# carefree0910/carefree-learn

Hardware: AMD Instinct MI355X
Metric: train samples/sec + step ms, ViT-B/16 bf16 DDP at 1/2/4/8 MI355X (higher is better)
Workload: dtype bf16

## Files before the change

carefree-learn_amd/csrc/common.h:

```cpp
#pragma once
#include <hip/hip_runtime.h>
#include <stdint.h>
#include <stdio.h>
#include <stdarg.h>

#include "../../include/cfhip.h"

typedef uint16_t bf16_t;
typedef __attribute__((ext_vector_type(8))) short bf16x8;
typedef __attribute__((ext_vector_type(4))) short s16x4;
typedef __attribute__((ext_vector_type(4))) float f32x4;
typedef __attribute__((ext_vector_type(2))) unsigned int u32x2;
typedef __attribute__((ext_vector_type(4))) unsigned int u32x4;

#define LDS_PTR(p) ((__attribute__((address_space(3))) void*)(p))

__device__ __forceinline__ void lds_dma16(__amdgpu_buffer_rsrc_t rsrc, const void* lds_dst, unsigned voff) {
#ifdef CFHIP_DMA_BUILTIN
  __builtin_amdgcn_raw_ptr_buffer_load_lds(rsrc, LDS_PTR(const_cast<void*>(lds_dst)), 16, voff, 0, 0, 0);
  return;
#endif
  const unsigned la = (unsigned)(uintptr_t)LDS_PTR(const_cast<void*>(lds_dst));
  asm volatile("s_nop 0\n\tbuffer_load_dwordx4 %1, %2, 0 offen lds" ::"{m0}"(la), "v"(voff), "s"(rsrc) : "memory");
}

__device__ __forceinline__ void lds_dma16_s(__amdgpu_buffer_rsrc_t rsrc, const void* lds_dst, unsigned voff, unsigned soff) {
  const unsigned la = (unsigned)(uintptr_t)LDS_PTR(const_cast<void*>(lds_dst));
  asm volatile("s_nop 0\n\tbuffer_load_dwordx4 %1, %2, %3 offen lds" ::"{m0}"(la), "v"(voff), "s"(rsrc), "s"(soff) : "memory");
}
__device__ __forceinline__ void lds_dma_wait_all() { asm volatile("s_waitcnt vmcnt(0)" ::: "memory"); }

void cfhip_set_error(const char* fmt, ...);

#define CFHIP_REQUIRE(cond, ...)          \
  do {                                    \
    if (!(cond)) {                        \
      cfhip_set_error(__VA_ARGS__);       \
      return CFHIP_ERR_INVALID;           \
    }                                     \
  } while (0)

#define CFHIP_CHECK_LAUNCH(name)                                                \
  do {                                                                          \
    hipError_t e__ = hipGetLastError();                                         \
    if (e__ != hipSuccess) {                                                    \
      cfhip_set_error("%s: launch failed: %s", name, hipGetErrorString(e__));   \
      return CFHIP_ERR_LAUNCH;                                                  \
    }                                                                           \
  } while (0)

__device__ __forceinline__ float bf16_to_f32(bf16_t v) {
  return __uint_as_float(((unsigned)v) << 16);
}
typedef __bf16 bf16x2_native __attribute__((ext_vector_type(2)));
__device__ __forceinline__ bf16_t f32_to_bf16(float f) {
  return __builtin_bit_cast(unsigned short, (__bf16)f);
}
__device__ __forceinline__ unsigned pack_bf16x2(float lo, float hi) {
  const bf16x2_native v = {(__bf16)lo, (__bf16)hi};
  return __builtin_bit_cast(unsigned, v);
}
__device__ __forceinline__ float bf16lo(unsigned w) { return __uint_as_float(w << 16); }
__device__ __forceinline__ float bf16hi(unsigned w) { return __uint_as_float(w & 0xffff0000u); }

__device__ __forceinline__ void gelu_parts(float x, float& cdf, float& e) {
#ifdef CFHIP_GELU_PROBE
  cdf = 0.5f;
  e = 1.0f;
  return;
#endif
  const float t = __builtin_amdgcn_rcpf(fmaf(0.3275911f * 0.70710678118654752440f, fabsf(x), 1.0f));
  e = __builtin_amdgcn_exp2f(x * x * (-0.5f * 1.4426950408889634f));
  float poly = fmaf(t, 1.061405429f, -1.453152027f);
  poly = fmaf(t, poly, 1.421413741f);
  poly = fmaf(t, poly, -0.284496736f);
  poly = fmaf(t, poly, 0.254829592f);
  const float erf_abs = fmaf(-(poly * t), e, 1.0f);
  cdf = fmaf(copysignf(0.5f, x), erf_abs, 0.5f);
}
__device__ __forceinline__ float gelu_erf_f(float x) {
  float cdf, e;
  gelu_parts(x, cdf, e);
  return x * cdf;
}
__device__ __forceinline__ float gelu_erf_grad_f(float x) {
  float cdf, e;
  gelu_parts(x, cdf, e);
  return fmaf(x * 0.39894228040143267794f, e, cdf);
}

__device__ __forceinline__ float sigmoid_1702(float x) {
  return __builtin_amdgcn_rcpf(1.0f + __builtin_amdgcn_exp2f(x * (-1.702f * 1.4426950408889634f)));
}
__device__ __forceinline__ float quick_gelu_f(float x) { return x * sigmoid_1702(x); }
__device__ __forceinline__ float quick_gelu_grad_f(float x) {
  const float s = sigmoid_1702(x);
  return s * fmaf(1.702f * x, 1.0f - s, 1.0f);
}

struct Philox {
  unsigned c[4];
};

__device__ __forceinline__ Philox philox4x32_10(unsigned long long ctr, unsigned long long seed) {
  constexpr unsigned M0 = 0xD2511F53u, M1 = 0xCD9E8D57u, W0 = 0x9E3779B9u, W1 = 0xBB67AE85u;
  unsigned c0 = (unsigned)ctr, c1 = (unsigned)(ctr >> 32), c2 = 0u, c3 = 0u;
  unsigned k0 = (unsigned)seed, k1 = (unsigned)(seed >> 32);
#pragma unroll
  for (int r = 0; r < 10; ++r) {
    const unsigned hi0 = __umulhi(M0, c0), lo0 = M0 * c0;
    const unsigned hi1 = __umulhi(M1, c2), lo1 = M1 * c2;
    c0 = hi1 ^ c1 ^ k0;
    c1 = lo1;
    c2 = hi0 ^ c3 ^ k1;
    c3 = lo0;
    k0 += W0;
    k1 += W1;
  }
  return Philox{{c0, c1, c2, c3}};
}

__device__ __forceinline__ float wave_sum(float v) {
#pragma unroll
  for (int off = 32; off > 0; off >>= 1) v += __shfl_xor(v, off, 64);
  return v;
}
__device__ __forceinline__ float wave_max(float v) {
#pragma unroll
  for (int off = 32; off > 0; off >>= 1) v = fmaxf(v, __shfl_xor(v, off, 64));
  return v;
}
__device__ __forceinline__ float block_sum(float v, float* red) {
  v = wave_sum(v);
  const int lane = threadIdx.x & 63, wave = threadIdx.x >> 6;
  __syncthreads();
  if (lane == 0) red[wave] = v;
  __syncthreads();
  float s = 0.f;
  for (int w = 0; w < (int)(blockDim.x >> 6); ++w) s += red[w];
  return s;
}

__device__ __forceinline__ float ld_act(const void* p, long i, bool f32) {
  return f32 ? reinterpret_cast<const float*>(p)[i] : bf16_to_f32(reinterpret_cast<const bf16_t*>(p)[i]);
}
template <bool IN_F32>
__device__ __forceinline__ void ld_act8(const void* p, long off, float (&v)[8]) {
  if (IN_F32) {
    const f32x4 a = *reinterpret_cast<const f32x4*>(reinterpret_cast<const float*>(p) + off);
    const f32x4 b = *reinterpret_cast<const f32x4*>(reinterpret_cast<const float*>(p) + off + 4);
    v[0] = a[0]; v[1] = a[1]; v[2] = a[2]; v[3] = a[3]; v[4] = b[0]; v[5] = b[1]; v[6] = b[2]; v[7] = b[3];
  } else {
    const u32x4 w = *reinterpret_cast<const u32x4*>(reinterpret_cast<const bf16_t*>(p) + off);
#pragma unroll
    for (int e = 0; e < 4; ++e) {
      v[2 * e] = bf16lo(w[e]);
      v[2 * e + 1] = bf16hi(w[e]);
    }
  }
}
__device__ __forceinline__ void st_bf16x8(bf16_t* p, long off, const float (&v)[8]) {
  *reinterpret_cast<u32x4*>(p + off) = u32x4{pack_bf16x2(v[0], v[1]), pack_bf16x2(v[2], v[3]), pack_bf16x2(v[4], v[5]),
                                             pack_bf16x2(v[6], v[7])};
}
__device__ __forceinline__ float silu_f(float v) { return v * __builtin_amdgcn_rcpf(1.0f + __builtin_amdgcn_exp2f(-1.4426950408889634f * v)); }
__device__ __forceinline__ float silu_grad_f(float v) {
  const float s = __builtin_amdgcn_rcpf(1.0f + __builtin_amdgcn_exp2f(-1.4426950408889634f * v));
  return s * fmaf(v, 1.0f - s, 1.0f);
}
```

carefree-learn_amd/csrc/gemm.hip:

```cpp
#include "gemm_device.h"

namespace {

template <bool AT, bool BT, class C>
struct ItemCtx {
  int m0, n0, z, klen, nk, tile_n;
  __amdgpu_buffer_rsrc_t a_rsrc, b_rsrc;
  StagePlan<C::A_INSTR> pa;
  StagePlan<C::B_INSTR> pb;
  unsigned yx[C::A_INSTR];
  int bshift[C::B_INSTR];
  int btap[C::B_INSTR];
  int kb;
};

template <bool AT, bool BT, class C, int CONV = 0>
__device__ __forceinline__ ItemCtx<AT, BT, C> setup_item(const GemmParams& p, int item, int wave, int lane) {
  ItemCtx<AT, BT, C> c;
  const int ntiles = p.tiles_m * p.tiles_n;
  c.z = item / ntiles;
  const int tile = item - c.z * ntiles;
  int tile_m;
  if (p.group_n > 0) {
    const int per_group = p.group_n * p.tiles_m;
    const int grp = tile / per_group;
    const int first_n = grp * p.group_n;
    const int gw = min(p.group_n, p.tiles_n - first_n);
    const int r = tile - grp * per_group;
    tile_m = r / gw;
    c.tile_n = first_n + (r - tile_m * gw);
  } else if (p.group_n < 0) {
    const int gm = -p.group_n;
    const int per_group = gm * p.tiles_n;
    const int grp = tile / per_group;
    const int first_m = grp * gm;
    const int gh = min(gm, p.tiles_m - first_m);
    const int r = tile - grp * per_group;
    c.tile_n = r / gh;
    tile_m = first_m + (r - c.tile_n * gh);
  } else {
    tile_m = tile / p.tiles_n;
    c.tile_n = tile - tile_m * p.tiles_n;
  }
  c.m0 = tile_m * C::BM;
  c.n0 = c.tile_n * C::BN;
  const int kb = c.z * p.k_chunk;
  c.kb = kb;
  c.klen = min(p.K - kb, p.k_chunk);
  c.nk = (c.klen + C::BK - 1) / C::BK;
  const int rows_a = p.M - c.m0, rows_b = p.N - c.n0;
  const bf16_t* a_base = AT ? p.A + (long)kb * p.lda + c.m0 : p.A + (long)c.m0 * p.lda + kb;
  const bf16_t* b_base = BT ? p.B + (long)kb * p.ldb + c.n0 : p.B + (long)c.n0 * p.ldb + kb;
  const long a_bytes = AT ? ((long)(c.klen - 1) * p.lda + rows_a) * 2 : ((long)(rows_a - 1) * p.lda + c.klen) * 2;
  const long b_bytes = BT ? ((long)(c.klen - 1) * p.ldb + rows_b) * 2 : ((long)(rows_b - 1) * p.ldb + c.klen) * 2;
  if constexpr (CONV == 2) {
    static_assert(CONV != 2 || (AT && BT), "implicit weight gradient: layout (1,1), a K-step = BK pixels");
    const int back = min(kb, p.conv_w + 1);
    const long span = min((long)p.K - (kb - back), (long)back + c.klen + p.conv_w + 1);
    c.b_rsrc = make_rsrc(p.B + (long)(kb - back) * p.conv_c, span * p.conv_c * 2);
    constexpr int SLOTS = C::BN / 8;
#pragma unroll
    for (int j = 0; j < C::B_INSTR; ++j) {
      const int inst = wave * C::B_INSTR + j;
      const int krow = inst * (64 / SLOTS) + lane / SLOTS;
      const int sl = lane % SLOTS;
      const int col = (((sl >> 1) ^ mkey<C::BN>(krow)) << 4) + ((sl & 1) << 3);
      const int n = c.n0 + col;
      const int tap = n / p.conv_c;
      const int ch = n - tap * p.conv_c;
      const int ky = (tap * 11) >> 5;
      const int dy = ky - 1, dx = tap - 3 * ky - 1;
      c.pb.kpos[j] = krow;
      c.pb.voff[j] = (col < rows_b) ? 0u : OOB;
      c.bshift[j] = ((back + krow + dy * p.conv_w + dx) * p.conv_c + ch) * 2;
      c.btap[j] = (dy + 1) | ((dx + 1) << 2);
    }
  } else {
    c.b_rsrc = make_rsrc(b_base, b_bytes);
    c.pb = make_plan<BT, C::BN, C::B_INSTR, C::BK>(wave, lane, p.ldb, C::B_PADDED ? min(rows_b, C::BN) : rows_b);
  }
  if constexpr (CONV == 1) {
    static_assert(!AT, "implicit convolution: k-major A, a K-step = BK channels of one tap");
    const int back = min(c.m0, p.conv_w + 1);
    const long span = min((long)p.M - (c.m0 - back), (long)back + C::BM + p.conv_w + 1);
    c.a_rsrc = make_rsrc(p.A + (long)(c.m0 - back) * p.conv_c, span * p.conv_c * 2);
#pragma unroll
    for (int j = 0; j < C::A_INSTR; ++j) {
      const int inst = wave * C::A_INSTR + j;
      constexpr int SPR = C::BK / 8;
      const int row = inst * (64 / SPR) + lane / SPR;
      const int chunk = (lane % SPR) ^ kswz<C::BK>(row);
      c.pa.kpos[j] = chunk * 8;
      c.pa.voff[j] = (row < rows_a) ? (unsigned)(((back + row) * p.conv_c + chunk * 8) * 2) : OOB;
      const int m = c.m0 + row;
      const int q = m / p.conv_w;
      c.yx[j] = ((unsigned)(q % p.conv_h) << 16) | (unsigned)(m - q * p.conv_w);
    }
  } else {
    c.a_rsrc = make_rsrc(a_base, a_bytes);
    c.pa = make_plan<AT, C::BM, C::A_INSTR, C::BK>(wave, lane, p.lda, rows_a);
  }
  return c;
}

template <class C>
__device__ __forceinline__ void stage_tile_conv(const __amdgpu_buffer_rsrc_t rsrc, char* lds_tile, int wave,
                                                const StagePlan<C::A_INSTR>& pl, const unsigned (&yx)[C::A_INSTR],
                                                const GemmParams& p, int kstep) {
  const int tap = (int)(((float)kstep + 0.5f) * p.conv_inv_kpt);
  const int c0 = (kstep - tap * p.conv_kpt) * C::BK;
  const int ky = (tap * 11) >> 5;
  const int dy = ky - 1, dx = tap - 3 * ky - 1;
  const int shift = ((dy * p.conv_w + dx) * p.conv_c + c0) * 2;
#pragma unroll
  for (int j = 0; j < C::A_INSTR; ++j) {
    const int y = (int)(yx[j] >> 16) + dy, x = (int)(yx[j] & 0xffffu) + dx;
    const bool ok = pl.voff[j] != OOB && (unsigned)y < (unsigned)p.conv_h && (unsigned)x < (unsigned)p.conv_w;
    const unsigned off = ok ? pl.voff[j] + (unsigned)shift : OOB;
    lds_dma16(rsrc, lds_tile + (wave * C::A_INSTR + j) * 1024, off);
  }
}

template <class C, class Ctx>
__device__ __forceinline__ void stage_tile_wgrad(const Ctx& c, char* lds_tile, int wave, const GemmParams& p, int kstep) {
  const int k0 = kstep * C::BK;
#pragma unroll
  for (int j = 0; j < C::B_INSTR; ++j) {
    const int kl = k0 + (int)c.pb.kpos[j];
    const unsigned pix = (unsigned)(c.kb + kl);
    const unsigned q = __umulhi(pix, p.conv_magic_w);
    const int x = (int)(pix - q * (unsigned)p.conv_w) + ((c.btap[j] >> 2) - 1);
    const int y = (int)(q - __umulhi(q, p.conv_magic_h) * (unsigned)p.conv_h) + ((c.btap[j] & 3) - 1);
    const bool ok = c.pb.voff[j] != OOB && kl < c.klen && (unsigned)y < (unsigned)p.conv_h && (unsigned)x < (unsigned)p.conv_w;
    const unsigned off = ok ? (unsigned)(c.bshift[j] + k0 * p.conv_c * 2) : OOB;
    lds_dma16(c.b_rsrc, lds_tile + (wave * C::B_INSTR + j) * 1024, off);
  }
}

template <bool AT, bool BT, class C, int CONV = 0>
__device__ __forceinline__ void stage_step(const ItemCtx<AT, BT, C>& c, const GemmParams& p, char* smem,
                                           int slot, int wave, int kstep) {
  char* st = smem + slot * C::STAGE_BYTES;
  if constexpr (CONV == 1) stage_tile_conv<C>(c.a_rsrc, st, wave, c.pa, c.yx, p, kstep + c.kb / C::BK);
  else stage_tile<AT, C::A_INSTR, C::BK>(c.a_rsrc, st, wave, c.pa, p.lda, kstep * C::BK, c.klen);
  if constexpr (CONV == 2) {
    stage_tile_wgrad<C>(c, st + C::A_BYTES, wave, p, kstep);
    return;
  }
  stage_tile<BT, C::B_INSTR, C::BK>(c.b_rsrc, st + C::A_BYTES, wave, c.pb, p.ldb, kstep * C::BK, c.klen);
}

__device__ __forceinline__ int xcd_item() {
  const int G = gridDim.x;
  const int bid = blockIdx.x;
  const int q8 = G >> 3, r8 = G & 7;
  const int xcd = bid & 7, loc = bid >> 3;
  return (xcd < r8 ? xcd * (q8 + 1) : r8 * (q8 + 1) + (xcd - r8) * q8) + loc;
}

template <bool AT, bool BT, int EPI, class C, int CONV = 0, bool BG = false>
__device__ __forceinline__ void gemm_tile(const GemmParams& p, const int item, char* smem) {
  constexpr int D = C::NSTAGE - 1;
  static_assert(kFlatEpilogue<C> ? C::NW * 16 * (C::FN * 16 + 4) * 4 <= C::LDS_BYTES : C::NW * 16 * (C::FN * 16) * 4 <= C::STAGE_BYTES,
                "epilogue staging must fit in one ring slot (80-column wave tiles: in the ring)");

  const int tid = threadIdx.x;
  const int lane = tid & 63;
  const int wave = __builtin_amdgcn_readfirstlane(tid >> 6);
  const int wm = wave / C::WN, wn = wave % C::WN;

  const ItemCtx<AT, BT, C> cur = setup_item<AT, BT, C, CONV>(p, item, wave, lane);
  const int nk = cur.nk;
  int rd = 0;
#pragma unroll
  for (int st = 0; st < D; ++st)
    if (st < nk) stage_step<AT, BT, C, CONV>(cur, p, smem, st, wave, st);

  f32x4 acc[C::FM][C::FN];
#pragma unroll
  for (int mi = 0; mi < C::FM; ++mi)
#pragma unroll
    for (int ni = 0; ni < C::FN; ++ni) acc[mi][ni] = f32x4{0.f, 0.f, 0.f, 0.f};
  float accb[BG ? C::FM : 1];
  if constexpr (BG) {
#pragma unroll
    for (int mi = 0; mi < C::FM; ++mi) accb[mi] = 0.f;
  }
  const bool do_bg = BG && cur.tile_n == 0 && wn == 0 && (p.bgrad != nullptr || p.bgrad_slabs != nullptr);

  for (int t = 0; t < nk; ++t) {
    const int younger = min(D - 1, nk - 1 - t);
    if (D >= 3 && younger >= 2) CFHIP_WAIT_VMCNT(2 * C::LPS);
    else if (D >= 2 && younger == 1) CFHIP_WAIT_VMCNT(1 * C::LPS);
    else CFHIP_WAIT_VMCNT(0);
    __builtin_amdgcn_s_barrier();
    if (t + D < nk CFHIP_ABLATE_AND(!(p.ablate & 1))) {
      int wr = rd + D;
      if (wr >= C::NSTAGE) wr -= C::NSTAGE;
      stage_step<AT, BT, C, CONV>(cur, p, smem, wr, wave, t + D);
    }
    const char* tile = smem + rd * C::STAGE_BYTES;
    if (true CFHIP_ABLATE_AND(!(p.ablate & 2))) compute_tile<AT, BT, C>(tile, tile + C::A_BYTES, wm, wn, lane, acc);
    if constexpr (BG) {
      if (do_bg) bias_rows<C>(tile, wm, lane, accb);
    }
    rd = rd + 1 == C::NSTAGE ? 0 : rd + 1;
  }
#ifdef CFHIP_ABLATE
  if (p.ablate & 4) return;
#endif
  const int m0 = cur.m0, n0 = cur.n0, z = cur.z;
  if constexpr (BG) {
    if (do_bg) {
#pragma unroll
      for (int mi = 0; mi < C::FM; ++mi) {
        float v = accb[mi];
        v += __shfl_xor(v, 16, 64);
        v += __shfl_xor(v, 32, 64);
        const int m = m0 + wm * (C::FM * 16) + mi * 16 + (lane & 15);
        if ((lane >> 4) == 0 && m < p.M) {
          if (p.bgrad_slabs != nullptr) p.bgrad_slabs[(long)z * p.M + m] = v;
          else p.bgrad[m] = p.bgrad_acc ? p.bgrad[m] + v : v;
        }
      }
    }
  }
  __builtin_amdgcn_s_barrier();
  int eslot = rd - 1;
  if (eslot < 0) eslot += C::NSTAGE;
  epilogue<EPI, C>(p, acc, kFlatEpilogue<C> ? smem : smem + eslot * C::STAGE_BYTES, m0, n0, z, wm, wn, wave, lane);
}

template <bool AT, bool BT, int EPI, class C, int CONV = 0, bool BG = false>
__global__ __launch_bounds__(C::NT, C::WAVES_PER_SIMD)
void gemm_bf16_kernel(GemmParams p) {
  extern __shared__ __attribute__((aligned(16))) char smem[];
  gemm_tile<AT, BT, EPI, C, CONV, BG>(p, xcd_item(), smem);
}

template <bool AT, bool BT, int EPI, class C, int CONV = 0>
__global__ __launch_bounds__(C::NT, C::WAVES_PER_SIMD)
void gemm_bf16_phase_kernel(GemmParams p) {
  extern __shared__ __attribute__((aligned(16))) char smem[];
  static_assert(C::BK == 32 && C::NSTAGE >= 3 && C::NSTAGE <= 7 && C::WM == 2, "phase kernel: BK = 32, 3-7 ring slots, 2 wave rows");
  static_assert(5 * C::LPS < 64, "vmcnt is a 6-bit counter");
  constexpr int D = C::NSTAGE - 1;
  static_assert(C::NW * 16 * (C::FN * 16 + 4) * 4 <= C::LDS_BYTES, "epilogue staging must fit in the (free) ring");
  constexpr int PH = (C::FM / 2) * C::FN >= 16 ? 2 : 1;
  constexpr int HM = C::FM / PH;
  const int nwg = gridDim.x;
  const int bid = blockIdx.x;
  const int q8 = nwg >> 3, r8 = nwg & 7;
  const int xcd = bid & 7, loc = bid >> 3;
  const int item = (xcd < r8 ? xcd * (q8 + 1) : r8 * (q8 + 1) + (xcd - r8) * q8) + loc;
  const int tid = threadIdx.x;
  const int lane = tid & 63;
  const int wave = __builtin_amdgcn_readfirstlane(tid >> 6);
  const int wm = wave / C::WN, wn = wave % C::WN;
  const int i = lane & 15, g = lane >> 4;

  const ItemCtx<AT, BT, C> cur = setup_item<AT, BT, C, CONV>(p, item, wave, lane);
  const int nk = cur.nk;
  f32x4 acc[C::FM][C::FN];
#pragma unroll
  for (int mi = 0; mi < C::FM; ++mi)
#pragma unroll
    for (int ni = 0; ni < C::FN; ++ni) acc[mi][ni] = f32x4{0.f, 0.f, 0.f, 0.f};

#pragma unroll
  for (int st = 0; st < D; ++st)
    if (st < nk) stage_step<AT, BT, C, CONV>(cur, p, smem, st, wave, st);
  wait_stages<C::LPS>(min(min(nk, D) - 1, 5));
  __builtin_amdgcn_s_barrier();
  if (wm == 1) __builtin_amdgcn_s_barrier();

  int rd = 0, wr = D;
  for (int t = 0; t < nk; ++t) {
    const char* a_tile = smem + rd * C::STAGE_BYTES;
    const char* b_tile = a_tile + C::A_BYTES;
    bf16x8 bfr[C::FN], af[HM];
#pragma unroll
    for (int ph = 0; ph < PH; ++ph) {
      if (ph == 0) {
#pragma unroll
        for (int n = 0; n < C::FN; ++n)
          bfr[n] = BT ? frag_mmajor<C::BN>(b_tile, wn * (C::FN * 16) + n * 16, 0, lane)
                      : frag_kmajor<C::BK>(b_tile, wn * (C::FN * 16) + n * 16, 0, i, g);
      }
#pragma unroll
      for (int m = 0; m < HM; ++m)
        af[m] = AT ? frag_mmajor<C::BM>(a_tile, wm * (C::FM * 16) + (ph * HM + m) * 16, 0, lane)
                   : frag_kmajor<C::BK>(a_tile, wm * (C::FM * 16) + (ph * HM + m) * 16, 0, i, g);
      if (ph == PH - 1)
        wait_stages<C::LPS>(max(0, min(min(D - 2, nk - 2 - t), 5)));
      __builtin_amdgcn_sched_barrier(0);
      __builtin_amdgcn_s_barrier();
      __builtin_amdgcn_sched_barrier(0);
      if (ph == PH - 1 && t + D < nk) stage_step<AT, BT, C, CONV>(cur, p, smem, wr, wave, t + D);
      __builtin_amdgcn_s_setprio(1);
#pragma unroll
      for (int m = 0; m < HM; ++m)
#pragma unroll
        for (int n = 0; n < C::FN; ++n)
          acc[ph * HM + m][n] = __builtin_amdgcn_mfma_f32_16x16x32_bf16(bfr[n], af[m], acc[ph * HM + m][n], 0, 0, 0);
      __builtin_amdgcn_s_setprio(0);
      __builtin_amdgcn_sched_barrier(0);
      __builtin_amdgcn_s_barrier();
      __builtin_amdgcn_sched_barrier(0);
    }
    rd = rd + 1 == C::NSTAGE ? 0 : rd + 1;
    wr = wr + 1 == C::NSTAGE ? 0 : wr + 1;
  }
  if (wm == 0) __builtin_amdgcn_s_barrier();
#ifdef CFHIP_ABLATE
  if (p.ablate & 4) return;
#endif
  epilogue<EPI, C>(p, acc, smem, cur.m0, cur.n0, cur.z, wm, wn, wave, lane);
}

__global__ void splitk_reduce_kernel(const float* __restrict__ slabs, void* C, const float* bias,
                                     int M, int N, long ldc, int splits, int out_f32, int accumulate,
                                     const float* __restrict__ bgrad_slabs, float* bgrad, int bgrad_acc) {
  const long n4 = N >> 2;
  const long total = (long)M * n4;
  for (long idx = blockIdx.x * (long)blockDim.x + threadIdx.x; idx < total;
       idx += (long)gridDim.x * blockDim.x) {
    if (bgrad != nullptr && idx < M) {
      float b = 0.f;
      for (int z = 0; z < splits; ++z) b += bgrad_slabs[(long)z * M + idx];
      bgrad[idx] = bgrad_acc ? bgrad[idx] + b : b;
    }
    const int row = (int)(idx / n4);
    const int col = (int)(idx - (long)row * n4) * 4;
    f32x4 v = {0.f, 0.f, 0.f, 0.f};
    for (int z = 0; z < splits; ++z)
      v += *reinterpret_cast<const f32x4*>(slabs + ((long)z * M + row) * N + col);
    if (bias != nullptr) v += *reinterpret_cast<const f32x4*>(bias + col);
    const long off = (long)row * ldc + col;
    if (out_f32) {
      float* dst = reinterpret_cast<float*>(C) + off;
      if (accumulate) v += *reinterpret_cast<const f32x4*>(dst);
      *reinterpret_cast<f32x4*>(dst) = v;
    } else {
      bf16_t* dst = reinterpret_cast<bf16_t*>(C) + off;
      *reinterpret_cast<u32x2*>(dst) = u32x2{pack_bf16x2(v[0], v[1]), pack_bf16x2(v[2], v[3])};
    }
  }
}

__global__ void splitk_reduce_filter_kernel(const float* __restrict__ slabs, float* __restrict__ dW, int Cout, int Cin,
                                            int splits, int accumulate, const float* __restrict__ bgrad_slabs,
                                            float* bgrad, int bgrad_acc) {
  const long c4n = Cin >> 2;
  const long total = (long)Cout * c4n;
  const long N = 9L * Cin;
  for (long idx = blockIdx.x * (long)blockDim.x + threadIdx.x; idx < total; idx += (long)gridDim.x * blockDim.x) {
    if (bgrad != nullptr && idx < Cout) {
      float b = 0.f;
      for (int z = 0; z < splits; ++z) b += bgrad_slabs[(long)z * Cout + idx];
      bgrad[idx] = bgrad_acc ? bgrad[idx] + b : b;
    }
    const int co = (int)(idx / c4n);
    const int c = (int)(idx - (long)co * c4n) * 4;
    float o[36];
#pragma unroll
    for (int tap = 0; tap < 9; ++tap) {
      f32x4 v = {0.f, 0.f, 0.f, 0.f};
      for (int z = 0; z < splits; ++z)
        v += *reinterpret_cast<const f32x4*>(slabs + ((long)z * Cout + co) * N + (long)tap * Cin + c);
#pragma unroll
      for (int e = 0; e < 4; ++e) o[e * 9 + tap] = v[e];
    }
    float* dst = dW + ((long)co * Cin + c) * 9;
#pragma unroll
    for (int i = 0; i < 9; ++i) {
      f32x4 v = {o[4 * i], o[4 * i + 1], o[4 * i + 2], o[4 * i + 3]};
      if (accumulate) v += *reinterpret_cast<const f32x4*>(dst + 4 * i);
      *reinterpret_cast<f32x4*>(dst + 4 * i) = v;
    }
  }
}

__global__ void gemm_bf16_generic_kernel(GemmParams p, int a_trans, int b_trans) {
  const long total = (long)p.M * p.N;
  for (long idx = blockIdx.x * (long)blockDim.x + threadIdx.x; idx < total;
       idx += (long)gridDim.x * blockDim.x) {
    const int m = (int)(idx / p.N), n = (int)(idx - (long)m * p.N);
    float acc = 0.f, asum = 0.f;
    for (int k = 0; k < p.K; ++k) {
      const float a = bf16_to_f32(a_trans ? p.A[(long)k * p.lda + m] : p.A[(long)m * p.lda + k]);
      const float b = bf16_to_f32(b_trans ? p.B[(long)k * p.ldb + n] : p.B[(long)n * p.ldb + k]);
      acc = fmaf(a, b, acc);
      asum += a;
    }
    if (p.bgrad != nullptr && n == 0) p.bgrad[m] = p.bgrad_acc ? p.bgrad[m] + asum : asum;
    if (p.bias != nullptr) acc += p.bias[n];
    const long off = (long)m * p.ldc + n;
    if (p.epilogue == CFHIP_EPI_GELU) {
      const float pre = bf16_to_f32(f32_to_bf16(acc));
      if (p.aux_out != nullptr) p.aux_out[off] = f32_to_bf16(acc);
      acc = p.quick ? quick_gelu_f(pre) : gelu_erf_f(pre);
    } else if (p.epilogue == CFHIP_EPI_RESIDUAL) {
      acc += p.out_f32 ? reinterpret_cast<const float*>(p.aux_in)[off] : bf16_to_f32(p.aux_in[off]);
    } else if (p.epilogue == CFHIP_EPI_DGELU) {
      acc *= p.quick ? quick_gelu_grad_f(bf16_to_f32(p.aux_in[off])) : gelu_erf_grad_f(bf16_to_f32(p.aux_in[off]));
    }
    if (p.out_f32) {
      float* dst = reinterpret_cast<float*>(p.C) + off;
      *dst = p.accumulate ? *dst + acc : acc;
    } else {
      reinterpret_cast<bf16_t*>(p.C)[off] = f32_to_bf16(acc);
    }
  }
}

inline bool aligned16(const void* p) { return (reinterpret_cast<uintptr_t>(p) & 15u) == 0; }

using CfgA = Cfg<128, 128, 2, 2, 2, 64>;
using CfgB = Cfg<128, 128, 2, 2, 2, 32>;
using CfgC = Cfg<128, 128, 2, 2, 3, 32>;
using CfgD = Cfg<128, 64, 2, 2, 2, 64>;
using CfgE = Cfg<128, 128, 2, 2, 4, 32>;
using CfgF = Cfg<128, 64, 2, 2, 2, 32>;
using CfgG = Cfg<128, 64, 2, 2, 3, 32>;
using CfgP = Cfg<256, 256, 2, 4, 4, 32>;
using CfgQ = Cfg<256, 128, 2, 4, 3, 32>;
using CfgR = Cfg<256, 128, 2, 2, 3, 32>;
using CfgS = Cfg<128, 256, 2, 2, 3, 32>;
using CfgT = Cfg<256, 128, 2, 4, 6, 32>;
using CfgU = Cfg<256, 256, 2, 4, 5, 32>;
using CfgW = Cfg<256, 256, 2, 4, 2, 64>;
using CfgY = Cfg<192, 128, 2, 4, 2, 64>;
using CfgZ = Cfg<192, 128, 2, 2, 2, 64>;
using CfgV = Cfg<128, 256, 2, 4, 2, 64>;
using CfgH = Cfg<128, 160, 2, 2, 4, 32>;
using CfgI = Cfg<128, 160, 2, 2, 2, 64>;
constexpr int NUM_CFG = 17;
constexpr int BK_MAX = 64;

int g_gemm_config = -1;
#ifdef CFHIP_ABLATE
int g_gemm_ablate = 0;
#endif
int g_gemm_heuristic = 9;
int g_gemm_group_n = 8;
int g_conv_form = -1;
int g_conv_split = -1;

template <bool AT, bool BT, int EPI, class C, bool PIPE, int CONV = 0>
int launch_cfg(const GemmParams& p, dim3 grid, hipStream_t s) {
  void (*kern)(GemmParams) = nullptr;
  if (PIPE && p.bgrad != nullptr) {
    cfhip_set_error("gemm: the fused bias gradient is not provided by the big-tile kernel (gemm_config 7 / 8)");
    return CFHIP_ERR_INVALID;
  }
  if constexpr (PIPE) kern = gemm_bf16_phase_kernel<AT, BT, EPI, C, CONV>;
  else if constexpr (AT && BT && EPI == CFHIP_EPI_NONE) {
    if (p.bgrad != nullptr) {
      if constexpr (C::BM * C::BN <= 192 * 128) kern = gemm_bf16_kernel<AT, BT, EPI, C, CONV, true>;
      else {
        cfhip_set_error("gemm: the fused bias gradient is not provided by this tile configuration");
        return CFHIP_ERR_INVALID;
      }
    } else kern = gemm_bf16_kernel<AT, BT, EPI, C, CONV, false>;
  } else kern = gemm_bf16_kernel<AT, BT, EPI, C, CONV>;
  static bool attr_done_bg[2] = {false, false};
  bool& attr_done = attr_done_bg[p.bgrad != nullptr ? 1 : 0];
  if (!attr_done && C::LDS_BYTES > 64 * 1024) {
    hipError_t e = hipFuncSetAttribute(reinterpret_cast<const void*>(kern),
                                       hipFuncAttributeMaxDynamicSharedMemorySize, C::LDS_BYTES);
    if (e != hipSuccess) {
      cfhip_set_error("gemm: cannot reserve %d bytes of LDS: %s", C::LDS_BYTES, hipGetErrorString(e));
      return CFHIP_ERR_LAUNCH;
    }
    attr_done = true;
  }
  GemmParams q = p;
  const int gn = g_gemm_group_n;
  q.group_n = (gn > 0 && gn < p.tiles_n) || (gn < 0 && p.tiles_m > 1) ? gn : 0;
  hipLaunchKernelGGL(kern, grid, dim3(C::NT), C::LDS_BYTES, s, q);
  return CFHIP_OK;
}

template <class C, bool PIPE>
constexpr bool kHasEpilogues = !(C::BM == 128 && C::BN == 128 && C::BK == 32 && C::NSTAGE == 2);
template <class C, bool PIPE>
constexpr bool kHasTn = !(PIPE && C::BM == 256 && C::BN == 128 && C::WN == 4 && C::NSTAGE == 3);

template <class C, bool PIPE = false>
int launch_layout(GemmParams p, int a_trans, int b_trans, int epilogue, int split_k, hipStream_t s) {
  p.tiles_m = (p.M + C::BM - 1) / C::BM;
  p.tiles_n = (p.N + C::BN - 1) / C::BN;
  const long a_span = a_trans ? (long)p.k_chunk * p.lda * 2 : (long)C::BM * p.lda * 2;
  const long b_span = b_trans ? (long)p.k_chunk * p.ldb * 2 : (long)C::BN * p.ldb * 2;
  CFHIP_REQUIRE(a_span < 0x7fffffffL && b_span < 0x7fffffffL,
                "gemm: operand tile span exceeds 2 GiB (lda=%ld ldb=%ld K=%d)", p.lda, p.ldb, p.K);
  p.splits = split_k;
  dim3 grid(p.tiles_m * p.tiles_n * split_k);
  if (!a_trans && !b_trans) {
    switch (epilogue) {
      case CFHIP_EPI_NONE: return launch_cfg<false, false, CFHIP_EPI_NONE, C, PIPE>(p, grid, s);
      case CFHIP_EPI_GELU: return launch_cfg<false, false, CFHIP_EPI_GELU, C, PIPE>(p, grid, s);
      case CFHIP_EPI_RESIDUAL:
        if constexpr (kHasEpilogues<C, PIPE>) return launch_cfg<false, false, CFHIP_EPI_RESIDUAL, C, PIPE>(p, grid, s);
        break;
      default: break;
    }
  } else if (!a_trans && b_trans) {
    switch (epilogue) {
      case CFHIP_EPI_NONE: return launch_cfg<false, true, CFHIP_EPI_NONE, C, PIPE>(p, grid, s);
      case CFHIP_EPI_DGELU:
        if constexpr (kHasEpilogues<C, PIPE>) return launch_cfg<false, true, CFHIP_EPI_DGELU, C, PIPE>(p, grid, s);
        break;
      default: break;
    }
  } else if (epilogue == CFHIP_EPI_NONE) {
    if constexpr (kHasTn<C, PIPE>) return launch_cfg<true, true, CFHIP_EPI_NONE, C, PIPE>(p, grid, s);
  }
  cfhip_set_error("gemm: epilogue %d is not provided for layout (%d,%d)", epilogue, a_trans, b_trans);
  return CFHIP_ERR_INVALID;
}

int g_cfg_class[4] = {-1, -1, -1, -1};

int pick_config(int M, int N, int a_trans, int b_trans) {
  if (g_gemm_config >= 0 && g_gemm_config < NUM_CFG) return g_gemm_config;
  if (M >= 1024 || a_trans) {
    const int cls = a_trans ? 3 : b_trans ? 2 : (N >= 2560 ? 0 : 1);
    if (g_cfg_class[cls] >= 0 && g_cfg_class[cls] < NUM_CFG) return g_cfg_class[cls];
  }
  if (g_gemm_heuristic >= 7) {
    if (a_trans) return 1;
    if (M >= 512) {
      const long t14 = (long)((M + 191) / 192) * ((N + 127) / 128);
      if (t14 < 160 || (N < 512 && N % 128 != 0 && N % 64 == 0)) return 3;
    }
    if (M >= 1024) return (g_gemm_heuristic >= 9 || (g_gemm_heuristic >= 8 && N <= 1024)) ? 15 : 14;
    if (b_trans) return 1;
    return N <= 1024 ? 3 : 0;
  }
  if (g_gemm_heuristic >= 6) {
    if (a_trans) return 1;
    if (M >= 1024) {
      if (b_trans) return 8;
      return N >= 2560 ? 14 : 0;
    }
    if (b_trans) return 1;
    return N <= 1024 ? 3 : 0;
  }
  if (g_gemm_heuristic == 1) {
    if (a_trans && (long)M * N <= 768L * 768L) return 0;
    if (a_trans || b_trans) return 1;
    return N <= 1024 ? 1 : 0;
  }
  if (g_gemm_heuristic >= 2) {
    if (a_trans) return 1;
    if (N >= 2560 && M >= 1024) return 8;
    if (g_gemm_heuristic >= 4 && b_trans && M >= 1024) return 8;
    if (g_gemm_heuristic >= 5 && M >= 1024) return 8;
    if (g_gemm_heuristic >= 3) {
      const long tiles128 = (long)((M + 127) / 128) * ((N + 127) / 128);
      if (tiles128 >= 1024) return 0;
    }
  }
  if (a_trans || b_trans) return 1;
  if (N <= 1024) return 3;
  return 0;
}

}

#ifdef CFHIP_ABLATE
int cfhip_internal_set_attn_ablate(int v);
#endif
int cfhip_internal_set_ln_fused(int v);
int cfhip_internal_set_attn_persistent(int v);
int cfhip_internal_set_attn_one_pass(int v);
int cfhip_internal_set_attn_pers_ctas(int v);
int cfhip_internal_set_grouped_variant(int v);
int cfhip_internal_set_attn_two_tiles(int v);
int cfhip_internal_set_attn_short_max(int v);

extern "C" int cfhip_set_option(const char* name, int value) {
  if (name != nullptr && strcmp(name, "gemm_config") == 0) {
    g_gemm_config = value;
    return CFHIP_OK;
  }
  if (name != nullptr && strcmp(name, "gemm_heuristic") == 0) {
    g_gemm_heuristic = value;
    return CFHIP_OK;
  }
  static const char* const cls_names[4] = {"gemm_cfg_nt_wide", "gemm_cfg_nt", "gemm_cfg_nn", "gemm_cfg_tn"};
  for (int i = 0; i < 4; ++i)
    if (name != nullptr && strcmp(name, cls_names[i]) == 0) {
      g_cfg_class[i] = value;
      return CFHIP_OK;
    }
  if (name != nullptr && strcmp(name, "gemm_group_n") == 0) {
    g_gemm_group_n = value;
    return CFHIP_OK;
  }
  if (name != nullptr && strcmp(name, "conv_form") == 0) {
    g_conv_form = value;
    return CFHIP_OK;
  }
  if (name != nullptr && strcmp(name, "conv_split") == 0) {
    g_conv_split = value;
    return CFHIP_OK;
  }
  if (name != nullptr && strcmp(name, "ln_bwd_fused") == 0) return cfhip_internal_set_ln_fused(value);
  if (name != nullptr && strcmp(name, "attn_persistent") == 0) return cfhip_internal_set_attn_persistent(value);
  if (name != nullptr && strcmp(name, "attn_one_pass") == 0) return cfhip_internal_set_attn_one_pass(value);
  if (name != nullptr && strcmp(name, "attn_pers_ctas") == 0) return cfhip_internal_set_attn_pers_ctas(value);
  if (name != nullptr && strcmp(name, "grouped_variant") == 0) return cfhip_internal_set_grouped_variant(value);
  if (name != nullptr && strcmp(name, "attn_two_tiles") == 0) return cfhip_internal_set_attn_two_tiles(value);
  if (name != nullptr && strcmp(name, "attn_short_max") == 0) return cfhip_internal_set_attn_short_max(value);
#ifdef CFHIP_ABLATE
  if (name != nullptr && strcmp(name, "gemm_ablate") == 0) {
    g_gemm_ablate = value;
    return CFHIP_OK;
  }
  if (name != nullptr && strcmp(name, "attn_ablate") == 0) return cfhip_internal_set_attn_ablate(value);
#endif
  cfhip_set_error("set_option: unknown option '%s'", name ? name : "(null)");
  return CFHIP_ERR_INVALID;
}

static int resolve_config(int cfg, int a_trans, int epilogue, bool bias_grad) {
  if (cfg == 8 && a_trans) cfg = 1;
  if (bias_grad && ((cfg >= 7 && cfg <= 13) || cfg == 16)) cfg = 1;
  if (cfg == 1 && (epilogue == CFHIP_EPI_RESIDUAL || epilogue == CFHIP_EPI_DGELU)) cfg = 3;
  return cfg;
}

extern "C" int cfhip_gemm_kernel_name(int M, int N, int K, int a_trans, int b_trans, int epilogue, char* out, size_t out_bytes) {
  CFHIP_REQUIRE(out != nullptr && out_bytes >= 96, "gemm_kernel_name: buffer of at least 96 bytes");
  static const char* const cfg_names[NUM_CFG] = {
      "Cfg<128, 128, 2, 2, 2, 64>", "Cfg<128, 128, 2, 2, 2, 32>", "Cfg<128, 128, 2, 2, 3, 32>", "Cfg<128, 64, 2, 2, 2, 64>",
      "Cfg<128, 128, 2, 2, 4, 32>", "Cfg<128, 64, 2, 2, 2, 32>", "Cfg<128, 64, 2, 2, 3, 32>", "Cfg<256, 256, 2, 4, 4, 32>",
      "Cfg<256, 128, 2, 4, 3, 32>", "Cfg<256, 128, 2, 2, 3, 32>", "Cfg<128, 256, 2, 2, 3, 32>", "Cfg<256, 128, 2, 4, 6, 32>",
      "Cfg<256, 256, 2, 4, 5, 32>", "Cfg<256, 256, 2, 4, 2, 64>", "Cfg<192, 128, 2, 4, 2, 64>", "Cfg<192, 128, 2, 2, 2, 64>",
      "Cfg<128, 256, 2, 4, 2, 64>"};
  int epi = epilogue == CFHIP_EPI_QGELU ? CFHIP_EPI_GELU : epilogue == CFHIP_EPI_DQGELU ? CFHIP_EPI_DGELU : epilogue;
  int cfg = pick_config(M, N, a_trans, b_trans);
  cfg = resolve_config(cfg, a_trans, epi, false);
  const bool phase = cfg >= 7 && cfg <= 12;
  snprintf(out, out_bytes, "%s<%s, %s, %d, %s>", phase ? "gemm_bf16_phase_kernel" : "gemm_bf16_kernel",
           a_trans ? "true" : "false", b_trans ? "true" : "false", epi, cfg_names[cfg]);
  return CFHIP_OK;
}

static thread_local int g_last_config = -2;
extern "C" int cfhip_gemm_last_config(void) { return g_last_config; }

static int gemm_bf16_impl(const void* A, const void* B, void* C, const float* bias,
                          const void* aux_in, void* aux_out, int M, int N, int K, int64_t lda,
                          int64_t ldb, int64_t ldc, int a_trans, int b_trans, int epilogue,
                          int out_dtype, int accumulate, int split_k, void* workspace,
                          size_t workspace_bytes, float* bias_grad, int bias_grad_accumulate,
                          void* stream, int config_rows) {
  CFHIP_REQUIRE(A && B && C, "gemm: null operand");
  CFHIP_REQUIRE(bias_grad == nullptr || (a_trans && b_trans),
                "gemm: the fused bias gradient exists for layout (1,1) only");
  CFHIP_REQUIRE(M > 0 && N > 0 && K > 0, "gemm: empty problem M=%d N=%d K=%d", M, N, K);
  CFHIP_REQUIRE(epilogue >= 0 && epilogue <= 5, "gemm: bad epilogue %d", epilogue);
  const int quick = epilogue == CFHIP_EPI_QGELU || epilogue == CFHIP_EPI_DQGELU;
  if (epilogue == CFHIP_EPI_QGELU) epilogue = CFHIP_EPI_GELU;
  if (epilogue == CFHIP_EPI_DQGELU) epilogue = CFHIP_EPI_DGELU;
  CFHIP_REQUIRE(!(epilogue == CFHIP_EPI_RESIDUAL || epilogue == CFHIP_EPI_DGELU) || aux_in,
                "gemm: epilogue %d needs aux_in", epilogue);
  CFHIP_REQUIRE(!accumulate || (out_dtype == 1 && epilogue == CFHIP_EPI_NONE), "gemm: accumulate needs f32 output and epilogue NONE");
  CFHIP_REQUIRE(!(epilogue == CFHIP_EPI_GELU || epilogue == CFHIP_EPI_DGELU) || out_dtype == 0,
                "gemm: the GELU / GELU' epilogues write bf16");
  CFHIP_REQUIRE(!(a_trans && !b_trans), "gemm: layout (a_trans=1, b_trans=0) is not provided");
  if (split_k < 1) split_k = 1;
  hipStream_t s = reinterpret_cast<hipStream_t>(stream);

  GemmParams p;
  p.A = reinterpret_cast<const bf16_t*>(A);
  p.B = reinterpret_cast<const bf16_t*>(B);
  p.C = C;
  p.bias = bias;
  p.aux_in = reinterpret_cast<const bf16_t*>(aux_in);
  p.aux_out = reinterpret_cast<bf16_t*>(aux_out);
  p.M = M; p.N = N; p.K = K;
  p.lda = lda; p.ldb = ldb; p.ldc = ldc;
  p.epilogue = epilogue; p.out_f32 = out_dtype; p.accumulate = accumulate;
  p.slabs = nullptr;
  p.tiles_m = p.tiles_n = 0;
  p.quick = quick;
#ifdef CFHIP_ABLATE
  p.ablate = g_gemm_ablate;
#endif
  p.bgrad = bias_grad;
  p.bgrad_acc = bias_grad_accumulate;
  p.bgrad_slabs = nullptr;
  p.conv_h = p.conv_w = p.conv_c = p.conv_kpt = 0;
  p.conv_inv_kpt = 0.f;
  p.conv_magic_w = p.conv_magic_h = 0u;
  p.k_chunk = ((K + BK_MAX - 1) / BK_MAX) * BK_MAX;

  const bool k_ok = (a_trans && b_trans) || (K % 8 == 0);
  const bool fast = k_ok && (lda % 8 == 0) && (ldb % 8 == 0) && (N % 4 == 0) &&
                    (ldc % 4 == 0) && (!a_trans || M % 8 == 0) && (!b_trans || N % 8 == 0) &&
                    aligned16(A) && aligned16(B) && aligned16(C) &&
                    (bias == nullptr || aligned16(bias)) && (aux_in == nullptr || aligned16(aux_in)) &&
                    (aux_out == nullptr || aligned16(aux_out));
  if (!fast) {
    CFHIP_REQUIRE(split_k == 1, "gemm: split_k needs the aligned fast path");
    const long total = (long)M * N;
    const int blocks = (int)((total + 255) / 256 > 65535 ? 65535 : (total + 255) / 256);
    g_last_config = -1;
    hipLaunchKernelGGL(gemm_bf16_generic_kernel, dim3(blocks), dim3(256), 0, s, p, a_trans, b_trans);
    CFHIP_CHECK_LAUNCH("gemm_generic");
    return CFHIP_OK;
  }

  if (split_k > 1) {
    CFHIP_REQUIRE(epilogue == CFHIP_EPI_NONE, "gemm: split_k supports epilogue NONE only");
    const int steps = (K + BK_MAX - 1) / BK_MAX;
    if (split_k > steps) split_k = steps;
    const int per = (steps + split_k - 1) / split_k;
    split_k = (steps + per - 1) / per;
    p.k_chunk = per * BK_MAX;
  }
  if (split_k > 1) {
    const size_t need = (size_t)split_k * M * N * sizeof(float) + (bias_grad ? (size_t)split_k * M * sizeof(float) : 0);
    if (workspace == nullptr || workspace_bytes < need) {
      cfhip_set_error("gemm: split_k=%d needs %zu workspace bytes, got %zu", split_k, need, workspace_bytes);
      return CFHIP_ERR_WORKSPACE;
    }
    p.slabs = reinterpret_cast<float*>(workspace);
    if (bias_grad) p.bgrad_slabs = p.slabs + (size_t)split_k * M * N;
  }

  int rc;
  int cfg = pick_config(config_rows > M ? config_rows : M, N, a_trans, b_trans);
  cfg = resolve_config(cfg, a_trans, epilogue, bias_grad != nullptr);
  g_last_config = cfg;
  switch (cfg) {
    case 1: rc = launch_layout<CfgB>(p, a_trans, b_trans, epilogue, split_k, s); break;
    case 2: rc = launch_layout<CfgC>(p, a_trans, b_trans, epilogue, split_k, s); break;
    case 3: rc = launch_layout<CfgD>(p, a_trans, b_trans, epilogue, split_k, s); break;
    case 4: rc = launch_layout<CfgE>(p, a_trans, b_trans, epilogue, split_k, s); break;
    case 5: rc = launch_layout<CfgF>(p, a_trans, b_trans, epilogue, split_k, s); break;
    case 6: rc = launch_layout<CfgG>(p, a_trans, b_trans, epilogue, split_k, s); break;
    case 7: rc = launch_layout<CfgP, true>(p, a_trans, b_trans, epilogue, split_k, s); break;
    case 8: rc = launch_layout<CfgQ, true>(p, a_trans, b_trans, epilogue, split_k, s); break;
    case 9: rc = launch_layout<CfgR, true>(p, a_trans, b_trans, epilogue, split_k, s); break;
    case 10: rc = launch_layout<CfgS, true>(p, a_trans, b_trans, epilogue, split_k, s); break;
    case 11: rc = launch_layout<CfgT, true>(p, a_trans, b_trans, epilogue, split_k, s); break;
    case 12: rc = launch_layout<CfgU, true>(p, a_trans, b_trans, epilogue, split_k, s); break;
    case 13: rc = launch_layout<CfgW>(p, a_trans, b_trans, epilogue, split_k, s); break;
    case 14: rc = launch_layout<CfgY>(p, a_trans, b_trans, epilogue, split_k, s); break;
    case 15: rc = launch_layout<CfgZ>(p, a_trans, b_trans, epilogue, split_k, s); break;
    case 16: rc = launch_layout<CfgV>(p, a_trans, b_trans, epilogue, split_k, s); break;
    default: rc = launch_layout<CfgA>(p, a_trans, b_trans, epilogue, split_k, s); break;
  }
  if (rc != CFHIP_OK) return rc;
  CFHIP_CHECK_LAUNCH("gemm_bf16");

  if (split_k > 1) {
    const long total = (long)M * (N / 4);
    int blocks = (int)((total + 255) / 256);
    if (blocks > 2048) blocks = 2048;
    hipLaunchKernelGGL(splitk_reduce_kernel, dim3(blocks), dim3(256), 0, s, p.slabs, C, bias, M, N,
                       (long)ldc, split_k, out_dtype, accumulate, p.bgrad_slabs, p.bgrad, p.bgrad_acc);
    CFHIP_CHECK_LAUNCH("splitk_reduce");
  }
  return CFHIP_OK;
}

extern "C" int cfhip_gemm_bf16(const void* A, const void* B, void* C, const float* bias,
                               const void* aux_in, void* aux_out, int M, int N, int K, int64_t lda,
                               int64_t ldb, int64_t ldc, int a_trans, int b_trans, int epilogue,
                               int out_dtype, int accumulate, int split_k, void* workspace,
                               size_t workspace_bytes, float* bias_grad, int bias_grad_accumulate,
                               void* stream) {
  return gemm_bf16_impl(A, B, C, bias, aux_in, aux_out, M, N, K, lda, ldb, ldc, a_trans, b_trans, epilogue, out_dtype, accumulate,
                        split_k, workspace, workspace_bytes, bias_grad, bias_grad_accumulate, stream, 0);
}

extern "C" int cfhip_gemm_bf16_rows(const void* A, const void* B, void* C, const float* bias, const void* aux_in, void* aux_out,
                                    int M, int N, int K, int64_t lda, int64_t ldb, int64_t ldc, int b_trans, int epilogue,
                                    int out_dtype, int config_rows, void* stream) {
  CFHIP_REQUIRE(config_rows >= M, "gemm_rows: config_rows = %d is less than M = %d", config_rows, M);
  return gemm_bf16_impl(A, B, C, bias, aux_in, aux_out, M, N, K, lda, ldb, ldc, 0, b_trans, epilogue, out_dtype, 0, 1, nullptr, 0,
                        nullptr, 0, stream, config_rows);
}

template <class C, bool PIPE>
static int launch_conv(GemmParams p, int split_k, hipStream_t s) {
  p.tiles_m = (p.M + C::BM - 1) / C::BM;
  p.tiles_n = (p.N + C::BN - 1) / C::BN;
  p.splits = split_k;
  return launch_cfg<false, false, CFHIP_EPI_NONE, C, PIPE, 1>(p, dim3(p.tiles_m * p.tiles_n * split_k), s);
}

struct ConvPlan { int form, split; };

static int conv_split_for(long tiles, long slots, int Cin) {
  const int steps = (9 * Cin + BK_MAX - 1) / BK_MAX;
  if (tiles * 2 > slots || steps < 16) return 1;
  long split = (slots + tiles - 1) / tiles;
  if (split > steps / 8) split = steps / 8;
  if (split < 1) split = 1;
  const int per = (int)((steps + split - 1) / split);
  return (steps + per - 1) / per;
}

static ConvPlan conv_plan(long pixels, int Cin, int Cout) {
  ConvPlan pl;
  pl.form = pixels >= 1024 ? 0 : 1;
  if (g_conv_form != -2 && (long)((Cout + 159) / 160) * 160 * 8 <= 9L * Cout) pl.form = 3;
  if (g_conv_form >= 0 && g_conv_form <= 3) pl.form = g_conv_form;
  static const int bm[4] = {256, 128, 128, 128}, bn[4] = {128, 128, 160, 160}, slots[4] = {512, 1024, 512, 512};
  if (pl.form == 3 && Cin % 64 != 0) pl.form = 2;
  const long tiles = ((pixels + bm[pl.form] - 1) / bm[pl.form]) * ((Cout + bn[pl.form] - 1) / bn[pl.form]);
  pl.split = conv_split_for(tiles, slots[pl.form], Cin);
  if (g_conv_split >= 1) {
    const int steps = (9 * Cin + BK_MAX - 1) / BK_MAX;
    int split = g_conv_split > steps ? steps : g_conv_split;
    const int per = (steps + split - 1) / split;
    pl.split = (steps + per - 1) / per;
  }
  return pl;
}

extern "C" size_t cfhip_conv3x3_workspace(int B, int H, int W, int Cin, int Cout) {
  const long pixels = (long)B * H * W;
  const int split = conv_plan(pixels, Cin, Cout).split;
  return split > 1 ? (size_t)split * pixels * Cout * sizeof(float) : 0;
}

extern "C" int cfhip_conv3x3_nhwc_bf16(const void* X, const void* Wk, const float* bias, void* Y, int B, int H, int W,
                                       int Cin, int Cout, void* workspace, size_t workspace_bytes, void* stream) {
  CFHIP_REQUIRE(X && Wk && Y, "conv3x3: null operand");
  CFHIP_REQUIRE(B > 0 && H > 0 && W > 0 && H < 65536 && W < 65536, "conv3x3: bad image shape %d x %d x %d", B, H, W);
  CFHIP_REQUIRE(Cin > 0 && Cin % 32 == 0, "conv3x3: Cin = %d must be a multiple of 32 (one K-step = 32 channels of a tap)", Cin);
  CFHIP_REQUIRE(Cout > 0 && Cout % 8 == 0, "conv3x3: Cout = %d must be a multiple of 8", Cout);
  const long pixels = (long)B * H * W;
  CFHIP_REQUIRE(pixels < (1L << 30) && 9L * Cin < (1L << 20), "conv3x3: problem too large (%ld pixels, Cin %d)", pixels, Cin);
  CFHIP_REQUIRE(aligned16(X) && aligned16(Wk) && aligned16(Y) && (bias == nullptr || aligned16(bias)),
                "conv3x3: operands must be 16-byte aligned");
  GemmParams p;
  p.A = reinterpret_cast<const bf16_t*>(X);
  p.B = reinterpret_cast<const bf16_t*>(Wk);
  p.C = Y;
  p.bias = bias;
  p.aux_in = nullptr;
  p.aux_out = nullptr;
  p.M = (int)pixels; p.N = Cout; p.K = 9 * Cin;
  p.lda = Cin; p.ldb = 9L * Cin; p.ldc = Cout;
  p.epilogue = CFHIP_EPI_NONE; p.out_f32 = 0; p.accumulate = 0;
  p.k_chunk = ((p.K + BK_MAX - 1) / BK_MAX) * BK_MAX;
  p.slabs = nullptr;
  p.tiles_m = p.tiles_n = 0; p.splits = 1;
  p.bgrad = nullptr; p.bgrad_slabs = nullptr; p.bgrad_acc = 0;
  p.quick = 0;
#ifdef CFHIP_ABLATE
  p.ablate = 0;
#endif
  p.conv_h = H; p.conv_w = W; p.conv_c = Cin; p.conv_kpt = Cin / 32;
  p.conv_inv_kpt = 1.0f / (float)p.conv_kpt;
  p.conv_magic_w = p.conv_magic_h = 0u;
  const ConvPlan plan = conv_plan(pixels, Cin, Cout);
  const int split = plan.split;
  if (split > 1) {
    const size_t need = (size_t)split * pixels * Cout * sizeof(float);
    if (workspace == nullptr || workspace_bytes < need) {
      cfhip_set_error("conv3x3: split_k=%d needs %zu workspace bytes (cfhip_conv3x3_workspace), got %zu", split, need, workspace_bytes);
      return CFHIP_ERR_WORKSPACE;
    }
    const int steps = (p.K + BK_MAX - 1) / BK_MAX;
    p.k_chunk = ((steps + split - 1) / split) * BK_MAX;
    p.slabs = reinterpret_cast<float*>(workspace);
  }
  hipStream_t s = (hipStream_t)stream;
  int rc;
  switch (plan.form) {
    case 0: rc = launch_conv<CfgQ, true>(p, split, s); break;
    case 2: rc = launch_conv<CfgH, false>(p, split, s); break;
    case 3:
      p.conv_kpt = Cin / 64;
      p.conv_inv_kpt = 1.0f / (float)p.conv_kpt;
      rc = launch_conv<CfgI, false>(p, split, s);
      break;
    default: rc = launch_conv<CfgB, false>(p, split, s); break;
  }
  if (rc != CFHIP_OK) return rc;
  CFHIP_CHECK_LAUNCH("conv3x3_nhwc");
  if (split > 1) {
    const long total = (long)p.M * (p.N / 4);
    int blocks = (int)((total + 255) / 256);
    if (blocks > 2048) blocks = 2048;
    hipLaunchKernelGGL(splitk_reduce_kernel, dim3(blocks), dim3(256), 0, s, p.slabs, Y, bias, p.M, p.N, (long)p.ldc, split,
                       0, 0, (const float*)nullptr, (float*)nullptr, 0);
    CFHIP_CHECK_LAUNCH("splitk_reduce");
  }
  return CFHIP_OK;
}

extern "C" size_t cfhip_conv3x3_wgrad_workspace(int Cin, int Cout, int split_k) {
  if (split_k < 1) split_k = 1;
  return (size_t)split_k * Cout * (9 * (size_t)Cin + 1) * sizeof(float);
}

extern "C" int cfhip_conv3x3_wgrad_nhwc_bf16(const void* dY, const void* X, float* dW, int accumulate, float* bias_grad,
                                             int bias_grad_accumulate, int B, int H, int W, int Cin, int Cout,
                                             int split_k, void* workspace, size_t workspace_bytes, void* stream) {
  CFHIP_REQUIRE(dY && X && dW, "conv3x3_wgrad: null operand");
  CFHIP_REQUIRE(B > 0 && H >= 2 && W >= 2 && H < 65536 && W < 65536, "conv3x3_wgrad: bad image shape %d x %d x %d", B, H, W);
  CFHIP_REQUIRE(Cin > 0 && Cin % 8 == 0 && Cout > 0 && Cout % 8 == 0, "conv3x3_wgrad: Cin = %d and Cout = %d must be multiples of 8", Cin, Cout);
  const long pixels = (long)B * H * W;
  CFHIP_REQUIRE(pixels * (W > H ? W : H) < (1L << 32) && 9L * Cin < (1L << 20),
                "conv3x3_wgrad: problem too large (%ld pixels of %d x %d, Cin %d)", pixels, H, W, Cin);
  CFHIP_REQUIRE(aligned16(dY) && aligned16(X) && aligned16(dW), "conv3x3_wgrad: operands must be 16-byte aligned");
  if (split_k < 1) split_k = 1;
  GemmParams p;
  p.A = reinterpret_cast<const bf16_t*>(dY);
  p.B = reinterpret_cast<const bf16_t*>(X);
  p.C = nullptr;
  p.bias = nullptr; p.aux_in = nullptr; p.aux_out = nullptr;
  p.M = Cout; p.N = 9 * Cin; p.K = (int)pixels;
  p.lda = Cout; p.ldb = Cin; p.ldc = 9L * Cin;
  p.epilogue = CFHIP_EPI_NONE; p.out_f32 = 1; p.accumulate = 0;
  p.bgrad = bias_grad; p.bgrad_acc = bias_grad_accumulate; p.bgrad_slabs = nullptr;
  p.quick = 0;
#ifdef CFHIP_ABLATE
  p.ablate = 0;
#endif
  p.conv_h = H; p.conv_w = W; p.conv_c = Cin; p.conv_kpt = 0; p.conv_inv_kpt = 0.f;
  p.conv_magic_w = (unsigned)((1ULL << 32) / (unsigned)W + 1ULL);
  p.conv_magic_h = (unsigned)((1ULL << 32) / (unsigned)H + 1ULL);
  const int steps = (p.K + BK_MAX - 1) / BK_MAX;
  if (split_k > steps) split_k = steps;
  const int per = (steps + split_k - 1) / split_k;
  split_k = (steps + per - 1) / per;
  p.k_chunk = per * BK_MAX;
  CFHIP_REQUIRE(((long)p.k_chunk + 2L * W + 2) * Cin * 2 < 0x7fffffffL && (long)p.k_chunk * Cout * 2 < 0x7fffffffL,
                "conv3x3_wgrad: a K slice of %d pixels exceeds the 2 GiB descriptor range (raise split_k)", p.k_chunk);
  const size_t need = (size_t)split_k * p.M * p.N * sizeof(float) + (bias_grad ? (size_t)split_k * p.M * sizeof(float) : 0);
  if (workspace == nullptr || workspace_bytes < need) {
    cfhip_set_error("conv3x3_wgrad: split_k=%d needs %zu workspace bytes, got %zu", split_k, need, workspace_bytes);
    return CFHIP_ERR_WORKSPACE;
  }
  p.slabs = reinterpret_cast<float*>(workspace);
  if (bias_grad) p.bgrad_slabs = p.slabs + (size_t)split_k * p.M * p.N;
  p.splits = split_k;
  hipStream_t s = (hipStream_t)stream;
  p.tiles_m = (p.M + CfgC::BM - 1) / CfgC::BM;
  p.tiles_n = (p.N + CfgC::BN - 1) / CfgC::BN;
  const int rc = launch_cfg<true, true, CFHIP_EPI_NONE, CfgC, false, 2>(p, dim3(p.tiles_m * p.tiles_n * split_k), s);
  if (rc != CFHIP_OK) return rc;
  CFHIP_CHECK_LAUNCH("conv3x3_wgrad");
  const long total = (long)Cout * (Cin / 4);
  int blocks = (int)((total + 255) / 256);
  if (blocks > 2048) blocks = 2048;
  hipLaunchKernelGGL(splitk_reduce_filter_kernel, dim3(blocks), dim3(256), 0, s, p.slabs, dW, Cout, Cin, split_k, accumulate,
                     p.bgrad_slabs, p.bgrad, p.bgrad_acc);
  CFHIP_CHECK_LAUNCH("splitk_reduce_filter");
  return CFHIP_OK;
}
```

carefree-learn_amd/csrc/gemm_device.h:

```cpp
#pragma once
#include "common.h"
#include <string.h>

namespace {

constexpr unsigned OOB = 0x80000000u;

struct GemmParams {
  const bf16_t* A;
  const bf16_t* B;
  void* C;
  const float* bias;
  const bf16_t* aux_in;
  bf16_t* aux_out;
  int M, N, K;
  long lda, ldb, ldc;
  int epilogue, out_f32, accumulate;
  int k_chunk;
  float* slabs;
  int tiles_m, tiles_n, splits;
  float* bgrad;
  float* bgrad_slabs;
  int bgrad_acc;
  int quick;
  int conv_h, conv_w, conv_c, conv_kpt;
  float conv_inv_kpt;
  unsigned conv_magic_w, conv_magic_h;
  int group_n;
#ifdef CFHIP_ABLATE
  int ablate;
#endif
};

template <int BM_, int BN_, int WM_, int WN_, int NSTAGE_, int BK_>
struct Cfg {
  static constexpr int BM = BM_, BN = BN_, WM = WM_, WN = WN_, NSTAGE = NSTAGE_, BK = BK_;
  static constexpr int NW = WM * WN, NT = NW * 64;
  static constexpr int FM = BM / WM / 16, FN = BN / WN / 16;
  static constexpr int A_BYTES = BM * BK * 2, B_RAW = BN * BK * 2;
  static constexpr int B_BYTES = (B_RAW + 1024 * WM_ * WN_ - 1) / (1024 * WM_ * WN_) * (1024 * WM_ * WN_), STAGE_BYTES = A_BYTES + B_BYTES;
  static constexpr bool B_PADDED = B_BYTES != B_RAW;
  static constexpr int LDS_BYTES = STAGE_BYTES * NSTAGE;
  static constexpr int A_INSTR = A_BYTES / 1024 / NW, B_INSTR = B_BYTES / 1024 / NW;
  static constexpr int LPS = A_INSTR + B_INSTR;
  static constexpr int WGS_PER_CU = (160 * 1024 / LDS_BYTES) > (16 / NW) ? (16 / NW) : (160 * 1024 / LDS_BYTES);
  static constexpr int WAVES_PER_SIMD = WGS_PER_CU * NW / 4 < 1 ? 1 : WGS_PER_CU * NW / 4;
  static_assert(BK == 32 || BK == 64, "K-step must be 32 or 64");
  static_assert(A_BYTES % (1024 * NW) == 0 && B_BYTES % (1024 * NW) == 0, "tiles must split evenly over the waves");
};

__device__ __forceinline__ __amdgpu_buffer_rsrc_t make_rsrc(const void* base, long bytes) {
  if (bytes > 0x7fffffffL) bytes = 0x7fffffffL;
  if (bytes < 0) bytes = 0;
  return __builtin_amdgcn_make_buffer_rsrc(const_cast<void*>(base), 0, (int)bytes, 0x00020000);
}

template <int NI>
struct StagePlan {
  unsigned voff[NI];
  unsigned kpos[NI];
};

template <int BK>
__device__ __forceinline__ int kswz(int row) { return BK == 64 ? ((row >> 1) & 7) : ((row >> 2) & 3); }

template <int R>
__device__ __forceinline__ int mkey(int krow) {
  return R % 128 == 0 ? ((krow & 3) | (((krow >> 3) & 1) << 2)) : (((krow >> 1) & 1) | (((krow >> 3) & 1) << 1));
}

template <int R>
__device__ __forceinline__ int mkey32(int krow) {
  return R % 128 == 0 ? ((krow & 3) << 1) : (krow & 2);
}

template <bool TRANS, int R, int NI, int BK, bool KEY32 = false>
__device__ __forceinline__ StagePlan<NI> make_plan(int wave, int lane, long ld, int extent_valid) {
  StagePlan<NI> p;
#pragma unroll
  for (int j = 0; j < NI; ++j) {
    const int inst = wave * NI + j;
    if constexpr (!TRANS) {
      constexpr int SPR = BK / 8;
      const int row = inst * (64 / SPR) + lane / SPR;
      const int chunk = (lane % SPR) ^ kswz<BK>(row);
      p.kpos[j] = chunk * 8;
      p.voff[j] = (row < extent_valid) ? (unsigned)(row * ld * 2 + chunk * 16) : OOB;
    } else {
      static_assert(R % 64 == 0, "m-major tiles: whole 128-byte lines per k-row (mkey / mkey32)");
      constexpr int SLOTS = R / 8;
      const int slot = inst * 64 + lane;
      const int krow = slot / SLOTS;
      const int s = slot - krow * SLOTS;
      const int col = (((s >> 1) ^ (KEY32 ? mkey32<R>(krow) : mkey<R>(krow))) << 4) + ((s & 1) << 3);
      p.kpos[j] = krow;
      p.voff[j] = (col < extent_valid) ? (unsigned)(krow * ld * 2 + col * 2) : OOB;
    }
  }
  return p;
}

template <bool TRANS, int NI, int BKS = 0>
__device__ __forceinline__ void stage_tile(__amdgpu_buffer_rsrc_t rsrc, char* lds_tile, int wave,
                                           const StagePlan<NI>& p, long ld, int k0, int klen) {
  if (BKS > 0 && k0 + BKS <= klen) {
    const unsigned soff = TRANS ? (unsigned)((long)k0 * ld * 2) : (unsigned)(k0 * 2);
#pragma unroll
    for (int j = 0; j < NI; ++j) lds_dma16_s(rsrc, lds_tile + (wave * NI + j) * 1024, p.voff[j], soff);
    return;
  }
#pragma unroll
  for (int j = 0; j < NI; ++j) {
    unsigned off = TRANS ? p.voff[j] + (unsigned)((long)k0 * ld * 2) : p.voff[j] + (unsigned)(k0 * 2);
    off = ((int)(k0 + p.kpos[j]) < klen && p.voff[j] != OOB) ? off : OOB;
    lds_dma16(rsrc, lds_tile + (wave * NI + j) * 1024, off);
  }
}

template <int BK>
__device__ __forceinline__ bf16x8 frag_kmajor(const char* tile, int r0, int ks, int i, int g) {
  const int row = r0 + i;
  const int slot = (ks * 4 + g) ^ kswz<BK>(row);
  return *reinterpret_cast<const bf16x8*>(tile + row * (BK * 2) + slot * 16);
}

template <int R>
__device__ __forceinline__ bf16x8 frag_mmajor(const char* tile, int c0, int ks, int lane) {
  const int g = lane >> 4;
  const int j = (lane & 15) >> 2;
  const int q = lane & 3;
  const int krow = ks * 32 + g * 8 + j;
  const char* p = tile + krow * (R * 2) + (((c0 >> 4) ^ mkey<R>(krow)) << 5) + q * 8;
  s16x4 lo = __builtin_amdgcn_ds_read_tr16_b64_v4i16(
      (__attribute__((address_space(3))) s16x4*)LDS_PTR(p));
  s16x4 hi = __builtin_amdgcn_ds_read_tr16_b64_v4i16(
      (__attribute__((address_space(3))) s16x4*)LDS_PTR(p + 4 * (R * 2)));
  bf16x8 r;
  r[0] = lo[0]; r[1] = lo[1]; r[2] = lo[2]; r[3] = lo[3];
  r[4] = hi[0]; r[5] = hi[1]; r[6] = hi[2]; r[7] = hi[3];
  return r;
}

template <bool AT, bool BT, class C>
__device__ __forceinline__ void compute_tile(const char* a_tile, const char* b_tile, int wm, int wn,
                                             int lane, f32x4 (&acc)[C::FM][C::FN]) {
  const int i = lane & 15, g = lane >> 4;
  constexpr int KS = C::BK / 32;
  constexpr bool PRELOAD = KS == 2 && C::WAVES_PER_SIMD <= 3;
  bf16x8 af[KS][C::FM], bfr[KS][C::FN];
#pragma unroll
  for (int ks = 0; ks < KS; ++ks) {
#pragma unroll
    for (int t = 0; t < C::FM; ++t)
      af[ks][t] = AT ? frag_mmajor<C::BM>(a_tile, wm * (C::FM * 16) + t * 16, ks, lane)
                     : frag_kmajor<C::BK>(a_tile, wm * (C::FM * 16) + t * 16, ks, i, g);
#pragma unroll
    for (int t = 0; t < C::FN; ++t)
      bfr[ks][t] = BT ? frag_mmajor<C::BN>(b_tile, wn * (C::FN * 16) + t * 16, ks, lane)
                      : frag_kmajor<C::BK>(b_tile, wn * (C::FN * 16) + t * 16, ks, i, g);
    if (!PRELOAD) {
#pragma unroll
      for (int mi = 0; mi < C::FM; ++mi)
#pragma unroll
        for (int ni = 0; ni < C::FN; ++ni)
          acc[mi][ni] = __builtin_amdgcn_mfma_f32_16x16x32_bf16(bfr[ks][ni], af[ks][mi], acc[mi][ni], 0, 0, 0);
    }
  }
  if (PRELOAD) {
    __builtin_amdgcn_sched_barrier(0);
#pragma unroll
    for (int ks = 0; ks < KS; ++ks)
#pragma unroll
      for (int mi = 0; mi < C::FM; ++mi)
#pragma unroll
        for (int ni = 0; ni < C::FN; ++ni)
          acc[mi][ni] = __builtin_amdgcn_mfma_f32_16x16x32_bf16(bfr[ks][ni], af[ks][mi], acc[mi][ni], 0, 0, 0);
  }
}

template <class C>
__device__ __forceinline__ void bias_rows(const char* a_tile, int wm, int lane, float (&accb)[C::FM]) {
#pragma unroll
  for (int ks = 0; ks < C::BK / 32; ++ks)
#pragma unroll
    for (int mi = 0; mi < C::FM; ++mi) {
      union { bf16x8 v; unsigned w[4]; } u;
      u.v = frag_mmajor<C::BM>(a_tile, wm * (C::FM * 16) + mi * 16, ks, lane);
      accb[mi] += ((bf16lo(u.w[0]) + bf16hi(u.w[0])) + (bf16lo(u.w[1]) + bf16hi(u.w[1]))) +
                  ((bf16lo(u.w[2]) + bf16hi(u.w[2])) + (bf16lo(u.w[3]) + bf16hi(u.w[3])));
    }
}

#define CFHIP_WAIT_VMCNT(N) asm volatile("s_waitcnt vmcnt(%0)" ::"n"(N) : "memory")

template <int LPS>
__device__ __forceinline__ void wait_stages(int n) {
  switch (n) {
    case 0: CFHIP_WAIT_VMCNT(0); break;
    case 1: CFHIP_WAIT_VMCNT(1 * LPS); break;
    case 2: CFHIP_WAIT_VMCNT(2 * LPS); break;
    case 3: CFHIP_WAIT_VMCNT(3 * LPS); break;
    case 4: CFHIP_WAIT_VMCNT(4 * LPS); break;
    default: CFHIP_WAIT_VMCNT(5 * LPS); break;
  }
}

#ifdef CFHIP_ABLATE
#define CFHIP_ABLATE_AND(cond) && (cond)
#else
#define CFHIP_ABLATE_AND(cond)
#endif


struct AuxRegs { u32x4 a, b; };
#ifndef CFHIP_PF_F32
#define CFHIP_PF_F32 2
#endif
#ifndef CFHIP_PF_BF16
#define CFHIP_PF_BF16 4
#endif

#ifndef CFHIP_ST_AUX
#define CFHIP_ST_AUX 0
#endif
#ifndef CFHIP_LD_AUX
#define CFHIP_LD_AUX 0
#endif
__device__ __forceinline__ u32x4 bload16(__amdgpu_buffer_rsrc_t r, unsigned off) {
  return __builtin_bit_cast(u32x4, __builtin_amdgcn_raw_buffer_load_b128(r, (int)off, 0, CFHIP_LD_AUX));
}
__device__ __forceinline__ u32x2 bload8(__amdgpu_buffer_rsrc_t r, unsigned off) {
  return __builtin_bit_cast(u32x2, __builtin_amdgcn_raw_buffer_load_b64(r, (int)off, 0, CFHIP_LD_AUX));
}
__device__ __forceinline__ void bstore16(__amdgpu_buffer_rsrc_t r, unsigned off, u32x4 v) {
  __builtin_amdgcn_raw_buffer_store_b128(__builtin_bit_cast(__attribute__((ext_vector_type(4))) unsigned int, v), r, (int)off, 0, CFHIP_ST_AUX);
}
__device__ __forceinline__ void bstore8(__amdgpu_buffer_rsrc_t r, unsigned off, u32x2 v) {
  __builtin_amdgcn_raw_buffer_store_b64(__builtin_bit_cast(__attribute__((ext_vector_type(2))) unsigned int, v), r, (int)off, 0, CFHIP_ST_AUX);
}
#ifdef CFHIP_EPI_AUX_TEMPORAL
#define CFHIP_PRE_AUX 0
#else
#define CFHIP_PRE_AUX 2
#endif
__device__ __forceinline__ u32x4 bload16_pre(__amdgpu_buffer_rsrc_t r, unsigned off) {
  return __builtin_bit_cast(u32x4, __builtin_amdgcn_raw_buffer_load_b128(r, (int)off, 0, CFHIP_PRE_AUX));
}
__device__ __forceinline__ u32x2 bload8_pre(__amdgpu_buffer_rsrc_t r, unsigned off) {
  return __builtin_bit_cast(u32x2, __builtin_amdgcn_raw_buffer_load_b64(r, (int)off, 0, CFHIP_PRE_AUX));
}
__device__ __forceinline__ void bstore16_pre(__amdgpu_buffer_rsrc_t r, unsigned off, u32x4 v) {
  __builtin_amdgcn_raw_buffer_store_b128(__builtin_bit_cast(__attribute__((ext_vector_type(4))) unsigned int, v), r, (int)off, 0, CFHIP_PRE_AUX);
}
__device__ __forceinline__ void bstore8_pre(__amdgpu_buffer_rsrc_t r, unsigned off, u32x2 v) {
  __builtin_amdgcn_raw_buffer_store_b64(__builtin_bit_cast(__attribute__((ext_vector_type(2))) unsigned int, v), r, (int)off, 0, CFHIP_PRE_AUX);
}
__device__ __forceinline__ __amdgpu_buffer_rsrc_t tile_rsrc(const void* base, long ld, int es, int m0, int n0, int M, int N) {
  const char* origin = reinterpret_cast<const char*>(base) + ((long)m0 * ld + n0) * es;
  return make_rsrc(origin, ((long)(M - 1 - m0) * ld + (N - n0)) * es);
}

template <int EPI, class C, bool F32, bool N8, bool QUICK>
__device__ __forceinline__ void epilogue_impl(const GemmParams& p, f32x4 (&acc)[C::FM][C::FN], char* stage,
                                              int m0, int n0, int wm, int wn, int wave, int lane) {
  constexpr int WCOLS = C::FN * 16;
  constexpr int LPR = WCOLS / 8;
  constexpr int RPP = 64 / LPR;
  constexpr int PPM = 16 / RPP;
  constexpr int NIT = C::FM * PPM;
  constexpr bool HAS_AUX = EPI == CFHIP_EPI_RESIDUAL || EPI == CFHIP_EPI_DGELU;
  constexpr bool AUX_F32 = EPI == CFHIP_EPI_RESIDUAL && F32;
  constexpr int PFW = AUX_F32 ? CFHIP_PF_F32 : CFHIP_PF_BF16;
  constexpr int PF = HAS_AUX ? (PFW < NIT ? PFW : NIT) : 1;
  constexpr int ES = F32 ? 4 : 2, AES = AUX_F32 ? 4 : 2;
  float* stg = reinterpret_cast<float*>(stage) + wave * (16 * WCOLS);
  const int i = lane & 15, g = lane >> 4;
  const int rr = lane / LPR, c8 = lane % LPR;
  const int lcol = wn * WCOLS + c8 * 8;
  const bool c_lo = n0 + lcol < p.N, c_hi = n0 + lcol + 4 < p.N;
  const int lrow0 = wm * (C::FM * 16) + rr;
  f32x4 b_lo = {0.f, 0.f, 0.f, 0.f}, b_hi = {0.f, 0.f, 0.f, 0.f};
  if (p.bias != nullptr) {
    if (c_lo) b_lo = *reinterpret_cast<const f32x4*>(p.bias + n0 + lcol);
    if (c_hi) b_hi = *reinterpret_cast<const f32x4*>(p.bias + n0 + lcol + 4);
  }
  const __amdgpu_buffer_rsrc_t c_rsrc = tile_rsrc(p.C, p.ldc, ES, m0, n0, p.M, p.N);
  __amdgpu_buffer_rsrc_t x_rsrc = c_rsrc, o_rsrc = c_rsrc;
  if constexpr (HAS_AUX) x_rsrc = tile_rsrc(p.aux_in, p.ldc, AES, m0, n0, p.M, p.N);
  if constexpr (EPI == CFHIP_EPI_GELU) o_rsrc = tile_rsrc(p.aux_out, p.ldc, 2, m0, n0, p.M, p.N);
  const bool has_pre = EPI == CFHIP_EPI_GELU && p.aux_out != nullptr;
  auto eoff = [&](int it) -> unsigned { return (unsigned)((lrow0 + (it / PPM) * 16 + (it % PPM) * RPP) * (int)p.ldc + lcol); };
  auto load_aux = [&](int it) -> AuxRegs {
    AuxRegs r;
    r.b = u32x4{0u, 0u, 0u, 0u};
    const unsigned e = eoff(it);
    if constexpr (AUX_F32) {
      r.a = bload16(x_rsrc, c_lo ? e * 4u : OOB);
      r.b = bload16(x_rsrc, c_hi ? e * 4u + 16u : OOB);
    } else if constexpr (EPI == CFHIP_EPI_DGELU) {
      if constexpr (N8) {
        r.a = bload16_pre(x_rsrc, c_lo ? e * 2u : OOB);
      } else {
        const u32x2 h0 = bload8_pre(x_rsrc, c_lo ? e * 2u : OOB), h1 = bload8_pre(x_rsrc, c_hi ? e * 2u + 8u : OOB);
        r.a = u32x4{h0[0], h0[1], h1[0], h1[1]};
      }
    } else if constexpr (N8) {
      r.a = bload16(x_rsrc, c_lo ? e * 2u : OOB);
    } else {
      const u32x2 h0 = bload8(x_rsrc, c_lo ? e * 2u : OOB), h1 = bload8(x_rsrc, c_hi ? e * 2u + 8u : OOB);
      r.a = u32x4{h0[0], h0[1], h1[0], h1[1]};
    }
    return r;
  };
  AuxRegs ring[PF];
  if constexpr (HAS_AUX) {
#pragma unroll
    for (int it = 0; it < PF; ++it) ring[it] = load_aux(it);
  }
#pragma unroll
  for (int it = 0; it < NIT; ++it) {
    const int mi = it / PPM, ps = it % PPM;
    if (ps == 0) {
#pragma unroll
      for (int ni = 0; ni < C::FN; ++ni)
        *reinterpret_cast<f32x4*>(stg + i * WCOLS + (((ni * 4 + g) ^ (i & 7)) << 2)) = acc[mi][ni];
    }
    const int r = ps * RPP + rr;
    f32x4 lo = *reinterpret_cast<const f32x4*>(stg + r * WCOLS + (((2 * c8) ^ (r & 7)) << 2));
    f32x4 hi = *reinterpret_cast<const f32x4*>(stg + r * WCOLS + (((2 * c8 + 1) ^ (r & 7)) << 2));
    AuxRegs aux;
    if constexpr (HAS_AUX) {
      aux = ring[it % PF];
      if (it + PF < NIT) ring[it % PF] = load_aux(it + PF);
    }
    const unsigned e = eoff(it);
    lo += b_lo;
    hi += b_hi;
    if constexpr (EPI == CFHIP_EPI_GELU) {
      const u32x4 w = {pack_bf16x2(lo[0], lo[1]), pack_bf16x2(lo[2], lo[3]), pack_bf16x2(hi[0], hi[1]),
                       pack_bf16x2(hi[2], hi[3])};
      if constexpr (N8) {
        bstore16_pre(o_rsrc, (has_pre && c_lo) ? e * 2u : OOB, w);
      } else {
        bstore8_pre(o_rsrc, (has_pre && c_lo) ? e * 2u : OOB, u32x2{w[0], w[1]});
        bstore8_pre(o_rsrc, (has_pre && c_hi) ? e * 2u + 8u : OOB, u32x2{w[2], w[3]});
      }
      if constexpr (QUICK) {
        lo = f32x4{quick_gelu_f(bf16lo(w[0])), quick_gelu_f(bf16hi(w[0])), quick_gelu_f(bf16lo(w[1])), quick_gelu_f(bf16hi(w[1]))};
        hi = f32x4{quick_gelu_f(bf16lo(w[2])), quick_gelu_f(bf16hi(w[2])), quick_gelu_f(bf16lo(w[3])), quick_gelu_f(bf16hi(w[3]))};
      } else {
        lo = f32x4{gelu_erf_f(bf16lo(w[0])), gelu_erf_f(bf16hi(w[0])), gelu_erf_f(bf16lo(w[1])), gelu_erf_f(bf16hi(w[1]))};
        hi = f32x4{gelu_erf_f(bf16lo(w[2])), gelu_erf_f(bf16hi(w[2])), gelu_erf_f(bf16lo(w[3])), gelu_erf_f(bf16hi(w[3]))};
      }
    } else if constexpr (AUX_F32) {
      lo += __builtin_bit_cast(f32x4, aux.a);
      hi += __builtin_bit_cast(f32x4, aux.b);
    } else if constexpr (HAS_AUX) {
      const u32x4 w = aux.a;
      if constexpr (EPI == CFHIP_EPI_RESIDUAL) {
        lo += f32x4{bf16lo(w[0]), bf16hi(w[0]), bf16lo(w[1]), bf16hi(w[1])};
        hi += f32x4{bf16lo(w[2]), bf16hi(w[2]), bf16lo(w[3]), bf16hi(w[3])};
      } else if constexpr (QUICK) {
        lo *= f32x4{quick_gelu_grad_f(bf16lo(w[0])), quick_gelu_grad_f(bf16hi(w[0])), quick_gelu_grad_f(bf16lo(w[1])), quick_gelu_grad_f(bf16hi(w[1]))};
        hi *= f32x4{quick_gelu_grad_f(bf16lo(w[2])), quick_gelu_grad_f(bf16hi(w[2])), quick_gelu_grad_f(bf16lo(w[3])), quick_gelu_grad_f(bf16hi(w[3]))};
      } else {
        lo *= f32x4{gelu_erf_grad_f(bf16lo(w[0])), gelu_erf_grad_f(bf16hi(w[0])), gelu_erf_grad_f(bf16lo(w[1])), gelu_erf_grad_f(bf16hi(w[1]))};
        hi *= f32x4{gelu_erf_grad_f(bf16lo(w[2])), gelu_erf_grad_f(bf16hi(w[2])), gelu_erf_grad_f(bf16lo(w[3])), gelu_erf_grad_f(bf16hi(w[3]))};
      }
    }
    if constexpr (F32) {
      if constexpr (EPI == CFHIP_EPI_NONE) {
        if (p.accumulate) {
          lo += __builtin_bit_cast(f32x4, bload16(c_rsrc, c_lo ? e * 4u : OOB));
          hi += __builtin_bit_cast(f32x4, bload16(c_rsrc, c_hi ? e * 4u + 16u : OOB));
        }
      }
#ifdef CFHIP_ABLATE
      if ((p.ablate & 8) && lo[0] != 12345.678f) continue;
#endif
      bstore16(c_rsrc, c_lo ? e * 4u : OOB, __builtin_bit_cast(u32x4, lo));
      bstore16(c_rsrc, c_hi ? e * 4u + 16u : OOB, __builtin_bit_cast(u32x4, hi));
    } else {
      const u32x4 w = {pack_bf16x2(lo[0], lo[1]), pack_bf16x2(lo[2], lo[3]), pack_bf16x2(hi[0], hi[1]),
                       pack_bf16x2(hi[2], hi[3])};
#ifdef CFHIP_ABLATE
      if ((p.ablate & 8) && w[0] != 0x12345678u) continue;
#endif
      if constexpr (N8) {
        bstore16(c_rsrc, c_lo ? e * 2u : OOB, w);
      } else {
        bstore8(c_rsrc, c_lo ? e * 2u : OOB, u32x2{w[0], w[1]});
        bstore8(c_rsrc, c_hi ? e * 2u + 8u : OOB, u32x2{w[2], w[3]});
      }
    }
  }
}

template <int EPI, class C>
__device__ __forceinline__ void epilogue_f32(const GemmParams& p, f32x4 (&acc)[C::FM][C::FN], char* stage,
                                             int m0, int n0, int wm, int wn, int wave, int lane) {
  static_assert(EPI == CFHIP_EPI_NONE || EPI == CFHIP_EPI_RESIDUAL, "f32 output: bias / residual / accumulate only");
  constexpr int WCOLS = C::FN * 16;
  constexpr int LPR = WCOLS / 4;
  constexpr int RPP = 64 / LPR;
  constexpr int PPM = 16 / RPP;
  constexpr int NIT = C::FM * PPM;
  constexpr bool HAS_AUX = EPI == CFHIP_EPI_RESIDUAL;
  constexpr int PF = HAS_AUX ? (CFHIP_PF_BF16 < NIT ? CFHIP_PF_BF16 : NIT) : 1;
  float* stg = reinterpret_cast<float*>(stage) + wave * (16 * WCOLS);
  const int i = lane & 15, g = lane >> 4;
  const int rr = lane / LPR, c4 = lane % LPR;
  const int lcol = wn * WCOLS + c4 * 4;
  const bool c_ok = n0 + lcol < p.N;
  const int lrow0 = wm * (C::FM * 16) + rr;
  f32x4 bias = {0.f, 0.f, 0.f, 0.f};
  if (p.bias != nullptr && c_ok) bias = *reinterpret_cast<const f32x4*>(p.bias + n0 + lcol);
  const __amdgpu_buffer_rsrc_t c_rsrc = tile_rsrc(p.C, p.ldc, 4, m0, n0, p.M, p.N);
  __amdgpu_buffer_rsrc_t x_rsrc = c_rsrc;
  if constexpr (HAS_AUX) x_rsrc = tile_rsrc(p.aux_in, p.ldc, 4, m0, n0, p.M, p.N);
  auto boff = [&](int it) -> unsigned {
    return c_ok ? (unsigned)((lrow0 + (it / PPM) * 16 + (it % PPM) * RPP) * (int)p.ldc + lcol) * 4u : OOB;
  };
  u32x4 ring[PF];
  if constexpr (HAS_AUX) {
#pragma unroll
    for (int it = 0; it < PF; ++it) ring[it] = bload16(x_rsrc, boff(it));
  }
#pragma unroll
  for (int it = 0; it < NIT; ++it) {
    const int mi = it / PPM, ps = it % PPM;
    if (ps == 0) {
#pragma unroll
      for (int ni = 0; ni < C::FN; ++ni)
        *reinterpret_cast<f32x4*>(stg + i * WCOLS + (((ni * 4 + g) ^ (i & 7)) << 2)) = acc[mi][ni];
    }
    const int r = ps * RPP + rr;
    f32x4 v = *reinterpret_cast<const f32x4*>(stg + r * WCOLS + ((c4 ^ (r & 7)) << 2));
    v += bias;
    if constexpr (HAS_AUX) {
      v += __builtin_bit_cast(f32x4, ring[it % PF]);
      if (it + PF < NIT) ring[it % PF] = bload16(x_rsrc, boff(it + PF));
    }
    const unsigned off = boff(it);
    if constexpr (EPI == CFHIP_EPI_NONE) {
      if (p.accumulate) v += __builtin_bit_cast(f32x4, bload16(c_rsrc, off));
    }
#ifdef CFHIP_ABLATE
    if ((p.ablate & 8) && v[0] != 12345.678f) continue;
#endif
    bstore16(c_rsrc, off, __builtin_bit_cast(u32x4, v));
  }
}

template <class C>
__device__ __forceinline__ void epilogue_slab(const GemmParams& p, f32x4 (&acc)[C::FM][C::FN], char* stage,
                                              int m0, int n0, int z, int wm, int wn, int wave, int lane) {
  constexpr int WCOLS = C::FN * 16, LPR = WCOLS / 4, RPP = 64 / LPR;
  float* stg = reinterpret_cast<float*>(stage) + wave * (16 * WCOLS);
  const int i = lane & 15, g = lane >> 4;
  const int rr = lane / LPR, c4 = lane % LPR;
  const int lcol = wn * WCOLS + c4 * 4;
  const bool c_ok = n0 + lcol < p.N;
  const __amdgpu_buffer_rsrc_t s_rsrc = tile_rsrc(p.slabs + (long)z * p.M * p.N, p.N, 4, m0, n0, p.M, p.N);
#pragma unroll
  for (int mi = 0; mi < C::FM; ++mi) {
#pragma unroll
    for (int ni = 0; ni < C::FN; ++ni)
      *reinterpret_cast<f32x4*>(stg + i * WCOLS + (((ni * 4 + g) ^ (i & 7)) << 2)) = acc[mi][ni];
#pragma unroll
    for (int ps = 0; ps < 16 / RPP; ++ps) {
      const int r = ps * RPP + rr;
      const f32x4 v = *reinterpret_cast<const f32x4*>(stg + r * WCOLS + ((c4 ^ (r & 7)) << 2));
      const unsigned e = (unsigned)((wm * (C::FM * 16) + mi * 16 + r) * p.N + lcol);
      bstore16(s_rsrc, c_ok ? e * 4u : OOB, __builtin_bit_cast(u32x4, v));
    }
  }
}

template <class C>
__device__ __forceinline__ void epilogue_flat(const GemmParams& p, f32x4 (&acc)[C::FM][C::FN], char* stage,
                                              int m0, int n0, int z, int wm, int wn, int wave, int lane) {
  constexpr int WCOLS = C::FN * 16, PITCH = WCOLS + 4;
  float* stg = reinterpret_cast<float*>(stage) + wave * (16 * PITCH);
  const int i = lane & 15, g = lane >> 4;
  if (p.slabs != nullptr) {
    constexpr int CPR = WCOLS / 4, NCH = 16 * CPR, NP = (NCH + 63) / 64;
    const __amdgpu_buffer_rsrc_t s_rsrc = tile_rsrc(p.slabs + (long)z * p.M * p.N, p.N, 4, m0, n0, p.M, p.N);
    int srow[NP], scol[NP];
    bool sok[NP];
#pragma unroll
    for (int ps = 0; ps < NP; ++ps) {
      const int c = ps * 64 + lane;
      srow[ps] = c / CPR;
      scol[ps] = (c - srow[ps] * CPR) * 4;
      sok[ps] = c < NCH && n0 + wn * WCOLS + scol[ps] < p.N;
    }
#pragma unroll
    for (int mi = 0; mi < C::FM; ++mi) {
#pragma unroll
      for (int ni = 0; ni < C::FN; ++ni) *reinterpret_cast<f32x4*>(stg + i * PITCH + ni * 16 + g * 4) = acc[mi][ni];
#pragma unroll
      for (int ps = 0; ps < NP; ++ps) {
        const int r = sok[ps] ? srow[ps] : 0;
        const f32x4 v = *reinterpret_cast<const f32x4*>(stg + r * PITCH + (sok[ps] ? scol[ps] : 0));
        const unsigned e = (unsigned)((wm * (C::FM * 16) + mi * 16 + srow[ps]) * p.N + wn * WCOLS + scol[ps]);
        bstore16(s_rsrc, sok[ps] ? e * 4u : OOB, __builtin_bit_cast(u32x4, v));
      }
    }
    return;
  }
  constexpr int CPR = WCOLS / 8, NCH = 16 * CPR, NP = (NCH + 63) / 64;
  const __amdgpu_buffer_rsrc_t c_rsrc = tile_rsrc(p.C, p.ldc, 2, m0, n0, p.M, p.N);
  int srow[NP], scol[NP];
  bool sok[NP];
  f32x4 b_lo[NP], b_hi[NP];
#pragma unroll
  for (int ps = 0; ps < NP; ++ps) {
    const int c = ps * 64 + lane;
    srow[ps] = c / CPR;
    scol[ps] = (c - srow[ps] * CPR) * 8;
    const int col = n0 + wn * WCOLS + scol[ps];
    sok[ps] = c < NCH && col < p.N;
    b_lo[ps] = b_hi[ps] = f32x4{0.f, 0.f, 0.f, 0.f};
    if (p.bias != nullptr && sok[ps]) {
      b_lo[ps] = *reinterpret_cast<const f32x4*>(p.bias + col);
      b_hi[ps] = *reinterpret_cast<const f32x4*>(p.bias + col + 4);
    }
  }
#pragma unroll
  for (int mi = 0; mi < C::FM; ++mi) {
#pragma unroll
    for (int ni = 0; ni < C::FN; ++ni) *reinterpret_cast<f32x4*>(stg + i * PITCH + ni * 16 + g * 4) = acc[mi][ni];
#pragma unroll
    for (int ps = 0; ps < NP; ++ps) {
      const int r = sok[ps] ? srow[ps] : 0, cc = sok[ps] ? scol[ps] : 0;
      const f32x4 lo = *reinterpret_cast<const f32x4*>(stg + r * PITCH + cc) + b_lo[ps];
      const f32x4 hi = *reinterpret_cast<const f32x4*>(stg + r * PITCH + cc + 4) + b_hi[ps];
      const u32x4 w = {pack_bf16x2(lo[0], lo[1]), pack_bf16x2(lo[2], lo[3]), pack_bf16x2(hi[0], hi[1]), pack_bf16x2(hi[2], hi[3])};
      const unsigned e = (unsigned)((wm * (C::FM * 16) + mi * 16 + srow[ps]) * (int)p.ldc + wn * WCOLS + scol[ps]);
      bstore16(c_rsrc, sok[ps] ? e * 2u : OOB, w);
    }
  }
}

template <class C>
constexpr bool kFlatEpilogue = 64 % (C::FN * 2) != 0;

template <int EPI, class C>
__device__ __forceinline__ void epilogue_std(const GemmParams& p, f32x4 (&acc)[C::FM][C::FN], char* stage,
                                             int m0, int n0, int z, int wm, int wn, int wave, int lane) {
  if constexpr (EPI == CFHIP_EPI_NONE) {
    if (p.slabs != nullptr) {
      epilogue_slab<C>(p, acc, stage, m0, n0, z, wm, wn, wave, lane);
      return;
    }
  }
  if constexpr (EPI == CFHIP_EPI_GELU || EPI == CFHIP_EPI_DGELU) {
    if (p.quick) {
      if ((p.N & 7) == 0) epilogue_impl<EPI, C, false, true, true>(p, acc, stage, m0, n0, wm, wn, wave, lane);
      else epilogue_impl<EPI, C, false, false, true>(p, acc, stage, m0, n0, wm, wn, wave, lane);
    } else {
      if ((p.N & 7) == 0) epilogue_impl<EPI, C, false, true, false>(p, acc, stage, m0, n0, wm, wn, wave, lane);
      else epilogue_impl<EPI, C, false, false, false>(p, acc, stage, m0, n0, wm, wn, wave, lane);
    }
  } else {
    if (p.out_f32) epilogue_f32<EPI, C>(p, acc, stage, m0, n0, wm, wn, wave, lane);
    else if ((p.N & 7) == 0) epilogue_impl<EPI, C, false, true, false>(p, acc, stage, m0, n0, wm, wn, wave, lane);
    else epilogue_impl<EPI, C, false, false, false>(p, acc, stage, m0, n0, wm, wn, wave, lane);
  }
}

template <int EPI, class C>
__device__ __forceinline__ void epilogue(const GemmParams& p, f32x4 (&acc)[C::FM][C::FN], char* stage,
                                         int m0, int n0, int z, int wm, int wn, int wave, int lane) {
  if constexpr (kFlatEpilogue<C>) {
    static_assert(!kFlatEpilogue<C> || EPI == CFHIP_EPI_NONE, "80-column wave tiles: bias / bf16 output / split-K slabs only");
    epilogue_flat<C>(p, acc, stage, m0, n0, z, wm, wn, wave, lane);
  } else {
    epilogue_std<EPI, C>(p, acc, stage, m0, n0, z, wm, wn, wave, lane);
  }
}

}
```

carefree-learn_amd/fused.py:

```python
import os
from typing import Any, Optional

import torch
from torch import Tensor
from torch.autograd import Function

from . import functional as _functional
from . import ops
from .functional import SideStream, bf16, f32, claim_grads, claim_grads_one_flag, commit_grads, shadow_bf16


FUSE_BIAS_GRAD = True
_SKIP_BIAS_GRAD = False


def _dw_db(w: Tensor, b: Optional[Tensor], dy2: Tensor, x2: Tensor) -> None:
    n, k = w.shape[0], x2.shape[1]
    split = ops.pick_split_k(n, k, x2.shape[0])
    prms = [w] + ([b] if (b is not None and b.requires_grad) else [])
    (gw, acc_w), *bias_claim = claim_grads(prms)
    kw = {}
    if bias_claim:
        gb, acc_b = bias_claim[0]
        if _SKIP_BIAS_GRAD:
            pass
        elif FUSE_BIAS_GRAD:
            kw = dict(bias_grad=gb.view(-1), bias_grad_accumulate=acc_b)
        else:
            SideStream.run(lambda: ops.colsum(dy2, out=gb.view(-1), accumulate=acc_b), (dy2,), lane=1)
    ops.gemm(dy2, x2, a_trans=True, b_trans=True, out=gw.view(n, k), accumulate=acc_w, split_k=split, **kw)
    commit_grads(prms)


DW_GROUP_BLOCKS = 2
DW_GROUP_TILES = 256
DW_TAIL_BLOCKS = 0
DW_GROUP_ON_MAIN = False
_pending_dw: list = []
_slice_streams: list = []


LINEAR_DW_TILES = 256
LINEAR_DW_MIN_ROWS = 49152
DW_MIN_TILES = 48
GROUP_MAX = 24
_end_flush_queued = False


def _groupable(w: Tensor, dy2: Tensor, x2: Tensor) -> bool:
    n, k = dy2.shape[1], x2.shape[1]
    g = w.grad
    if g is not None and (not g.is_contiguous() or g.data_ptr() % 16 != 0 or g.dtype != f32):
        return False
    return (dy2.is_cuda and w.numel() == n * k and w.is_contiguous() and n % 8 == 0 and k % 8 == 0 and dy2.stride(0) % 8 == 0
            and x2.stride(0) % 8 == 0 and x2.shape[0] * max(dy2.stride(0), x2.stride(0)) * 2 < 2 ** 31
            and dy2.data_ptr() % 16 == 0 and x2.data_ptr() % 16 == 0)


DW_PEROP_TAIL = 0
_perop_now = False


def _queue_dw(w: Tensor, b: Optional[Tensor], dy2: Tensor, x2: Tensor) -> None:
    if not w.requires_grad:
        if b is not None and b.requires_grad:
            SideStream.run(lambda: _functional.write_param_grad(b, lambda out, acc: ops.colsum(dy2, out=out.view(-1), accumulate=acc)),
                           (dy2,), wait=tuple(_slice_streams))
        return
    if DW_GROUP_BLOCKS <= 0 or _perop_now or not _groupable(w, dy2, x2):
        SideStream.run(lambda: _dw_db(w, b, dy2, x2), (dy2, x2), wait=tuple(_slice_streams))
        return
    _pending_dw.append((w, b, dy2, x2))


def queue_linear_dw(w: Tensor, b: Optional[Tensor], dy2: Tensor, x2: Tensor) -> bool:
    global _end_flush_queued
    if LINEAR_DW_TILES <= 0 or DW_GROUP_BLOCKS <= 0 or not w.requires_grad or x2.shape[0] < LINEAR_DW_MIN_ROWS or not _groupable(w, dy2, x2):
        return False
    if any(not getattr(getattr(cb, "__self__", None), "accepts_deferred_gradients", False) for cb in _functional.grad_ready_callbacks):
        return False
    if not _end_flush_queued:
        try:
            torch.autograd.Variable._execution_engine.queue_callback(_end_of_backward_flush)
        except RuntimeError:
            return False
        _end_flush_queued = True
    _pending_dw.append((w, b, dy2, x2))
    if _pending_tiles() >= LINEAR_DW_TILES:
        _flush_dw(tuple(_slice_streams))
    return True


def _end_of_backward_flush() -> None:
    global _end_flush_queued
    _end_flush_queued = False
    if _pending_dw:
        _flush_dw(tuple(_slice_streams))
        SideStream.join()


def _flush_deferred() -> None:
    if _pending_dw:
        _flush_dw(tuple(_slice_streams))


_functional.deferred_grad_flushes.append(_flush_deferred)


def _tiles_of(items: list) -> int:
    return sum(((dy2.shape[1] + 255) // 256) * ((x2.shape[1] + 255) // 256) for _, _, dy2, x2 in items)


def _pending_tiles() -> int:
    return _tiles_of(_pending_dw)


def _flush_dw(wait: tuple = ()) -> None:
    if not _pending_dw:
        return
    items = list(_pending_dw)
    _pending_dw.clear()
    few = _tiles_of(items) < DW_MIN_TILES
    if few:
        for w, b, dy2, x2 in items:
            SideStream.run(lambda w=w, b=b, dy2=dy2, x2=x2: _dw_db(w, b, dy2, x2), (dy2, x2), wait=wait)
        return
    launches: list = [[]]
    seen: set = set()
    for it in items:
        if id(it[0]) in seen or len(launches[-1]) == GROUP_MAX:
            launches.append([])
            seen = set()
        seen.add(id(it[0]))
        launches[-1].append(it)

    def launch() -> None:
        for group in launches:
            probs, done = [], []
            for w, b, dy2, x2 in group:
                prms = [w] + ([b] if (b is not None and b.requires_grad) else [])
                (gw, acc_w), *bias_claim = claim_grads(prms)
                bg, acc_b = None, False
                if bias_claim and not _SKIP_BIAS_GRAD:
                    bg, acc_b = bias_claim[0][0].view(-1), bias_claim[0][1]
                probs.append((dy2, x2, gw.view(dy2.shape[1], x2.shape[1]), acc_w, bg, acc_b))
                done.extend(prms)
            ops.gemm_grouped_tn(probs)
            commit_grads(done)

    if DW_GROUP_ON_MAIN:
        for st in wait:
            _functional.cur_stream().wait_stream(st)
        launch()
    else:
        SideStream.run(launch, tuple(t for it in items for t in (it[2], it[3])), wait=wait)


LN_REDUCE_ASIDE = True
SPLIT_LN_BWD = False


def _ln_defers(w: Tensor, b: Tensor, dy2: Tensor) -> bool:
    return (LN_REDUCE_ASIDE and not SPLIT_LN_BWD and dy2.is_cuda and SideStream.enabled and _functional.cuda_ok()
            and w.shape[0] % 256 == 0 and w.shape[0] <= 1280 and w.grad is not None and b.grad is not None
            and b.grad.dtype == f32 and b.grad.data_ptr() == w.grad.data_ptr() + 4 * w.numel() and dy2.stride(0) % 8 == 0)


def _ln_bwd(dy2: Tensor, x2: Tensor, w: Tensor, b: Tensor, mean: Tensor, rstd: Tensor,
            dx_add: Optional[Tensor], dx_out: Optional[Tensor] = None, notify: bool = True,
            dx_add_lo: Optional[Tensor] = None, dx_lo_out: Optional[Tensor] = None) -> Tensor:
    gamma = w.detach()
    if not (w.requires_grad and b.requires_grad):
        dx, dg, db = ops.layernorm_bwd(dy2, x2, gamma, mean, rstd, dx_add=dx_add, dx_out=dx_out, dx_add_lo=dx_add_lo, dx_lo_out=dx_lo_out)
        for prm, g in ((w, dg), (b, db)):
            if prm.requires_grad:
                ((buf, acc),) = claim_grads((prm,))
                buf.add_(g.view(buf.shape)) if acc else buf.copy_(g.view(buf.shape))
                commit_grads((prm,), notify)
        return dx
    if _ln_defers(w, b, dy2):
        dx, ws, rows = ops.layernorm_bwd_partials(dy2, x2, gamma, mean, rstd, dx_add=dx_add, dx_out=dx_out, dx_add_lo=dx_add_lo,
                                                  dx_lo_out=dx_lo_out)
        (gw, gb), acc = claim_grads_one_flag((w, b))
        d = w.shape[0]

        def reduce() -> None:
            ops.layernorm_bwd_reduce(ws, rows, d, gw.view(-1), gb.view(-1), acc)
            commit_grads((w, b), notify)

        SideStream.run(reduce, (ws,))
        return dx

    def param_grads(with_dx: bool = False) -> Optional[Tensor]:
        (gw, gb), acc = claim_grads_one_flag((w, b))
        dx, _, _ = ops.layernorm_bwd(dy2, x2, gamma, mean, rstd, dgamma=gw.view(-1), dbeta=gb.view(-1),
                                     accumulate=acc, want_dx=with_dx, dx_add=dx_add if with_dx else None,
                                     dx_out=dx_out if with_dx else None, dx_add_lo=dx_add_lo if with_dx else None,
                                     dx_lo_out=dx_lo_out if with_dx else None)
        commit_grads((w, b), notify)
        return dx

    if not SPLIT_LN_BWD:
        return param_grads(True)
    SideStream.run(param_grads, (dy2, x2, mean, rstd), lane=1)
    dx, _, _ = ops.layernorm_bwd(dy2, x2, gamma, mean, rstd, dx_add=dx_add, want_param_grads=False, dx_out=dx_out,
                                 dx_add_lo=dx_add_lo, dx_lo_out=dx_lo_out)
    return dx


FWD_HALVES = int(os.environ.get("CFHIP_FWD_HALVES", "2"))


def _block_fwd(x2: Tensor, prm: tuple, num_heads: int, eps1: float, eps2: float, bsz: int, t: int,
               keep_mask: Optional[Tensor], causal: bool, quick: bool = False, streams: Optional[list] = None,
               head_only: bool = False):
    ln1_w, ln1_b, in_w, qkv_b, out_w, out_b, ln2_w, ln2_b, w1, b1, w2, b2 = prm
    d = x2.shape[1]
    fb = lambda p: None if p is None else p.detach().reshape(-1)
    in_w16, out_w16 = shadow_bf16(in_w), shadow_bf16(out_w)
    w1_16, w2_16 = shadow_bf16(w1), shadow_bf16(w2)
    m, dev = bsz * t, x2.device
    ff = w1.shape[0]
    E = lambda *shape, dt=bf16: torch.empty(shape, dtype=dt, device=dev)
    ln1, mean1, rstd1 = E(m, d), E(m, dt=f32), E(m, dt=f32)
    qkv, o2, lse = E(m, 3 * d), E(m, d), E(bsz, num_heads, t, dt=f32)
    x1 = E(m, d, dt=x2.dtype)
    ln2, mean2, rstd2 = E(m, d), E(m, dt=f32), E(m, dt=f32)
    pre, h, y = E(m, ff), E(m, ff), E(m, d, dt=x2.dtype)
    act = ops.EPI_QGELU if quick else ops.EPI_GELU
    g1, bt1, g2, bt2 = ln1_w.detach(), ln1_b.detach(), ln2_w.detach(), ln2_b.detach()

    def run(b0: int, b1_: int) -> None:
        r = slice(b0 * t, b1_ * t)
        nb = b1_ - b0
        km = None if keep_mask is None else keep_mask[b0:b1_] if keep_mask.shape[0] == bsz else keep_mask
        ops.layernorm_fwd(x2[r], g1, bt1, eps1, out=ln1[r], mean=mean1[r], rstd=rstd1[r])
        ops.gemm(ln1[r], in_w16, bias=fb(qkv_b), out=qkv[r])
        q3 = qkv[r].view(nb, t, 3 * d)
        ops.attn_fwd(q3[..., :d], q3[..., d:2 * d], q3[..., 2 * d:], num_heads, mask=km, causal=causal,
                     out=o2[r].view(nb, t, d), lse=lse[b0:b1_])
        if head_only:
            rows = nb * t
            hv = lambda u: u[r].view(nb, -1)[:, :u.shape[1]]
            with _Unrecorded():
                ops.head_rows_zero(x1[r], d)
                ops.head_rows_zero(h[r], ff)
            ops.gemm(hv(o2), out_w16, bias=fb(out_b), epilogue=ops.EPI_RESIDUAL, aux_in=hv(x2), out=hv(x1), config_rows=rows)
            ops.layernorm_fwd(x1[r], g2, bt2, eps2, out=ln2[r], mean=mean2[r], rstd=rstd2[r])
            ops.gemm(hv(ln2), w1_16, bias=fb(b1), epilogue=act, aux_out=hv(pre), out=hv(h), config_rows=rows)
            ops.gemm(hv(h), w2_16, bias=fb(b2), epilogue=ops.EPI_RESIDUAL, aux_in=hv(x1), out=hv(y), config_rows=rows)
            return
        ops.gemm(o2[r], out_w16, bias=fb(out_b), epilogue=ops.EPI_RESIDUAL, aux_in=x2[r], out=x1[r])
        ops.layernorm_fwd(x1[r], g2, bt2, eps2, out=ln2[r], mean=mean2[r], rstd=rstd2[r])
        ops.gemm(ln2[r], w1_16, bias=fb(b1), epilogue=act, aux_out=pre[r], out=h[r])
        ops.gemm(h[r], w2_16, bias=fb(b2), epilogue=ops.EPI_RESIDUAL, aux_in=x1[r], out=y[r])

    if not streams or len(streams) == 1 or bsz < 2 * len(streams):
        run(0, bsz)
    else:
        n = len(streams)
        cuts = _slice_cuts(bsz, n)
        for i, st in enumerate(streams):
            with _functional.on_stream(st):
                run(cuts[i], cuts[i + 1])
    saved = (x2, mean1, rstd1, ln1, qkv, o2, lse, x1, mean2, rstd2, ln2, pre, h, in_w16, out_w16, w1_16, w2_16)
    return y, saved


N_SAVED = 17

FIRST_SLICE_SHARE = 0.5


def _slice_cuts(bsz: int, n: int) -> list:
    if n == 2 and FIRST_SLICE_SHARE != 0.5:
        first = min(bsz - 1, max(1, int(round(bsz * FIRST_SLICE_SHARE))))
        return [0, first, bsz]
    return [bsz * i // n for i in range(n + 1)]


BWD_HALVES = int(os.environ.get("CFHIP_BWD_HALVES", "2"))
SideStream.lanes = min(4, max(SideStream.lanes, BWD_HALVES, FWD_HALVES - 1))


class _Unrecorded:

    def __enter__(self) -> None:
        from . import _lib

        self.rec, _lib.RECORDER = _lib.RECORDER, None

    def __exit__(self, *exc: Any) -> None:
        from . import _lib

        _lib.RECORDER = self.rec


def _block_bwd(saved: tuple, prm: tuple, num_heads: int, bsz: int, t: int, keep_mask: Optional[Tensor],
               causal: bool, d2: Tensor, quick: bool = False, streams: Optional[list] = None, head_only: bool = False) -> Tensor:
    x2, mean1, rstd1, ln1, qkv, o2, lse, x1, mean2, rstd2, ln2, pre, h, in_w16, out_w16, w1_16, w2_16 = saved
    ln1_w, ln1_b, in_w, qkv_b, out_w, out_b, ln2_w, ln2_b, w1, b1, w2, b2 = prm
    two = d2.dim() == 3
    d2_full = d2
    d2, d2_lo = (d2[0], d2[1]) if two else (d2, None)
    d = d2.shape[1]
    m = bsz * t
    E = lambda cols: torch.empty((m, cols), dtype=bf16, device=d2.device)
    dpre, dqkv = E(pre.shape[1]), E(3 * d)
    if two:
        dx1_full, dx_full = (torch.empty((2, m, d), dtype=bf16, device=d2.device) for _ in range(2))
        (dx1, dx1_lo), (dx, dx_lo) = (dx1_full[0], dx1_full[1]), (dx_full[0], dx_full[1])
    else:
        dx1, dx = E(d), E(d)
        dx1_lo = dx_lo = None
        dx_full = dx
    qkv3, dqkv3, o3 = qkv.view(bsz, t, 3 * d), dqkv.view(bsz, t, 3 * d), o2.view(bsz, t, d)
    dact = ops.EPI_DQGELU if quick else ops.EPI_DGELU
    nsl = len(streams) if streams else 1
    if bsz < 2 * nsl:
        nsl, streams = 1, None
    cuts = _slice_cuts(bsz, nsl)
    ln_done: list = [None, None]

    def run(i: int) -> None:
        b0, b1_ = cuts[i], cuts[i + 1]
        r = slice(b0 * t, b1_ * t)
        nb = b1_ - b0
        last = i == nsl - 1
        km = None if keep_mask is None else keep_mask[b0:b1_] if keep_mask.shape[0] == bsz else keep_mask
        cur = _functional.cur_stream() if d2.is_cuda else None

        def ln(which: int, dy_, x_, w_, b_, mean_, rstd_, add_, out_, add_lo_=None, out_lo_=None) -> None:
            if _ln_defers(w_, b_, dy_):
                _ln_bwd(dy_, x_, w_, b_, mean_, rstd_, dx_add=add_, dx_out=out_, notify=last, dx_add_lo=add_lo_, dx_lo_out=out_lo_)
                return
            if ln_done[which] is not None:
                _functional.rec_wait_event(cur, ln_done[which])
            _ln_bwd(dy_, x_, w_, b_, mean_, rstd_, dx_add=add_, dx_out=out_, notify=last, dx_add_lo=add_lo_, dx_lo_out=out_lo_)
            if nsl > 1 and not last:
                ev = torch.cuda.Event()
                _functional.rec_record_event(ev, cur)
                ln_done[which] = ev

        if head_only:
            rows = nb * t
            hv = lambda u: u[r].view(nb, -1)[:, :u.shape[1]]
            dln2, d_o = (torch.empty((rows, d), dtype=bf16, device=d2.device) for _ in range(2))
            hv0 = lambda u: u.view(nb, -1)[:, :d]
            with _Unrecorded():
                ops.head_rows_zero(dpre[r], dpre.shape[1])
                ops.head_rows_zero(dln2, d)
                ops.head_rows_zero(d_o, d)
            ops.gemm(hv(d2), w2_16, b_trans=True, epilogue=dact, aux_in=hv(pre), out=hv(dpre), config_rows=rows)
            ops.gemm(hv(dpre), w1_16, b_trans=True, out=hv0(dln2), config_rows=rows)
        else:
            ops.gemm(d2[r], w2_16, b_trans=True, epilogue=dact, aux_in=pre[r], out=dpre[r])
            dln2 = ops.gemm(dpre[r], w1_16, b_trans=True)
        ln(0, dln2, x1[r], ln2_w, ln2_b, mean2[r], rstd2[r], d2[r], dx1[r], None if d2_lo is None else d2_lo[r],
           None if dx1_lo is None else dx1_lo[r])
        if head_only:
            ops.gemm(hv(dx1), out_w16, b_trans=True, out=hv0(d_o), config_rows=rows)
        else:
            d_o = ops.gemm(dx1[r], out_w16, b_trans=True)
        q3, dq3 = qkv3[b0:b1_], dqkv3[b0:b1_]
        ops.attn_bwd(q3[..., :d], q3[..., d:2 * d], q3[..., 2 * d:], o3[b0:b1_], d_o.view(nb, t, d), lse[b0:b1_], num_heads,
                     dq=dq3[..., :d], dk=dq3[..., d:2 * d], dv=dq3[..., 2 * d:], mask=km, causal=causal)
        dln1 = ops.gemm(dqkv[r], in_w16, b_trans=True)
        ln(1, dln1, x2[r], ln1_w, ln1_b, mean1[r], rstd1[r], dx1[r], dx[r], None if dx1_lo is None else dx1_lo[r],
           None if dx_lo is None else dx_lo[r])

    if nsl == 1:
        run(0)
    else:
        for i, st in enumerate(streams):
            with _functional.on_stream(st):
                run(i)
    _queue_dw(w2, b2, d2, h)
    _queue_dw(w1, b1, dpre, ln2)
    _queue_dw(out_w, out_b, dx1, o2)
    _queue_dw(in_w, qkv_b, dqkv, ln1)
    if two:
        SideStream.keep.append(d2_full)
    return dx_full


GRAD_STREAM_WORDS = int(os.environ.get("CFHIP_GRAD_STREAM_WORDS", "2"))

HEAD_ONLY = os.environ.get("CFHIP_HEAD_ONLY", "1") != "0"
HEAD_ONLY_MIN_ROWS = 1024


def _as_bf16_rows(dy: Tensor, rows: int, d: int, words: int = 1) -> Tensor:
    if words == 2:
        out = torch.empty((2, rows, d), dtype=bf16, device=dy.device)
        if dy.dtype == bf16:
            out[0].copy_(dy.contiguous().view(rows, d))
            out[1].zero_()
        else:
            ops.split_f32(dy.float().contiguous().view(rows, d), out[0], out[1])
        return out
    if dy.dtype != bf16:
        dy = ops.to_bf16(dy.float().contiguous())
    return dy.contiguous().view(rows, d)


class MixingBlockFn(Function):
    @staticmethod
    def forward(ctx: Any, x: Tensor, ln1_w: Tensor, ln1_b: Tensor, in_w: Tensor, qkv_b: Optional[Tensor],
                out_w: Tensor, out_b: Optional[Tensor], ln2_w: Tensor, ln2_b: Tensor, w1: Tensor,
                b1: Optional[Tensor], w2: Tensor, b2: Optional[Tensor], num_heads: int, eps1: float,
                eps2: float, keep_mask: Optional[Tensor], causal: bool, quick: bool = False) -> Tensor:
        bsz, t, d = x.shape
        if x.dtype not in (bf16, f32):
            x = x.float()
        x2 = x.contiguous().view(bsz * t, d)
        prm = (ln1_w, ln1_b, in_w, qkv_b, out_w, out_b, ln2_w, ln2_b, w1, b1, w2, b2)
        y, saved = _block_fwd(x2, prm, num_heads, eps1, eps2, bsz, t, keep_mask, causal, quick)
        ctx.save_for_backward(*saved, keep_mask)
        ctx.params = prm
        ctx.meta = (bsz, t, d, num_heads, causal, quick)
        return y.view(bsz, t, d)

    @staticmethod
    def backward(ctx: Any, dy: Tensor):
        *saved, keep_mask = ctx.saved_tensors
        bsz, t, d, num_heads, causal, quick = ctx.meta
        d2 = _as_bf16_rows(dy, bsz * t, d)
        dx = _block_bwd(tuple(saved), ctx.params, num_heads, bsz, t, keep_mask, causal, d2, quick)
        _flush_dw()
        return (dx.view(bsz, t, d),) + (None,) * 18


STACK_PLANS = os.environ.get("CFHIP_STACK_PLANS", "1") != "0"
_plans: dict = {}
_plan_conflicts: dict = {}
_PLAN_CACHE = 8


class StackPlan:
    def __init__(self, key: tuple, params: tuple) -> None:
        self.key = key
        self.calls = 0
        self.fwd: list = []
        self.bwd: list = []
        self.fwd_alt: Optional[list] = None
        self.bwd_alt: Optional[list] = None
        self.keep: list = []
        self.x_in: Optional[Tensor] = None
        self.y_out: Optional[Tensor] = None
        self.dy_in: Optional[Tensor] = None
        self.dx_out: Optional[Tensor] = None
        self.all_saved: Optional[list] = None
        self.w_ptr = 0
        self.w_alt = 0
        self.in_flight = False
        self.ready_fwd = False
        self.ready_bwd = False
        self.x_live: Optional[Tensor] = None
        self.x_sites: list = []
        self.dy_sites: list = []
        self.x_now = self.dy_now = 0
        self.disabled = False
        self.mask_tensor: Optional[Tensor] = None
        self.state = key[-1]
        self.params_ref = [__import__("weakref").ref(p) for p in params if p is not None][:1]

    @staticmethod
    def _subst(ops_: list, mp: dict) -> list:
        out = []
        for kind, f, a in ops_:
            if kind == 0:
                a = tuple(mp.get(v, v) if type(v) is int else v for v in a)
            out.append((kind, f, a))
        return out

    def _patch_sites(self, base: int, nbytes: int) -> list:
        sites = []
        for li, ops_ in enumerate((self.fwd, self.bwd)):
            for ei, (kind, _f, a) in enumerate(ops_):
                if kind == 3:
                    for pi in range(a):
                        for field in ("A", "B"):
                            v = getattr(_f[pi], field) or 0
                            if base <= v < base + nbytes:
                                sites.append((li, ei, (pi, field), v - base))
                    continue
                if kind != 0:
                    continue
                for ai, v in enumerate(a):
                    if type(v) is int and base <= v < base + nbytes:
                        sites.append((li, ei, ai, v - base))
        return sites

    def repoint(self, sites: list, new_base: int) -> None:
        for li, ei, ai, off in sites:
            if type(ai) is tuple:
                setattr((self.fwd if li == 0 else self.bwd)[ei][1][ai[0]], ai[1], new_base + off)
                continue
            for ops_ in ((self.fwd, self.fwd_alt) if li == 0 else (self.bwd, self.bwd_alt)):
                if ops_ is None:
                    continue
                kind, f, a = ops_[ei]
                ops_[ei] = (kind, f, a[:ai] + (new_base + off,) + a[ai + 1:])

    def finish_recording(self, params: tuple) -> None:
        self.x_sites = self._patch_sites(self.x_in.data_ptr(), self.x_in.numel() * self.x_in.element_size())
        self.dy_sites = self._patch_sites(self.dy_in.data_ptr(), self.dy_in.numel() * self.dy_in.element_size())
        self.x_now, self.dy_now = self.x_in.data_ptr(), self.dy_in.data_ptr()
        mp = {}
        for p in params:
            ar = getattr(p, "_cfhip_arena", None) if p is not None else None
            views = getattr(ar, "_shadow_views", None) if ar is not None else None
            if views is None:
                continue
            i = ar._index(p)
            a0, a1 = views[0][i].data_ptr(), views[1][i].data_ptr()
            mp[a0], mp[a1] = a1, a0
        if mp:
            self.fwd_alt, self.bwd_alt = self._subst(self.fwd, mp), self._subst(self.bwd, mp)
            self.w_alt = mp.get(self.w_ptr, 0)


def _replay(ops_: list) -> None:
    from . import _lib

    for kind, f, a in ops_:
        if kind == 0:
            rc = f(*a)
            if rc:
                _lib.check(rc, "launch plan")
        elif kind == 1:
            f(*a)
        elif kind == 3:
            continue
        else:
            with _functional.on_stream(a):
                commit_grads((f,))


class _KeepAllocations:

    def __init__(self, keep: list) -> None:
        self.keep = keep

    def __enter__(self) -> None:
        import threading

        self.empty, self.empty_like = torch.empty, torch.empty_like
        keep, e0, e1 = self.keep, self.empty, self.empty_like
        me, ident = threading.get_ident(), threading.get_ident

        def empty(*a, **k):
            t = e0(*a, **k)
            if ident() == me:
                keep.append(t)
            return t

        def empty_like(*a, **k):
            t = e1(*a, **k)
            if ident() == me:
                keep.append(t)
            return t

        torch.empty, torch.empty_like = empty, empty_like

    def __exit__(self, *exc) -> None:
        torch.empty, torch.empty_like = self.empty, self.empty_like


def _grad_state(params: tuple) -> Optional[tuple]:
    n_fresh = n = 0
    fp = 0
    for p in params:
        if p is None:
            continue
        g = p.grad
        if g is None or not p.requires_grad:
            return None
        n += 1
        n_fresh += 1 if getattr(p, "_cfhip_fresh", False) else 0
        fp = (fp * 1000003 + p.data_ptr() + 31 * g.data_ptr()) & 0xFFFFFFFFFFFFFFFF
    state = 1 if n_fresh == n else 0 if n_fresh == 0 else None
    return None if state is None else (state, fp)


def _plan_key(x: Tensor, metas: tuple, keep_mask: Optional[Tensor], causal: bool, state: tuple) -> tuple:
    return (tuple(x.shape), x.dtype, metas, causal, None if keep_mask is None else keep_mask.data_ptr(), FWD_HALVES, BWD_HALVES,
            DW_GROUP_BLOCKS, DW_GROUP_TILES, DW_TAIL_BLOCKS, DW_PEROP_TAIL, LN_REDUCE_ASIDE, DW_GROUP_ON_MAIN, FIRST_SLICE_SHARE, FUSE_BIAS_GRAD,
            ops.FORCE_SPLIT_K, tuple(id(cb) for cb in _functional.grad_ready_callbacks), x.requires_grad, GRAD_STREAM_WORDS, HEAD_ONLY,
            HEAD_ONLY_MIN_ROWS, state)


def _plan_for(x: Tensor, metas: tuple, keep_mask: Optional[Tensor], causal: bool, params: tuple, training: bool) -> Optional[StackPlan]:
    from . import _lib

    if (not STACK_PLANS or not x.is_cuda or not training or ops.GEMM_TIMER is not None or ops.FLOP_COUNTER is not None
            or _lib.RECORDER is not None or torch.cuda.is_current_stream_capturing() or params[2] is None):
        return None
    state = _grad_state(params)
    if state is None:
        return None
    key = _plan_key(x, metas, keep_mask, causal, state)
    pid = id(params[0])
    plan = _plans.get(pid)
    if plan is None or plan.key != key or (plan.params_ref and plan.params_ref[0]() is not params[0]):
        if len(_plans) >= _PLAN_CACHE:
            _plan_conflicts.pop(next(iter(_plans)), None)
            _plans.pop(next(iter(_plans)))
        if plan is not None and plan.params_ref and plan.params_ref[0]() is not params[0]:
            _plan_conflicts.pop(pid, None)
        plan = _plans[pid] = StackPlan(key, params)
    return plan


class MixingStackFn(Function):

    @staticmethod
    def _slices(metas: tuple, default: int) -> int:
        m0 = metas[0]
        return int(m0[4]) if len(m0) > 4 and m0[4] else default

    @staticmethod
    def _slices_bwd(metas: tuple, default: int) -> int:
        m0 = metas[0]
        return int(m0[5]) if len(m0) > 5 and m0[5] else MixingStackFn._slices(metas, default)

    @staticmethod
    def _words(metas: tuple, x_is_f32: bool) -> int:
        m0 = metas[0]
        w = int(m0[6]) if len(m0) > 6 and m0[6] else GRAD_STREAM_WORDS
        return 2 if (w == 2 and x_is_f32) else 1

    @staticmethod
    def _head_only(metas: tuple, keep_mask: Optional[Tensor], causal: bool, training: bool, rows: int) -> bool:
        m = metas[-1]
        return bool(HEAD_ONLY and len(m) > 7 and m[7] and training and keep_mask is None and not causal and rows >= HEAD_ONLY_MIN_ROWS)

    @staticmethod
    def _forward_body(cur: Tensor, bsz: int, t: int, metas: tuple, keep_mask: Optional[Tensor], causal: bool, params: tuple,
                      head_only: bool = False):
        nblk = len(metas)
        all_saved = []
        streams = None
        FWD_HALVES = MixingStackFn._slices(metas, globals()["FWD_HALVES"])
        if FWD_HALVES > 1 and cur.is_cuda and bsz >= 2 * FWD_HALVES:
            for i in range(nblk):
                for j in (2, 4, 8, 10):
                    shadow_bf16(params[12 * i + j])
            main = _functional.cur_stream()
            streams = [main] + [SideStream.fork(lane) for lane in range(FWD_HALVES - 1)]
            if any(st is None for st in streams):
                streams = None
        for i, meta in enumerate(metas):
            num_heads, eps1, eps2 = meta[:3]
            quick = bool(meta[3]) if len(meta) > 3 else False
            cur, saved = _block_fwd(cur, params[12 * i:12 * i + 12], num_heads, eps1, eps2, bsz, t, keep_mask, causal,
                                    quick, streams, head_only and i == nblk - 1)
            all_saved.extend(saved)
        if streams is not None:
            for st in streams[1:]:
                _functional.rec_wait_stream(_functional.cur_stream(), st)
        return cur, all_saved

    @staticmethod
    def forward(ctx: Any, x: Tensor, metas: tuple, keep_mask: Optional[Tensor], causal: bool,
                *params: Optional[Tensor]) -> Tensor:
        from . import _lib

        bsz, t, d = x.shape
        if x.dtype not in (bf16, f32):
            x = x.float()
        cur = x.contiguous().view(bsz * t, d)
        assert len(params) == 12 * len(metas)
        ctx.params = params
        ctx.meta = (bsz, t, d, metas, causal)
        ctx.words = MixingStackFn._words(metas, x.dtype == f32)
        ctx.plan = None
        ho = ctx.head_only = MixingStackFn._head_only(metas, keep_mask, causal, any(ctx.needs_input_grad), bsz * t)
        plan = _plan_for(x, metas, keep_mask, causal, params, any(ctx.needs_input_grad))
        if plan is not None and plan.in_flight and not plan.disabled:
            pid = id(params[0])
            n = _plan_conflicts[pid] = _plan_conflicts.get(pid, 0) + 1
            plan = _plans[pid] = StackPlan(plan.key, params)
            if n > 2:
                plan.disabled = True
                if n == 3:
                    import warnings

                    warnings.warn("cfhip: a block stack is called again before the backward of its previous call, repeatedly: "
                                  "launch plans are off for this stack (normal launch path; results are the same)")
        if plan is not None and not plan.in_flight and not plan.disabled:
            plan.calls += 1
            plan.mask_tensor = keep_mask
            for j in range(2, len(params), 12):
                for q in (params[j], params[j + 2], params[j + 6], params[j + 8]):
                    shadow_bf16(q)
            w_now = shadow_bf16(params[2]).data_ptr()
            if plan.ready_fwd and plan.ready_bwd and w_now in (plan.w_ptr, plan.w_alt):
                if cur.data_ptr() != plan.x_now:
                    plan.repoint(plan.x_sites, cur.data_ptr())
                    plan.x_now = cur.data_ptr()
                plan.x_live = cur
                _replay(plan.fwd if w_now == plan.w_ptr else plan.fwd_alt)
                plan.in_flight = True
                ctx.plan = plan
                ctx.plan_alt = w_now != plan.w_ptr
                return plan.y_out.detach().view(bsz, t, d)
            if plan.calls >= 2 and not plan.ready_fwd:
                plan.keep, plan.fwd, plan.bwd = [], [], []
                plan.w_ptr = w_now
                _lib.RECORDER = plan.fwd
                try:
                    with _KeepAllocations(plan.keep):
                        plan.x_in = cur
                        y, all_saved = MixingStackFn._forward_body(cur, bsz, t, metas, keep_mask, causal, params, ho)
                finally:
                    _lib.RECORDER = None
                plan.y_out, plan.all_saved = y, all_saved
                plan.ready_fwd, plan.in_flight = True, True
                ctx.plan, ctx.plan_alt = plan, False
                return y.detach().view(bsz, t, d)
        y, all_saved = MixingStackFn._forward_body(cur, bsz, t, metas, keep_mask, causal, params, ho)
        ctx.save_for_backward(*all_saved, keep_mask)
        return y.view(bsz, t, d)

    @staticmethod
    def _backward_body(all_saved: list, keep_mask: Optional[Tensor], bsz: int, t: int, metas: tuple, causal: bool, d2: Tensor,
                       params: tuple, head_only: bool = False) -> Tensor:
        streams = None
        BWD_HALVES = MixingStackFn._slices_bwd(metas, globals()["BWD_HALVES"])
        if BWD_HALVES > 1 and d2.is_cuda and bsz >= 2 * BWD_HALVES:
            main = _functional.cur_stream()
            streams = [main] + [SideStream.fork(lane + 1) for lane in range(BWD_HALVES - 1)]
            if any(st is None for st in streams) or len({id(st) for st in streams}) != len(streams) or SideStream.get(0) in streams[1:]:
                streams = None
        _slice_streams[:] = streams[1:] if streams else []
        try:
            for i in range(len(metas) - 1, -1, -1):
                saved = tuple(all_saved[N_SAVED * i:N_SAVED * (i + 1)])
                quick = bool(metas[i][3]) if len(metas[i]) > 3 else False
                before = _pending_tiles()
                global _perop_now
                if i < DW_PEROP_TAIL and not _perop_now:
                    _flush_dw(tuple(_slice_streams))
                    _perop_now = True
                d2 = _block_bwd(saved, params[12 * i:12 * i + 12], metas[i][0], bsz, t, keep_mask, causal, d2, quick, streams,
                                head_only and i == len(metas) - 1)
                if DW_GROUP_BLOCKS > 0 and DW_GROUP_TILES > 0:
                    now = _pending_tiles()
                    if now + (now - before) > DW_GROUP_TILES or i <= DW_TAIL_BLOCKS:
                        _flush_dw(tuple(_slice_streams))
                elif DW_GROUP_BLOCKS > 0 and (len(metas) - i) % DW_GROUP_BLOCKS == 0:
                    _flush_dw(tuple(_slice_streams))
            _flush_dw(tuple(_slice_streams))
            if streams is not None:
                for st in streams[1:]:
                    _functional.rec_wait_stream(_functional.cur_stream(), st)
                SideStream.keep.append(d2)
            if d2.dim() == 3:
                d2 = ops.join_bf16x2(d2[0], d2[1])
        except BaseException:
            _pending_dw.clear()
            raise
        finally:
            _slice_streams[:] = []
            _perop_now = False
        return d2

    @staticmethod
    def backward(ctx: Any, dy: Tensor):
        from . import _lib

        bsz, t, d, metas, causal = ctx.meta
        params = ctx.params
        plan: Optional[StackPlan] = ctx.plan
        nret = (None, None, None) + (None,) * len(params)
        if plan is None:
            *all_saved, keep_mask = ctx.saved_tensors
            d2 = _as_bf16_rows(dy, bsz * t, d, ctx.words)
            d2 = MixingStackFn._backward_body(list(all_saved), keep_mask, bsz, t, metas, causal, d2, params, ctx.head_only)
            return (d2.view(bsz, t, d),) + nret
        plan.in_flight = False
        if _plan_conflicts:
            _plan_conflicts.pop(id(params[0]), None)
        km = plan.mask_tensor
        fresh = _grad_state(params) == plan.state
        if plan.ready_bwd and fresh and _lib.RECORDER is None and ops.GEMM_TIMER is None and ops.FLOP_COUNTER is None:
            d2 = _as_bf16_rows(dy, bsz * t, d, ctx.words)
            if d2.data_ptr() != plan.dy_now:
                plan.repoint(plan.dy_sites, d2.data_ptr())
                plan.dy_now = d2.data_ptr()
            SideStream.queue_join()
            _replay(plan.bwd_alt if ctx.plan_alt else plan.bwd)
            SideStream.keep.append(d2)
            plan.x_live = None
            return (plan.dx_out.detach().view(bsz, t, d),) + nret
        if not plan.ready_bwd and fresh and _lib.RECORDER is None:
            d2 = _as_bf16_rows(dy, bsz * t, d, ctx.words)
            plan.dy_in = d2
            _lib.RECORDER = plan.bwd
            try:
                with _KeepAllocations(plan.keep):
                    dx = MixingStackFn._backward_body(plan.all_saved, km, bsz, t, metas, causal, d2, params, ctx.head_only)
            finally:
                _lib.RECORDER = None
            plan.dx_out = dx
            plan.keep.append(dx)
            plan.finish_recording(params)
            plan.ready_bwd = True
            return (dx.detach().view(bsz, t, d),) + nret
        d2 = _as_bf16_rows(dy, bsz * t, d, ctx.words)
        saved = list(plan.all_saved)
        if plan.x_live is not None:
            saved[0] = plan.x_live
            plan.x_live = None
        d2 = MixingStackFn._backward_body(saved, km, bsz, t, metas, causal, d2, params, ctx.head_only)
        return (d2.view(bsz, t, d),) + nret


def mixing_block(x: Tensor, *args: Any) -> Tensor:
    return MixingBlockFn.apply(x, *args)


def mixing_stack(x: Tensor, metas: tuple, keep_mask: Optional[Tensor], causal: bool, params: list) -> Tensor:
    return MixingStackFn.apply(x, metas, keep_mask, causal, *params)
```

carefree-learn_amd/ops.py:

```python
import math
import os
from typing import Dict, List, Optional, Sequence, Tuple

import ctypes

import torch
from torch import Tensor

from . import _lib

_H = _lib.DEFINES
EPI_NONE, EPI_GELU, EPI_RESIDUAL, EPI_DGELU, EPI_QGELU, EPI_DQGELU = (_H["CFHIP_EPI_" + e] for e in ("NONE", "GELU", "RESIDUAL", "DGELU", "QGELU", "DQGELU"))

bf16 = torch.bfloat16
f32 = torch.float32


_raw_stream = getattr(torch._C, "_cuda_getCurrentRawStream", None)
_raw_device = getattr(torch._C, "_cuda_getDevice", None)


def _stream() -> int:
    if _raw_stream is not None and _raw_device is not None:
        return _raw_stream(_raw_device())
    return torch.cuda.current_stream().cuda_stream


def _p(t: Optional[Tensor]) -> Optional[int]:
    return None if t is None else t.data_ptr()


def _need(t: Tensor, dtype: torch.dtype, name: str) -> None:
    if not t.is_cuda:
        raise RuntimeError(f"cfhip: `{name}` must live on the HIP device (got {t.device})")
    if t.dtype != dtype:
        raise TypeError(f"cfhip: `{name}` must be {dtype}, got {t.dtype}")


def _mat(t: Tensor, name: str) -> Tuple[int, int, int]:
    if t.dim() != 2 or t.stride(1) != 1:
        raise ValueError(f"cfhip: `{name}` must be 2-D with a contiguous last dim, got {tuple(t.shape)} / {t.stride()}")
    return t.shape[0], t.shape[1], t.stride(0)


def set_option(name: str, value: int) -> None:
    _lib.check(_lib.load().cfhip_set_option(name.encode(), int(value)), "set_option")




FORCE_SPLIT_K = 0


def pick_split_k(m: int, n: int, k: int) -> int:
    if FORCE_SPLIT_K > 0:
        return FORCE_SPLIT_K
    tiles = ((m + 127) // 128) * ((n + 127) // 128)
    steps = (k + 63) // 64
    if tiles >= 256 or steps < 16:
        return 1
    split = min(steps // 4, (512 + tiles - 1) // tiles, 32)
    return max(1, split)


class GemmTimer:

    def __init__(self) -> None:
        self.records: list = []

    def durations(self) -> dict:
        per: dict = {}
        for key, e0, e1 in self.records:
            e1.synchronize()
            per.setdefault(key, []).append(e0.elapsed_time(e1) * 1.0e-3)
        out: dict = {}
        for key, ds in per.items():
            med = sorted(ds)[len(ds) // 2]
            out[key] = [len(ds), sum(d if d <= 8.0 * med else med for d in ds)]
        return out


GEMM_TIMER: Optional[GemmTimer] = None


class FlopCounter:

    def __init__(self) -> None:
        self.flops = {"gemm": 0.0, "conv3x3": 0.0, "attention": 0.0}

    def total(self) -> float:
        return sum(self.flops.values())


FLOP_COUNTER: Optional[FlopCounter] = None


def gemm(
    a: Tensor,
    b: Tensor,
    *,
    a_trans: bool = False,
    b_trans: bool = False,
    bias: Optional[Tensor] = None,
    epilogue: int = EPI_NONE,
    aux_in: Optional[Tensor] = None,
    aux_out: Optional[Tensor] = None,
    out: Optional[Tensor] = None,
    out_dtype: torch.dtype = bf16,
    accumulate: bool = False,
    split_k: int = 1,
    bias_grad: Optional[Tensor] = None,
    bias_grad_accumulate: bool = False,
    config_rows: int = 0,
) -> Tensor:
    if a.dtype is not bf16 or b.dtype is not bf16 or not a.is_cuda or not b.is_cuda:
        _need(a, bf16, "a")
        _need(b, bf16, "b")
    sha, shb, sta, stb = a.shape, b.shape, a.stride(), b.stride()
    if len(sha) != 2 or sta[1] != 1:
        _mat(a, "a")
    if len(shb) != 2 or stb[1] != 1:
        _mat(b, "b")
    lda, ldb = sta[0], stb[0]
    m, k = (sha[1], sha[0]) if a_trans else (sha[0], sha[1])
    n, kb = (shb[1], shb[0]) if b_trans else (shb[0], shb[1])
    if k != kb:
        raise ValueError(f"cfhip gemm: reduction dims differ ({k} vs {kb})")
    if out is None:
        out = torch.empty((m, n), dtype=out_dtype, device=a.device)
        ldc, odt = n, out_dtype
    else:
        odt, sho, sto = out.dtype, out.shape, out.stride()
        if not out.is_cuda or (odt is not bf16 and odt is not f32) or len(sho) != 2 or sho[0] != m or sho[1] != n or sto[1] != 1:
            raise ValueError("cfhip gemm: bad `out`")
        ldc = sto[0]
    if bias is not None and (bias.dtype is not f32 or not bias.is_cuda or bias.numel() != n or not bias.is_contiguous()):
        _need(bias, f32, "bias")
        raise ValueError("cfhip gemm: bias must be a contiguous f32 [N]")
    if aux_in is not None or aux_out is not None:
        for t, nm in ((aux_in, "aux_in"), (aux_out, "aux_out")):
            if t is not None:
                _need(t, f32 if (nm == "aux_in" and epilogue == EPI_RESIDUAL and odt is f32) else bf16, nm)
                stt = t.stride()
                if tuple(t.shape) != (m, n) or stt[1] != 1 or stt[0] != ldc:
                    raise ValueError(f"cfhip gemm: `{nm}` must match the output layout")
    if bias_grad is not None:
        _need(bias_grad, f32, "bias_grad")
        if bias_grad.numel() != m or not bias_grad.is_contiguous():
            raise ValueError("cfhip gemm: bias_grad must be a contiguous f32 [M]")
    ws, ws_bytes = None, 0
    if split_k > 1:
        ws = torch.empty((split_k * m * (n + (1 if bias_grad is not None else 0)),), dtype=f32, device=a.device)
        ws_bytes = ws.numel() * 4
    if FLOP_COUNTER is not None:
        FLOP_COUNTER.flops["gemm"] += 2.0 * m * n * k
    timer = GEMM_TIMER
    if timer is not None:
        e0, e1 = torch.cuda.Event(enable_timing=True), torch.cuda.Event(enable_timing=True)
        e0.record()
    if config_rows:
        if a_trans or split_k > 1 or accumulate or bias_grad is not None or config_rows < m:
            raise ValueError("cfhip gemm: config_rows takes a_trans = False, no split_k / accumulate / bias_grad, and at least m rows")
        rc = _lib.load().cfhip_gemm_bf16_rows(a.data_ptr(), b.data_ptr(), out.data_ptr(), _p(bias), _p(aux_in), _p(aux_out), m, n, k, lda,
                                              ldb, ldc, int(b_trans), epilogue, 1 if odt is f32 else 0, int(config_rows), _stream())
    else:
        rc = _lib.load().cfhip_gemm_bf16(
            a.data_ptr(), b.data_ptr(), out.data_ptr(), _p(bias), _p(aux_in), _p(aux_out), m, n, k, lda,
            ldb, ldc, int(a_trans), int(b_trans), epilogue, 1 if odt is f32 else 0,
            int(accumulate), split_k, _p(ws), ws_bytes, _p(bias_grad), int(bias_grad_accumulate), _stream(),
        )
    _lib.check(rc, "gemm")
    if timer is not None:
        e1.record()
        layout = "tn" if a_trans else ("nn" if b_trans else "nt")
        timer.records.append(((layout, m, n, k, int(epilogue)), e0, e1))
    return out


def gemm_grouped_tn(problems: list) -> None:
    if not problems:
        return
    arr = (_lib.GemmProblem * len(problems))()
    flops = 0.0
    for i, (dy, x, out, acc, bg, bg_acc) in enumerate(problems):
        _need(dy, bf16, "dy")
        _need(x, bf16, "x")
        _need(out, f32, "out")
        k, m, lda = _mat(dy, "dy")
        kb, n, ldb = _mat(x, "x")
        if k != kb or tuple(out.shape) != (m, n) or out.stride(1) != 1:
            raise ValueError(f"cfhip gemm_grouped_tn: problem {i}: dy {tuple(dy.shape)} x {tuple(x.shape)} out {tuple(out.shape)}")
        if bg is not None:
            _need(bg, f32, "bias_grad")
            if bg.numel() != m or not bg.is_contiguous():
                raise ValueError("cfhip gemm_grouped_tn: bias_grad must be a contiguous f32 [M]")
        pr = arr[i]
        pr.A, pr.B, pr.C, pr.bias_grad = dy.data_ptr(), x.data_ptr(), out.data_ptr(), _p(bg)
        pr.M, pr.N, pr.K = m, n, k
        pr.lda, pr.ldb, pr.ldc = lda, ldb, out.stride(0)
        pr.accumulate, pr.bias_grad_accumulate = int(bool(acc)), int(bool(bg_acc))
        flops += 2.0 * m * n * k
    if FLOP_COUNTER is not None:
        FLOP_COUNTER.flops["gemm"] += flops
    timer = GEMM_TIMER
    if timer is not None:
        e0, e1 = torch.cuda.Event(enable_timing=True), torch.cuda.Event(enable_timing=True)
        e0.record()
    if _lib.RECORDER is not None:
        _lib.RECORDER.append((3, arr, len(problems)))
    rc = _lib.load().cfhip_gemm_bf16_grouped_tn(ctypes.cast(arr, ctypes.c_void_p), len(problems), _stream())
    _lib.check(rc, "gemm_grouped_tn")
    if timer is not None:
        e1.record()
        timer.records.append((("tn-grouped", tuple((int(pr.M), int(pr.N), int(pr.K)) for pr in arr), 0, 0, 0), e0, e1))


def colsum(x: Tensor, out: Optional[Tensor] = None, accumulate: bool = False) -> Tensor:
    _need(x, bf16, "x")
    m, n, ldx = _mat(x, "x")
    if out is None:
        out = torch.empty((n,), dtype=f32, device=x.device)
        accumulate = False
    _need(out, f32, "out")
    lib = _lib.load()
    nbytes = lib.cfhip_colsum_workspace(m, n)
    ws = torch.empty((max(nbytes, 4) // 4,), dtype=f32, device=x.device)
    rc = lib.cfhip_colsum_bf16(x.data_ptr(), out.data_ptr(), m, n, ldx, int(accumulate), ws.data_ptr(),
                               ws.numel() * 4, _stream())
    _lib.check(rc, "colsum")
    return out




def layernorm_fwd(
    x: Tensor, gamma: Tensor, beta: Tensor, eps: float, out: Optional[Tensor] = None,
    mean: Optional[Tensor] = None, rstd: Optional[Tensor] = None, out_f32: bool = False,
) -> Tuple[Tensor, Tensor, Tensor]:
    _need(x, x.dtype if x.dtype in (bf16, f32) else bf16, "x")
    _need(gamma, f32, "gamma")
    _need(beta, f32, "beta")
    m, d, xs = _mat(x, "x")
    if out is not None:
        out_f32 = out.dtype == f32
    if out_f32 and x.dtype != f32:
        raise ValueError("cfhip layernorm_fwd: an f32 output is built for f32 rows only")
    y = torch.empty((m, d), dtype=f32 if out_f32 else bf16, device=x.device) if out is None else out
    mean = torch.empty((m,), dtype=f32, device=x.device) if mean is None else mean
    rstd = torch.empty((m,), dtype=f32, device=x.device) if rstd is None else rstd
    rc = _lib.load().cfhip_layernorm_fwd(
        x.data_ptr(), int(x.dtype == f32) | (2 if out_f32 else 0), gamma.data_ptr(), beta.data_ptr(), y.data_ptr(), mean.data_ptr(),
        rstd.data_ptr(), m, d, xs, y.stride(0), float(eps), _stream(),
    )
    _lib.check(rc, "layernorm_fwd")
    return y, mean, rstd


def layernorm4d_fwd(x: Tensor, weight: Optional[Tensor], bias: Optional[Tensor], eps: float) -> Tuple[Tensor, Tensor, Tensor]:
    _need(x, bf16, "x")
    if x.dim() != 4 or not x.is_contiguous():
        raise ValueError("cfhip layernorm4d_fwd: a contiguous [B, C, H, W] tensor is expected")
    if (weight is None) != (bias is None):
        raise ValueError("cfhip layernorm4d_fwd: weight and bias come together")
    b, c, h, w = x.shape
    lib = _lib.load()
    nbytes = lib.cfhip_layernorm4d_workspace(b, c, h * w)
    ws = torch.empty((nbytes,), dtype=torch.uint8, device=x.device)
    y = torch.empty_like(x)
    mean = torch.empty((b,), dtype=f32, device=x.device)
    std = torch.empty((b,), dtype=f32, device=x.device)
    _lib.check(lib.cfhip_layernorm4d_fwd(x.data_ptr(), _p(weight), _p(bias), y.data_ptr(), mean.data_ptr(), std.data_ptr(), b, c, h * w,
                                         float(eps), ws.data_ptr(), nbytes, _stream()), "layernorm4d_fwd")
    return y, mean, std


def layernorm4d_bwd(dy: Tensor, x: Tensor, weight: Optional[Tensor], mean: Tensor, std: Tensor, eps: float, *, want_dx: bool = True,
                    dweight: Optional[Tensor] = None, dbias: Optional[Tensor] = None, accumulate: bool = False) -> Optional[Tensor]:
    _need(dy, bf16, "dy")
    _need(x, bf16, "x")
    if dy.shape != x.shape or not dy.is_contiguous() or not x.is_contiguous():
        raise ValueError("cfhip layernorm4d_bwd: dy and x must be contiguous [B, C, H, W] of one shape")
    b, c, h, w = x.shape
    lib = _lib.load()
    nbytes = lib.cfhip_layernorm4d_workspace(b, c, h * w)
    ws = torch.empty((nbytes,), dtype=torch.uint8, device=x.device)
    dx = torch.empty_like(x) if want_dx else None
    _lib.check(lib.cfhip_layernorm4d_bwd(dy.data_ptr(), x.data_ptr(), _p(weight), mean.data_ptr(), std.data_ptr(), _p(dx), _p(dweight),
                                         _p(dbias), int(accumulate), b, c, h * w, float(eps), ws.data_ptr(), nbytes, _stream()),
               "layernorm4d_bwd")
    return dx


def layernorm_bwd(
    dy: Tensor,
    x: Tensor,
    gamma: Tensor,
    mean: Tensor,
    rstd: Tensor,
    *,
    dx_add: Optional[Tensor] = None,
    dgamma: Optional[Tensor] = None,
    dbeta: Optional[Tensor] = None,
    accumulate: bool = False,
    want_dx: bool = True,
    want_param_grads: bool = True,
    dx_out: Optional[Tensor] = None,
    dx_add_lo: Optional[Tensor] = None,
    dx_lo_out: Optional[Tensor] = None,
) -> Tuple[Optional[Tensor], Optional[Tensor], Optional[Tensor]]:
    _need(dy, bf16, "dy")
    _need(x, x.dtype if x.dtype in (bf16, f32) else bf16, "x")
    m, d, xs = _mat(x, "x")
    _, _, dys = _mat(dy, "dy")
    if dx_out is not None and want_dx:
        _need(dx_out, bf16, "dx_out")
# ... 2798 lines not shown
```

include/cfhip.h:

```cpp
#ifndef CFHIP_H
#define CFHIP_H

#include <stddef.h>
#include <stdint.h>

#ifdef __cplusplus
extern "C" {
#endif

#define CFHIP_VERSION 100

#define CFHIP_OK 0
#define CFHIP_ERR_INVALID (-1)
#define CFHIP_ERR_LAUNCH (-2)
#define CFHIP_ERR_WORKSPACE (-3)

int cfhip_version(void);
const char* cfhip_last_error(void);
int cfhip_set_option(const char* name, int value);

#define CFHIP_EPI_NONE 0
#define CFHIP_EPI_GELU 1
#define CFHIP_EPI_RESIDUAL 2
#define CFHIP_EPI_DGELU 3
#define CFHIP_EPI_QGELU 4
#define CFHIP_EPI_DQGELU 5

int cfhip_gemm_bf16(const void* A, const void* B, void* C, const float* bias, const void* aux_in,
                    void* aux_out, int M, int N, int K, int64_t lda, int64_t ldb, int64_t ldc,
                    int a_trans, int b_trans, int epilogue, int out_dtype, int accumulate,
                    int split_k, void* workspace, size_t workspace_bytes, float* bias_grad,
                    int bias_grad_accumulate, void* stream);

int cfhip_gemm_kernel_name(int M, int N, int K, int a_trans, int b_trans, int epilogue, char* out, size_t out_bytes);

int cfhip_gemm_last_config(void);

typedef struct cfhip_gemm_problem {
  const void* A;
  const void* B;
  void* C;
  float* bias_grad;
  int M, N, K;
  int64_t lda, ldb, ldc;
  int accumulate;
  int bias_grad_accumulate;
} cfhip_gemm_problem;
int cfhip_gemm_bf16_grouped_tn(const cfhip_gemm_problem* problems, int count, void* stream);

size_t cfhip_colsum_workspace(int M, int N);
int cfhip_colsum_bf16(const void* X, float* out, int M, int N, int64_t ldx, int accumulate,
                      void* workspace, size_t workspace_bytes, void* stream);

int cfhip_layernorm_fwd(const void* x, int dtype_flags, const float* gamma, const float* beta, void* y,
                        float* mean, float* rstd, int M, int D, int64_t x_row_stride,
                        int64_t y_row_stride, float eps, void* stream);
size_t cfhip_layernorm_bwd_workspace(int M, int D);
int cfhip_layernorm_bwd(const void* dy, const void* x, int x_is_f32, const float* gamma, const float* mean,
                        const float* rstd, const void* dx_add, void* dx, float* dgamma, float* dbeta,
                        int M, int D, int64_t dy_row_stride, int64_t x_row_stride,
                        int64_t dx_row_stride, int accumulate_param_grads, void* workspace,
                        size_t workspace_bytes, void* stream);
int cfhip_layernorm_bwd_partials(const void* dy, const void* x, int x_is_f32, const float* gamma, const float* mean,
                                 const float* rstd, const void* dx_add, void* dx, int M, int D, int64_t dy_row_stride,
                                 int64_t x_row_stride, int64_t dx_row_stride, void* workspace, size_t workspace_bytes,
                                 int* rows_out, void* stream);
int cfhip_layernorm_bwd_reduce(void* workspace, int rows, int D, float* dgamma, float* dbeta, int accumulate, void* stream);
int cfhip_layernorm_bwd2(const void* dy, const void* x, int x_is_f32, const float* gamma, const float* mean,
                         const float* rstd, const void* dx_add, const void* dx_add_lo, void* dx, void* dx_lo,
                         float* dgamma, float* dbeta, int M, int D, int64_t dy_row_stride, int64_t x_row_stride,
                         int64_t dx_row_stride, int accumulate_param_grads, void* workspace, size_t workspace_bytes,
                         int* rows_out, void* stream);
size_t cfhip_layernorm4d_workspace(int B, int C, int HW);
int cfhip_layernorm4d_fwd(const void* x, const float* weight, const float* bias, void* y, float* mean, float* std, int B, int C,
                          int HW, float eps, void* workspace, size_t workspace_bytes, void* stream);
int cfhip_layernorm4d_bwd(const void* dy, const void* x, const float* weight, const float* mean, const float* std, void* dx,
                          float* dweight, float* dbias, int accumulate_param_grads, int B, int C, int HW, float eps, void* workspace,
                          size_t workspace_bytes, void* stream);
int cfhip_split_f32_bf16x2(const float* src, void* hi, void* lo, int64_t n, void* stream);
int cfhip_join_bf16x2_f32(const void* hi, const void* lo, float* dst, int64_t n, void* stream);

#define CFHIP_ATTN_MAX_T 256
#define CFHIP_ATTN_HEAD_DIM 64

int cfhip_attn_fwd(const void* q, const void* k, const void* v, void* o, float* lse,
                   const uint8_t* mask, int B, int H, int Tq, int Tk, int64_t q_stride_b,
                   int64_t q_stride_t, int64_t kv_stride_b, int64_t kv_stride_t, int64_t o_stride_b,
                   int64_t o_stride_t, int64_t ms_b, int64_t ms_h, int64_t ms_q, float scale,
                   int causal, void* stream);

int cfhip_attn_bwd(const void* q, const void* k, const void* v, const void* o, const void* d_o,
                   const float* lse, float* delta, const uint8_t* mask, void* dq, void* dk, void* dv,
                   int B, int H, int Tq, int Tk, int64_t q_stride_b, int64_t q_stride_t,
                   int64_t kv_stride_b, int64_t kv_stride_t, int64_t o_stride_b, int64_t o_stride_t,
                   int64_t ms_b, int64_t ms_h, int64_t ms_q, float scale, int causal, int parts,
                   void* stream);
int cfhip_attn_probs(const void* q, const void* k, const float* lse, const uint8_t* mask, float* probs, int B, int H,
                     int Tq, int Tk, int head_dim, int64_t q_stride_b, int64_t q_stride_t, int64_t k_stride_b,
                     int64_t k_stride_t, int64_t ms_b, int64_t ms_h, int64_t ms_q, float scale, int causal, void* stream);
int cfhip_attn_probs_bwd(const void* q, const void* k, const float* lse, const uint8_t* mask, const float* d_probs,
                         float* ds_workspace, void* dq, void* dk, int B, int H, int Tq, int Tk, int head_dim,
                         int64_t q_stride_b, int64_t q_stride_t, int64_t k_stride_b, int64_t k_stride_t, int64_t ms_b,
                         int64_t ms_h, int64_t ms_q, float scale, int causal, void* stream);

int cfhip_attn_fwd_dh(const void* q, const void* k, const void* v, void* o, float* lse,
                      const uint8_t* mask, int B, int H, int Tq, int Tk, int head_dim, int64_t q_stride_b,
                      int64_t q_stride_t, int64_t kv_stride_b, int64_t kv_stride_t, int64_t o_stride_b,
                      int64_t o_stride_t, int64_t ms_b, int64_t ms_h, int64_t ms_q, float scale, int causal,
                      void* stream);
int cfhip_attn_bwd_dh(const void* q, const void* k, const void* v, const void* o, const void* d_o,
                      const float* lse, float* delta, const uint8_t* mask, void* dq, void* dk, void* dv,
                      int B, int H, int Tq, int Tk, int head_dim, int64_t q_stride_b, int64_t q_stride_t,
                      int64_t kv_stride_b, int64_t kv_stride_t, int64_t o_stride_b, int64_t o_stride_t,
                      int64_t ms_b, int64_t ms_h, int64_t ms_q, float scale, int causal, int parts,
                      void* stream);
int cfhip_attn_fwd_dropout(const void* q, const void* k, const void* v, void* o, float* lse, const uint8_t* mask,
                           int B, int H, int Tq, int Tk, int head_dim, int64_t q_stride_b, int64_t q_stride_t,
                           int64_t kv_stride_b, int64_t kv_stride_t, int64_t o_stride_b, int64_t o_stride_t,
                           int64_t ms_b, int64_t ms_h, int64_t ms_q, float scale, int causal, float dropout_p,
                           uint64_t seed, uint64_t offset, void* stream);
int cfhip_attn_bwd_dropout(const void* q, const void* k, const void* v, const void* o, const void* d_o,
                           const float* lse, float* delta, const uint8_t* mask, void* dq, void* dk, void* dv, int B,
                           int H, int Tq, int Tk, int head_dim, int64_t q_stride_b, int64_t q_stride_t,
                           int64_t kv_stride_b, int64_t kv_stride_t, int64_t o_stride_b, int64_t o_stride_t,
                           int64_t ms_b, int64_t ms_h, int64_t ms_q, float scale, int causal, int parts,
                           float dropout_p, uint64_t seed, uint64_t offset, void* stream);
int cfhip_attn_dropout_mask(void* mask_out, int B, int H, int Tq, int Tk, float dropout_p, uint64_t seed,
                            uint64_t offset, void* stream);
int cfhip_attn_plan(int backward, int head_dim, int Tq, int Tk, int has_mask, int causal, int dropout, int parts,
                    int has_lse, char* out, size_t out_bytes);

#define CFHIP_ATTN_WIDE_MAX_HEAD_DIM 512
#define CFHIP_ATTN_WIDE_CHUNK 64
int cfhip_attn_wide_fwd(const void* q, const void* k, const void* v, void* o, float* lse, int B, int H, int Tq, int Tk,
                        int head_dim, int64_t q_stride_b, int64_t q_stride_t, int64_t kv_stride_b, int64_t kv_stride_t,
                        int64_t o_stride_b, int64_t o_stride_t, float scale, void* stream);

int cfhip_im2row(const void* img, int img_is_bf16, void* rows, int B, int C, int Hh, int Ww, int P,
                 void* stream);
int cfhip_assemble_tokens_fwd(const void* patches, const float* head_token, const float* pos,
                              void* x0, int x0_is_f32, int B, int Np, int D, void* stream);
int cfhip_assemble_tokens_bwd(const void* dx0, void* dpatches, float* dhead_token, float* dpos,
                              int B, int Np, int D, int accumulate, void* stream);

int cfhip_cast_f32_to_bf16(const float* src, void* dst, int64_t n, void* stream);
int cfhip_cast_bf16_to_f32(const void* src, float* dst, int64_t n, void* stream);
int cfhip_gelu_fwd(const void* x, void* y, int64_t n, void* stream);
int cfhip_gelu_bwd(const void* dy, const void* x, void* dx, int64_t n, void* stream);
int cfhip_quick_gelu_fwd(const void* x, void* y, int64_t n, void* stream);
int cfhip_quick_gelu_bwd(const void* dy, const void* x, void* dx, int64_t n, void* stream);
int cfhip_q_sample(const float* x, const float* noise, const int64_t* t, const float* sqrt_ac,
                   const float* sqrt_1mac, void* out, int out_is_f32, int64_t B, int64_t inner, void* stream);
int cfhip_mse_loss(const void* pred, const float* target, float* loss_sum, void* dpred, int64_t B, int64_t inner,
                   float grad_scale, void* stream);
int cfhip_diffusion_loss(const void* pred, const float* target, const float* weight, float* per_sample, void* dpred,
                         int64_t B, int64_t inner, int loss_type, void* stream);
#define CFHIP_SAMPLE_ROW 8
#define CFHIP_SAMPLER_DDIM 0
#define CFHIP_SAMPLER_BASIC 1
#define CFHIP_PARAM_EPS 0
#define CFHIP_PARAM_X0 1
#define CFHIP_PARAM_V 2
int cfhip_randn_f32(float* out, int64_t n, uint64_t seed, uint64_t offset, void* stream);
int cfhip_gaussian_posterior(const void* moments, int channels_last, float* z, float* kl, const float* noise, int deterministic,
                             int64_t B, int E, int64_t hw, float scale_factor, uint64_t seed, uint64_t offset, void* stream);
int cfhip_diffusion_sample_step(float* x, void* xin, const void* out_c, const void* out_u, float scale, const float* table,
                                int steps, const int* k, const float* noise, int64_t B, int64_t n, int kind, int param,
                                float temperature, int clip_last, int dup, uint64_t seed, uint64_t offset, void* stream);
int cfhip_diffusion_sample_advance(int* k, const float* table, int steps, int64_t* timesteps, int gb, void* stream);
#define CFHIP_KSAMPLE_ROW 12
#define CFHIP_KSAMPLER_EULER_A 0
#define CFHIP_KSAMPLER_HEUN 1
#define CFHIP_KSAMPLER_DPMPP_2M 2
int cfhip_k_sample_step(float* x, float* aux, void* xin, const void* out_c, const void* out_u, float scale, const float* table,
                        int rows, const int* k, const float* noise, int64_t B, int64_t n, int kind, int param, int clip_last,
                        int dup, uint64_t seed, uint64_t offset, void* stream);
int cfhip_k_sample_advance(int* k, const float* table, int rows, void* timesteps, int timesteps_int64, int gb, void* stream);
#define CFHIP_MERGE_NOISE_PHILOX 0
#define CFHIP_MERGE_NOISE_UNIFIED 1
#define CFHIP_MERGE_NOISE_BANK 2
int cfhip_diffusion_sample_step_ref(float* x, void* xin, const void* out_c, const void* out_u, float scale, const float* table,
                                    int steps, const int* k, const float* noise, int64_t B, int64_t n, int kind, int param,
                                    float temperature, int clip_last, int dup, uint64_t seed, uint64_t offset, const float* ref,
                                    const float* mask, int64_t mask_bstride, int64_t mask_cstride, int64_t hw, const float* side,
                                    const float* merge_noise, int merge_noise_mode, int merge_row0, void* stream);
int cfhip_diffusion_sample_merge(float* x, void* xin, int steps, const int* k, int64_t B, int64_t n, int dup, uint64_t seed,
                                 uint64_t offset, const float* ref, const float* mask, int64_t mask_bstride, int64_t mask_cstride,
                                 int64_t hw, const float* side, const float* merge_noise, int merge_noise_mode, int merge_row0,
                                 void* stream);
int cfhip_k_sample_step_ref(float* x, float* aux, void* xin, const void* out_c, const void* out_u, float scale, const float* table,
                            int rows, const int* k, const float* noise, int64_t B, int64_t n, int kind, int param, int clip_last,
                            int dup, uint64_t seed, uint64_t offset, const float* ref, const float* mask, int64_t mask_bstride,
                            int64_t mask_cstride, int64_t hw, void* stream);
#define CFHIP_VQ_MAX_DIM 64
#define CFHIP_VQ_LDS_FLOATS 8192
#define CFHIP_VQ_TWO_ROWS_MIN_GROUPS 512
int cfhip_vq_chunk(int D);
int cfhip_vq_code_sqnorm(const float* codebook, float* out, int N, int D, void* stream);
int cfhip_vq_nearest(const void* z, int z_is_f32, int channels_last, const float* codebook, const float* code_sq, int64_t* indices,
                     float* z_q, int64_t B, int D, int64_t hw, int N, float scale_factor, void* stream);
#define CFHIP_TOME_MAX_CHANNELS 1280
#define CFHIP_TOME_MAX_TOKENS 65536
int cfhip_tome_match(const void* x, const int* src_idx, const int* dst_idx, float* rinv, float* node_max, int* node_idx, int64_t B,
                     int N, int C, int n_src, int n_dst, void* stream);
int cfhip_tome_select(const float* node_max, const int* node_idx, const int* src_idx, const int* dst_idx, int* row_of_token,
                      int* token_of_row, int* member_off, int* members, int* cursor, int64_t B, int N, int n_src, int n_dst, int r,
                      void* stream);
int cfhip_tome_merge(const void* x, const int* token_of_row, const int* member_off, const int* members, void* out, int64_t B, int N,
                     int C, int n_src, int n_dst, int r, void* stream);
int cfhip_tome_unmerge_add(const void* y, const int* row_of_token, const void* residual, void* out, int out_is_f32, int64_t B, int N,
                           int C, int r, void* stream);
int cfhip_copy_strided_bf16(const void* src, void* dst, int64_t batch, int64_t n, int64_t src_batch_stride,
                            int64_t dst_batch_stride, void* stream);
int cfhip_copy_strided2_bf16(const void* src_a, void* dst_a, int64_t n_a, int64_t src_a_batch_stride, int64_t dst_a_batch_stride,
                             const void* src_b, void* dst_b, int64_t n_b, int64_t src_b_batch_stride, int64_t dst_b_batch_stride,
                             int64_t batch, void* stream);
int cfhip_geglu_fwd(const void* vg, void* out, int64_t M, int L, void* stream);
int cfhip_geglu_bwd(const void* dy, const void* vg, void* dvg, int64_t M, int L, void* stream);
int cfhip_add_bf16(const void* a, const void* b, void* out, int64_t n, void* stream);
int cfhip_transpose_bf16(const void* src, void* dst, int R, int C, int64_t ld_src, int64_t ld_dst,
                         void* stream);

int cfhip_adam_step(float* p, const float* g, float* m, float* v, void* p_bf16, int64_t n, float lr,
                    double beta1, double beta2, float eps, float weight_decay, int decoupled, int step,
                    float grad_scale, void* stream);
int cfhip_adam_step_dev(float* p, const float* g, float* m, float* v, void* p_bf16, int64_t n,
                        const float* hyper, int decoupled, void* stream);
int cfhip_ema_update(float* ema, const float* p, int64_t n, float one_minus_decay, float decay, void* stream);
size_t cfhip_conv3x3_workspace(int B, int H, int W, int Cin, int Cout);
int cfhip_conv3x3_nhwc_bf16(const void* X, const void* Wk, const float* bias, void* Y, int B, int H, int W, int Cin,
                            int Cout, void* workspace, size_t workspace_bytes, void* stream);
size_t cfhip_conv3x3_wgrad_workspace(int Cin, int Cout, int split_k);
int cfhip_conv3x3_wgrad_nhwc_bf16(const void* dY, const void* X, float* dW, int accumulate, float* bias_grad,
                                  int bias_grad_accumulate, int B, int H, int W, int Cin, int Cout, int split_k,
                                  void* workspace, size_t workspace_bytes, void* stream);
int cfhip_conv3x3_pack_filters(const void* w, void* out, int Cout, int Cin, int rotate, void* stream);
#define CFHIP_PACK_GROUP_MAX 64
int cfhip_conv3x3_pack_filters_grouped(const int64_t* table, int count, void* stream);
int cfhip_conv3x3_direct_pack(const float* w, void* wp, int Cout, int Cin, int mode, void* stream);
int cfhip_conv3x3_direct_bf16(const void* x, const void* wp, const float* bias, void* y, int B, int H, int W, int Cp, int N,
                              int stride, int mode, void* stream);
int cfhip_silu_bf16_fwd(const void* x, void* y, int64_t n, void* stream);
int cfhip_silu_bf16_bwd(const void* dy, const void* x, void* dx, int64_t n, void* stream);
int cfhip_scale_bf16(const void* x, void* y, int64_t n, float scale, void* stream);
#define CFHIP_DENSE_TILE_H 8
#define CFHIP_DENSE_TILE_W 32
#define CFHIP_DENSE_EPI_NONE 0
#define CFHIP_DENSE_EPI_LRELU 1
#define CFHIP_DENSE_EPI_RES1 2
#define CFHIP_DENSE_EPI_RES2 3
int cfhip_conv3x3_dense_bf16(const void* x, const void* wp, const float* bias, void* y, const void* r1, const void* r2, int B, int H, int W,
                             int Cin, int N, int n_store, int64_t ld_in, int64_t ld_out, int64_t ld_r1, int64_t ld_r2, int epilogue,
                             float slope, float s1, float s2, int up2, int out_f32_nchw, void* stream);
int cfhip_pixel_unshuffle_nhwc(const void* x, int x_is_f32, void* y, int64_t B, int C, int H, int W, int s, void* stream);
int cfhip_spin(int microseconds, void* stream);
int cfhip_sumsq_f32(const float* g, float* out, int64_t n, void* stream);

int cfhip_softmax_xent(const float* logits, const int64_t* labels, float* loss_sum, float* dlogits,
                       int B, int C, float grad_scale, void* stream);
int cfhip_softmax_focal(const float* logits, const int64_t* labels, float* loss_sum, float* dlogits,
                        int B, int C, float gamma, float eps, float grad_scale, void* stream);

int cfhip_conv_im2row(const void* x, int x_is_f32, void* rows, int B, int C, int H, int W, int kh,
                      int kw, int stride, int pad, int dil, int Kp, void* stream);
int cfhip_conv_row2im(const void* drows, void* dx, int B, int C, int H, int W, int kh, int kw,
                      int stride, int pad, int dil, int Kp, void* stream);
int cfhip_conv_im2row_pad(const void* x, int x_is_f32, void* rows, int B, int C, int H, int W, int kh, int kw, int stride,
                          int pad_t, int pad_b, int pad_l, int pad_r, int dil, int Kp, void* stream);
int cfhip_conv_row2im_pad(const void* drows, void* dx, int B, int C, int H, int W, int kh, int kw, int stride, int pad_t,
                          int pad_b, int pad_l, int pad_r, int dil, int Kp, void* stream);
int cfhip_transpose_batched(const void* src, int src_is_f32, void* dst, int batch, int R, int C,
                            void* stream);
int cfhip_batchnorm_fwd(const void* x, int x_is_f32, const float* gamma, const float* beta, void* y,
                        float* mean, float* rstd, float* running_mean, float* running_var, int B, int C,
                        int inner, float eps, float momentum, int training, void* stream);
int cfhip_batchnorm_bwd(const void* dy, const void* x, int x_is_f32, const float* gamma,
                        const float* mean, const float* rstd, void* dx, float* dgamma, float* dbeta,
                        int B, int C, int inner, int accumulate, int training, void* stream);
int cfhip_leaky_relu_fwd(const void* x, void* y, int64_t n, float slope, void* stream);
int cfhip_leaky_relu_bwd(const void* dy, const void* x, void* dx, int64_t n, float slope, void* stream);
int cfhip_avgpool_fwd(const void* x, void* y, int64_t BC, int inner, void* stream);
int cfhip_avgpool_bwd(const void* dy, void* dx, int64_t BC, int inner, void* stream);

#define CFHIP_GN_MAX_CG 128
int cfhip_groupnorm_fwd(const void* x, int x_is_f32, const float* add, const float* gamma, const float* beta,
                        void* y, float* mean, float* rstd, int B, int C, int G, int inner, float eps, int silu,
                        int affine_batch_stride, int splits, float* workspace, void* stream);
int cfhip_groupnorm_bwd(const void* dy, const void* x, int x_is_f32, const float* add, const float* gamma,
                        const float* beta, const float* mean, const float* rstd, void* dx, float* dgamma_part,
                        float* dbeta_part, float* dadd, int B, int C, int G, int inner, int silu,
                        int affine_batch_stride, int splits, float* workspace, void* stream);
int cfhip_silu_f32_fwd(const float* x, float* y, int64_t n, void* stream);
int cfhip_silu_f32_bwd(const float* dy, const float* x, float* dx, int64_t n, void* stream);
#define CFHIP_TIME_PROJ_MAX 32
int cfhip_time_proj_fwd(const float* emb, int B, int K, const int64_t* table, int count, void* t_bf16, void* stream);
int cfhip_time_proj_bwd(const float* emb, int B, int K, const int64_t* table, int count, float* partial, float* d_emb, void* stream);
int cfhip_upsample2_fwd(const void* x, void* y, int64_t BC, int H, int W, void* stream);
int cfhip_upsample2_bwd(const void* dy, void* dx, int64_t BC, int H, int W, void* stream);
int cfhip_avgpool2_fwd(const void* x, void* y, int64_t BC, int Ho, int Wo, void* stream);
int cfhip_avgpool2_bwd(const void* dy, void* dx, int64_t BC, int Ho, int Wo, void* stream);
size_t cfhip_groupnorm_nhwc_workspace(int B, int C, int G, int splits, int backward, int with_add);
int cfhip_groupnorm_nhwc_fwd(const void* x, const float* add, const float* gamma, const float* beta, void* y, float* mean, float* rstd,
                             int B, int C, int G, int inner, float eps, int silu, int affine_batch_stride, int splits, float* workspace,
                             void* stream);
int cfhip_groupnorm_nhwc_bwd(const void* dy, const void* x, const float* add, const float* gamma, const float* beta, const float* mean,
                             const float* rstd, void* dx, float* dgamma_part, float* dbeta_part, float* dadd, int B, int C, int G, int inner,
                             int silu, int affine_batch_stride, int splits, float* workspace, void* stream);
int cfhip_upsample2_nhwc_fwd(const void* x, void* y, int64_t B, int H, int W, int C, void* stream);
int cfhip_upsample2_nhwc_bwd(const void* dy, void* dx, int64_t B, int H, int W, int C, void* stream);
int cfhip_reflect_pad2d_fwd(const void* x, int x_is_f32, void* y, int64_t BC, int H, int W, int pl, int pr, int pt, int pb,
                            void* stream);
int cfhip_reflect_pad2d_bwd(const void* dy, void* dx, int64_t BC, int H, int W, int pl, int pr, int pt, int pb, void* stream);
int cfhip_colreduce_f32(const float* x, float* out, int R, int D, int accumulate, void* stream);
int cfhip_colreduce2_f32(const float* x_a, float* out_a, const float* x_b, float* out_b, int R, int D, int accumulate, void* stream);
int cfhip_timestep_embedding(const int64_t* t, float* out, int B, int dim, float max_period, void* stream);
int cfhip_timestep_embedding_f32(const float* t, float* out, int B, int dim, float max_period, void* stream);


int cfhip_embedding_fwd(const float* table, const int64_t* indices, const float* pos, void* out,
                        int out_is_f32, int64_t N, int D, int T, int64_t V, void* stream);
int cfhip_embedding_bwd(const void* dy, int dy_is_f32, const int64_t* indices, float* dtable, int64_t N,
                        int D, int64_t V, int64_t padding_idx, void* stream);
int cfhip_l2norm_fwd(const float* x, float* y, float* inv_norm, int64_t N, int D, void* stream);
int cfhip_l2norm_bwd(const float* dy, const float* y, const float* inv_norm, float* dx, int64_t N, int D,
                     void* stream);
int cfhip_sgemm_f32(const float* A, const float* B, float* C, int M, int N, int K, int64_t lda, int64_t ldb,
                    int a_trans, int b_trans, const float* alpha_dev, float alpha, void* stream);
int cfhip_dot_f32(const float* a, const float* b, float* out, int64_t n, void* stream);

// ... 146 lines not shown
```

Measured before the change: 7509.

## Save encoded GELU derivative in forward epilogue, multiply it in backward

The FC1 forward GEMM epilogue now computes the GELU derivative alongside the activation and stores it as a 16-bit fixed-point code in place of the pre-activation. The backward FC2 dgrad GEMM then decodes that code and multiplies, so the erf/sigmoid evaluation in the backward epilogue is skipped. This moves transcendental work from backward into the forward epilogue, which now computes both values. The fixed-point encoding (scale 1/32768, offset) changes gradient precision relative to recomputing from the bf16 pre-activation.

New measurement: 7545, median of 6. About the same (+0.5%).

```diff
diff --git a/carefree-learn_amd/csrc/common.h b/carefree-learn_amd/csrc/common.h
--- a/carefree-learn_amd/csrc/common.h
+++ b/carefree-learn_amd/csrc/common.h
@@ -98,6 +98,34 @@
   return s * fmaf(1.702f * x, 1.0f - s, 1.0f);
 }
 
+__device__ __forceinline__ unsigned grad_code_enc(float d) {
+  return __float_as_uint(fmaf(d, 32768.0f, 8388608.0f + 16384.0f)) & 0xffffu;
+}
+__device__ __forceinline__ unsigned grad_code_enc2(float d_lo, float d_hi) {
+  return __builtin_amdgcn_perm(__float_as_uint(fmaf(d_hi, 32768.0f, 8388608.0f + 16384.0f)),
+                               __float_as_uint(fmaf(d_lo, 32768.0f, 8388608.0f + 16384.0f)), 0x05040100u);
+}
+__device__ __forceinline__ float grad_code_dec(unsigned code) {
+  return fmaf(__uint_as_float(0x4B000000u | code), 1.0f / 32768.0f, -256.5f);
+}
+__device__ __forceinline__ float grad_code_dec_lo(unsigned w) {
+  return fmaf(__uint_as_float((w & 0xffffu) | 0x4B000000u), 1.0f / 32768.0f, -256.5f);
+}
+__device__ __forceinline__ float grad_code_dec_hi(unsigned w) {
+  return fmaf(__uint_as_float(__builtin_amdgcn_perm(0x4B000000u, w, 0x07060302u)), 1.0f / 32768.0f, -256.5f);
+}
+__device__ __forceinline__ void gelu_erf_both(float x, float& h, float& d) {
+  float cdf, e;
+  gelu_parts(x, cdf, e);
+  h = x * cdf;
+  d = fmaf(x * 0.39894228040143267794f, e, cdf);
+}
+__device__ __forceinline__ void quick_gelu_both(float x, float& h, float& d) {
+  const float s = sigmoid_1702(x);
+  h = x * s;
+  d = s * fmaf(1.702f * x, 1.0f - s, 1.0f);
+}
+
 struct Philox {
   unsigned c[4];
 };
diff --git a/carefree-learn_amd/csrc/gemm.hip b/carefree-learn_amd/csrc/gemm.hip
--- a/carefree-learn_amd/csrc/gemm.hip
+++ b/carefree-learn_amd/csrc/gemm.hip
@@ -238,10 +238,16 @@
   gemm_tile<AT, BT, EPI, C, CONV, BG>(p, xcd_item(), smem);
 }
 
+template <bool AT, bool BT, int EPI, class C>
+__global__ __launch_bounds__(C::NT, C::WAVES_PER_SIMD)
+void gemm_bf16_sgrad_kernel(GemmParams p) {
+  static_assert(EPI == CFHIP_EPI_GELU_SAVE_GRAD || EPI == CFHIP_EPI_MUL_SAVED_GRAD, "the saved-derivative forms only");
+  extern __shared__ __attribute__((aligned(16))) char smem[];
+  gemm_tile<AT, BT, EPI, C, 0, false>(p, xcd_item(), smem);
+}
+
 template <bool AT, bool BT, int EPI, class C, int CONV = 0>
-__global__ __launch_bounds__(C::NT, C::WAVES_PER_SIMD)
-void gemm_bf16_phase_kernel(GemmParams p) {
-  extern __shared__ __attribute__((aligned(16))) char smem[];
+__device__ __forceinline__ void gemm_phase_tile(const GemmParams& p, char* smem) {
   static_assert(C::BK == 32 && C::NSTAGE >= 3 && C::NSTAGE <= 7 && C::WM == 2, "phase kernel: BK = 32, 3-7 ring slots, 2 wave rows");
   static_assert(5 * C::LPS < 64, "vmcnt is a 6-bit counter");
   constexpr int D = C::NSTAGE - 1;
@@ -318,6 +324,21 @@
   epilogue<EPI, C>(p, acc, smem, cur.m0, cur.n0, cur.z, wm, wn, wave, lane);
 }
 
+template <bool AT, bool BT, int EPI, class C, int CONV = 0>
+__global__ __launch_bounds__(C::NT, C::WAVES_PER_SIMD)
+void gemm_bf16_phase_kernel(GemmParams p) {
+  extern __shared__ __attribute__((aligned(16))) char smem[];
+  gemm_phase_tile<AT, BT, EPI, C, CONV>(p, smem);
+}
+
+template <bool AT, bool BT, int EPI, class C>
+__global__ __launch_bounds__(C::NT, C::WAVES_PER_SIMD)
+void gemm_bf16_sgrad_phase_kernel(GemmParams p) {
+  static_assert(EPI == CFHIP_EPI_GELU_SAVE_GRAD || EPI == CFHIP_EPI_MUL_SAVED_GRAD, "the saved-derivative forms only");
+  extern __shared__ __attribute__((aligned(16))) char smem[];
+  gemm_phase_tile<AT, BT, EPI, C, 0>(p, smem);
+}
+
 __global__ void splitk_reduce_kernel(const float* __restrict__ slabs, void* C, const float* bias,
                                      int M, int N, long ldc, int splits, int out_f32, int accumulate,
                                      const float* __restrict__ bgrad_slabs, float* bgrad, int bgrad_acc) {
@@ -404,6 +425,14 @@
       acc += p.out_f32 ? reinterpret_cast<const float*>(p.aux_in)[off] : bf16_to_f32(p.aux_in[off]);
     } else if (p.epilogue == CFHIP_EPI_DGELU) {
       acc *= p.quick ? quick_gelu_grad_f(bf16_to_f32(p.aux_in[off])) : gelu_erf_grad_f(bf16_to_f32(p.aux_in[off]));
+    } else if (p.epilogue == CFHIP_EPI_GELU_SAVE_GRAD) {
+      const float pre = bf16_to_f32(f32_to_bf16(acc));
+      float d;
+      if (p.quick) quick_gelu_both(pre, acc, d);
+      else gelu_erf_both(pre, acc, d);
+      if (p.aux_out != nullptr) p.aux_out[off] = (bf16_t)grad_code_enc(d);
+    } else if (p.epilogue == CFHIP_EPI_MUL_SAVED_GRAD) {
+      acc *= grad_code_dec(p.aux_in[off]);
     }
     if (p.out_f32) {
       float* dst = reinterpret_cast<float*>(p.C) + off;
@@ -454,7 +483,11 @@
     cfhip_set_error("gemm: the fused bias gradient is not provided by the big-tile kernel (gemm_config 7 / 8)");
     return CFHIP_ERR_INVALID;
   }
-  if constexpr (PIPE) kern = gemm_bf16_phase_kernel<AT, BT, EPI, C, CONV>;
+  if constexpr (EPI == CFHIP_EPI_GELU_SAVE_GRAD || EPI == CFHIP_EPI_MUL_SAVED_GRAD) {
+    static_assert(CONV == 0, "the saved-derivative forms are Linear epilogues");
+    if constexpr (PIPE) kern = gemm_bf16_sgrad_phase_kernel<AT, BT, EPI, C>;
+    else kern = gemm_bf16_sgrad_kernel<AT, BT, EPI, C>;
+  } else if constexpr (PIPE) kern = gemm_bf16_phase_kernel<AT, BT, EPI, C, CONV>;
   else if constexpr (AT && BT && EPI == CFHIP_EPI_NONE) {
     if (p.bgrad != nullptr) {
       if constexpr (C::BM * C::BN <= 192 * 128) kern = gemm_bf16_kernel<AT, BT, EPI, C, CONV, true>;
@@ -504,6 +537,9 @@
       case CFHIP_EPI_RESIDUAL:
         if constexpr (kHasEpilogues<C, PIPE>) return launch_cfg<false, false, CFHIP_EPI_RESIDUAL, C, PIPE>(p, grid, s);
         break;
+      case CFHIP_EPI_GELU_SAVE_GRAD:
+        if constexpr (kHasEpilogues<C, PIPE>) return launch_cfg<false, false, CFHIP_EPI_GELU_SAVE_GRAD, C, PIPE>(p, grid, s);
+        break;
       default: break;
     }
   } else if (!a_trans && b_trans) {
@@ -511,6 +547,9 @@
       case CFHIP_EPI_NONE: return launch_cfg<false, true, CFHIP_EPI_NONE, C, PIPE>(p, grid, s);
       case CFHIP_EPI_DGELU:
         if constexpr (kHasEpilogues<C, PIPE>) return launch_cfg<false, true, CFHIP_EPI_DGELU, C, PIPE>(p, grid, s);
+        break;
+      case CFHIP_EPI_MUL_SAVED_GRAD:
+        if constexpr (kHasEpilogues<C, PIPE>) return launch_cfg<false, true, CFHIP_EPI_MUL_SAVED_GRAD, C, PIPE>(p, grid, s);
         break;
       default: break;
     }
@@ -629,7 +668,9 @@
 static int resolve_config(int cfg, int a_trans, int epilogue, bool bias_grad) {
   if (cfg == 8 && a_trans) cfg = 1;
   if (bias_grad && ((cfg >= 7 && cfg <= 13) || cfg == 16)) cfg = 1;
-  if (cfg == 1 && (epilogue == CFHIP_EPI_RESIDUAL || epilogue == CFHIP_EPI_DGELU)) cfg = 3;
+  if (cfg == 1 && (epilogue == CFHIP_EPI_RESIDUAL || epilogue == CFHIP_EPI_DGELU || epilogue == CFHIP_EPI_GELU_SAVE_GRAD ||
+                   epilogue == CFHIP_EPI_MUL_SAVED_GRAD))
+    cfg = 3;
   return cfg;
 }
 
@@ -641,11 +682,14 @@
       "Cfg<256, 128, 2, 4, 3, 32>", "Cfg<256, 128, 2, 2, 3, 32>", "Cfg<128, 256, 2, 2, 3, 32>", "Cfg<256, 128, 2, 4, 6, 32>",
       "Cfg<256, 256, 2, 4, 5, 32>", "Cfg<256, 256, 2, 4, 2, 64>", "Cfg<192, 128, 2, 4, 2, 64>", "Cfg<192, 128, 2, 2, 2, 64>",
       "Cfg<128, 256, 2, 4, 2, 64>"};
-  int epi = epilogue == CFHIP_EPI_QGELU ? CFHIP_EPI_GELU : epilogue == CFHIP_EPI_DQGELU ? CFHIP_EPI_DGELU : epilogue;
+  int epi = epilogue == CFHIP_EPI_QGELU ? CFHIP_EPI_GELU : epilogue == CFHIP_EPI_DQGELU ? CFHIP_EPI_DGELU
+          : epilogue == CFHIP_EPI_QGELU_SAVE_GRAD ? CFHIP_EPI_GELU_SAVE_GRAD : epilogue;
   int cfg = pick_config(M, N, a_trans, b_trans);
   cfg = resolve_config(cfg, a_trans, epi, false);
   const bool phase = cfg >= 7 && cfg <= 12;
-  snprintf(out, out_bytes, "%s<%s, %s, %d, %s>", phase ? "gemm_bf16_phase_kernel" : "gemm_bf16_kernel",
+  const bool sgrad = epi == CFHIP_EPI_GELU_SAVE_GRAD || epi == CFHIP_EPI_MUL_SAVED_GRAD;
+  snprintf(out, out_bytes, "%s<%s, %s, %d, %s>",
+           sgrad ? (phase ? "gemm_bf16_sgrad_phase_kernel" : "gemm_bf16_sgrad_kernel") : (phase ? "gemm_bf16_phase_kernel" : "gemm_bf16_kernel"),
            a_trans ? "true" : "false", b_trans ? "true" : "false", epi, cfg_names[cfg]);
   return CFHIP_OK;
 }
@@ -663,14 +707,16 @@
   CFHIP_REQUIRE(bias_grad == nullptr || (a_trans && b_trans),
                 "gemm: the fused bias gradient exists for layout (1,1) only");
   CFHIP_REQUIRE(M > 0 && N > 0 && K > 0, "gemm: empty problem M=%d N=%d K=%d", M, N, K);
-  CFHIP_REQUIRE(epilogue >= 0 && epilogue <= 5, "gemm: bad epilogue %d", epilogue);
-  const int quick = epilogue == CFHIP_EPI_QGELU || epilogue == CFHIP_EPI_DQGELU;
+  CFHIP_REQUIRE(epilogue >= 0 && epilogue <= CFHIP_EPI_MUL_SAVED_GRAD, "gemm: bad epilogue %d", epilogue);
+  const int quick = epilogue == CFHIP_EPI_QGELU || epilogue == CFHIP_EPI_DQGELU || epilogue == CFHIP_EPI_QGELU_SAVE_GRAD;
   if (epilogue == CFHIP_EPI_QGELU) epilogue = CFHIP_EPI_GELU;
   if (epilogue == CFHIP_EPI_DQGELU) epilogue = CFHIP_EPI_DGELU;
-  CFHIP_REQUIRE(!(epilogue == CFHIP_EPI_RESIDUAL || epilogue == CFHIP_EPI_DGELU) || aux_in,
+  if (epilogue == CFHIP_EPI_QGELU_SAVE_GRAD) epilogue = CFHIP_EPI_GELU_SAVE_GRAD;
+  CFHIP_REQUIRE(!(epilogue == CFHIP_EPI_RESIDUAL || epilogue == CFHIP_EPI_DGELU || epilogue == CFHIP_EPI_MUL_SAVED_GRAD) || aux_in,
                 "gemm: epilogue %d needs aux_in", epilogue);
   CFHIP_REQUIRE(!accumulate || (out_dtype == 1 && epilogue == CFHIP_EPI_NONE), "gemm: accumulate needs f32 output and epilogue NONE");
-  CFHIP_REQUIRE(!(epilogue == CFHIP_EPI_GELU || epilogue == CFHIP_EPI_DGELU) || out_dtype == 0,
+  CFHIP_REQUIRE(!(epilogue == CFHIP_EPI_GELU || epilogue == CFHIP_EPI_DGELU || epilogue == CFHIP_EPI_GELU_SAVE_GRAD ||
+                  epilogue == CFHIP_EPI_MUL_SAVED_GRAD) || out_dtype == 0,
                 "gemm: the GELU / GELU' epilogues write bf16");
   CFHIP_REQUIRE(!(a_trans && !b_trans), "gemm: layout (a_trans=1, b_trans=0) is not provided");
   if (split_k < 1) split_k = 1;
diff --git a/carefree-learn_amd/csrc/gemm_device.h b/carefree-learn_amd/csrc/gemm_device.h
--- a/carefree-learn_amd/csrc/gemm_device.h
+++ b/carefree-learn_amd/csrc/gemm_device.h
@@ -268,7 +268,10 @@
   constexpr int RPP = 64 / LPR;
   constexpr int PPM = 16 / RPP;
   constexpr int NIT = C::FM * PPM;
-  constexpr bool HAS_AUX = EPI == CFHIP_EPI_RESIDUAL || EPI == CFHIP_EPI_DGELU;
+  constexpr bool SAVE_GRAD = EPI == CFHIP_EPI_GELU_SAVE_GRAD;
+  constexpr bool ACT = EPI == CFHIP_EPI_GELU || SAVE_GRAD;
+  constexpr bool SAVED = EPI == CFHIP_EPI_DGELU || EPI == CFHIP_EPI_MUL_SAVED_GRAD;
+  constexpr bool HAS_AUX = EPI == CFHIP_EPI_RESIDUAL || SAVED;
   constexpr bool AUX_F32 = EPI == CFHIP_EPI_RESIDUAL && F32;
   constexpr int PFW = AUX_F32 ? CFHIP_PF_F32 : CFHIP_PF_BF16;
   constexpr int PF = HAS_AUX ? (PFW < NIT ? PFW : NIT) : 1;
@@ -287,8 +290,8 @@
   const __amdgpu_buffer_rsrc_t c_rsrc = tile_rsrc(p.C, p.ldc, ES, m0, n0, p.M, p.N);
   __amdgpu_buffer_rsrc_t x_rsrc = c_rsrc, o_rsrc = c_rsrc;
   if constexpr (HAS_AUX) x_rsrc = tile_rsrc(p.aux_in, p.ldc, AES, m0, n0, p.M, p.N);
-  if constexpr (EPI == CFHIP_EPI_GELU) o_rsrc = tile_rsrc(p.aux_out, p.ldc, 2, m0, n0, p.M, p.N);
-  const bool has_pre = EPI == CFHIP_EPI_GELU && p.aux_out != nullptr;
+  if constexpr (ACT) o_rsrc = tile_rsrc(p.aux_out, p.ldc, 2, m0, n0, p.M, p.N);
+  const bool has_pre = ACT && p.aux_out != nullptr;
   auto eoff = [&](int it) -> unsigned { return (unsigned)((lrow0 + (it / PPM) * 16 + (it % PPM) * RPP) * (int)p.ldc + lcol); };
   auto load_aux = [&](int it) -> AuxRegs {
     AuxRegs r;
@@ -297,7 +300,7 @@
     if constexpr (AUX_F32) {
       r.a = bload16(x_rsrc, c_lo ? e * 4u : OOB);
       r.b = bload16(x_rsrc, c_hi ? e * 4u + 16u : OOB);
-    } else if constexpr (EPI == CFHIP_EPI_DGELU) {
+    } else if constexpr (SAVED) {
       if constexpr (N8) {
         r.a = bload16_pre(x_rsrc, c_lo ? e * 2u : OOB);
       } else {
@@ -336,7 +339,30 @@
     const unsigned e = eoff(it);
     lo += b_lo;
     hi += b_hi;
-    if constexpr (EPI == CFHIP_EPI_GELU) {
+    if constexpr (SAVE_GRAD) {
+      const u32x4 w = {pack_bf16x2(lo[0], lo[1]), pack_bf16x2(lo[2], lo[3]), pack_bf16x2(hi[0], hi[1]),
+                       pack_bf16x2(hi[2], hi[3])};
+      float h[8], d[8];
+#pragma unroll
+      for (int j = 0; j < 4; ++j) {
+        if constexpr (QUICK) {
+          quick_gelu_both(bf16lo(w[j]), h[2 * j], d[2 * j]);
+          quick_gelu_both(bf16hi(w[j]), h[2 * j + 1], d[2 * j + 1]);
+        } else {
+          gelu_erf_both(bf16lo(w[j]), h[2 * j], d[2 * j]);
+          gelu_erf_both(bf16hi(w[j]), h[2 * j + 1], d[2 * j + 1]);
+        }
+      }
+      const u32x4 cw = {grad_code_enc2(d[0], d[1]), grad_code_enc2(d[2], d[3]), grad_code_enc2(d[4], d[5]), grad_code_enc2(d[6], d[7])};
+      if constexpr (N8) {
+        bstore16_pre(o_rsrc, (has_pre && c_lo) ? e * 2u : OOB, cw);
+      } else {
+        bstore8_pre(o_rsrc, (has_pre && c_lo) ? e * 2u : OOB, u32x2{cw[0], cw[1]});
+        bstore8_pre(o_rsrc, (has_pre && c_hi) ? e * 2u + 8u : OOB, u32x2{cw[2], cw[3]});
+      }
+      lo = f32x4{h[0], h[1], h[2], h[3]};
+      hi = f32x4{h[4], h[5], h[6], h[7]};
+    } else if constexpr (EPI == CFHIP_EPI_GELU) {
       const u32x4 w = {pack_bf16x2(lo[0], lo[1]), pack_bf16x2(lo[2], lo[3]), pack_bf16x2(hi[0], hi[1]),
                        pack_bf16x2(hi[2], hi[3])};
       if constexpr (N8) {
@@ -360,6 +386,9 @@
       if constexpr (EPI == CFHIP_EPI_RESIDUAL) {
         lo += f32x4{bf16lo(w[0]), bf16hi(w[0]), bf16lo(w[1]), bf16hi(w[1])};
         hi += f32x4{bf16lo(w[2]), bf16hi(w[2]), bf16lo(w[3]), bf16hi(w[3])};
+      } else if constexpr (EPI == CFHIP_EPI_MUL_SAVED_GRAD) {
+        lo *= f32x4{grad_code_dec_lo(w[0]), grad_code_dec_hi(w[0]), grad_code_dec_lo(w[1]), grad_code_dec_hi(w[1])};
+        hi *= f32x4{grad_code_dec_lo(w[2]), grad_code_dec_hi(w[2]), grad_code_dec_lo(w[3]), grad_code_dec_hi(w[3])};
       } else if constexpr (QUICK) {
         lo *= f32x4{quick_gelu_grad_f(bf16lo(w[0])), quick_gelu_grad_f(bf16hi(w[0])), quick_gelu_grad_f(bf16lo(w[1])), quick_gelu_grad_f(bf16hi(w[1]))};
         hi *= f32x4{quick_gelu_grad_f(bf16lo(w[2])), quick_gelu_grad_f(bf16hi(w[2])), quick_gelu_grad_f(bf16lo(w[3])), quick_gelu_grad_f(bf16hi(w[3]))};
@@ -555,7 +584,10 @@
       return;
     }
   }
-  if constexpr (EPI == CFHIP_EPI_GELU || EPI == CFHIP_EPI_DGELU) {
+  if constexpr (EPI == CFHIP_EPI_MUL_SAVED_GRAD) {
+    if ((p.N & 7) == 0) epilogue_impl<EPI, C, false, true, false>(p, acc, stage, m0, n0, wm, wn, wave, lane);
+    else epilogue_impl<EPI, C, false, false, false>(p, acc, stage, m0, n0, wm, wn, wave, lane);
+  } else if constexpr (EPI == CFHIP_EPI_GELU || EPI == CFHIP_EPI_DGELU || EPI == CFHIP_EPI_GELU_SAVE_GRAD) {
     if (p.quick) {
       if ((p.N & 7) == 0) epilogue_impl<EPI, C, false, true, true>(p, acc, stage, m0, n0, wm, wn, wave, lane);
       else epilogue_impl<EPI, C, false, false, true>(p, acc, stage, m0, n0, wm, wn, wave, lane);
diff --git a/carefree-learn_amd/fused.py b/carefree-learn_amd/fused.py
--- a/carefree-learn_amd/fused.py
+++ b/carefree-learn_amd/fused.py
@@ -210,6 +210,8 @@
 
 FWD_HALVES = int(os.environ.get("CFHIP_FWD_HALVES", "2"))
 
+SAVE_ACT_GRAD = True
+
 
 def _block_fwd(x2: Tensor, prm: tuple, num_heads: int, eps1: float, eps2: float, bsz: int, t: int,
                keep_mask: Optional[Tensor], causal: bool, quick: bool = False, streams: Optional[list] = None,
@@ -226,8 +228,11 @@
     qkv, o2, lse = E(m, 3 * d), E(m, d), E(bsz, num_heads, t, dt=f32)
     x1 = E(m, d, dt=x2.dtype)
     ln2, mean2, rstd2 = E(m, d), E(m, dt=f32), E(m, dt=f32)
-    pre, h, y = E(m, ff), E(m, ff), E(m, d, dt=x2.dtype)
-    act = ops.EPI_QGELU if quick else ops.EPI_GELU
+    dact, h, y = E(m, ff), E(m, ff), E(m, d, dt=x2.dtype)
+    if SAVE_ACT_GRAD:
+        act = ops.EPI_QGELU_SAVE_GRAD if quick else ops.EPI_GELU_SAVE_GRAD
+    else:
+        act = ops.EPI_QGELU if quick else ops.EPI_GELU
     g1, bt1, g2, bt2 = ln1_w.detach(), ln1_b.detach(), ln2_w.detach(), ln2_b.detach()
 
     def run(b0: int, b1_: int) -> None:
@@ -247,12 +252,12 @@
                 ops.head_rows_zero(h[r], ff)
             ops.gemm(hv(o2), out_w16, bias=fb(out_b), epilogue=ops.EPI_RESIDUAL, aux_in=hv(x2), out=hv(x1), config_rows=rows)
             ops.layernorm_fwd(x1[r], g2, bt2, eps2, out=ln2[r], mean=mean2[r], rstd=rstd2[r])
-            ops.gemm(hv(ln2), w1_16, bias=fb(b1), epilogue=act, aux_out=hv(pre), out=hv(h), config_rows=rows)
+            ops.gemm(hv(ln2), w1_16, bias=fb(b1), epilogue=act, aux_out=hv(dact), out=hv(h), config_rows=rows)
             ops.gemm(hv(h), w2_16, bias=fb(b2), epilogue=ops.EPI_RESIDUAL, aux_in=hv(x1), out=hv(y), config_rows=rows)
             return
         ops.gemm(o2[r], out_w16, bias=fb(out_b), epilogue=ops.EPI_RESIDUAL, aux_in=x2[r], out=x1[r])
         ops.layernorm_fwd(x1[r], g2, bt2, eps2, out=ln2[r], mean=mean2[r], rstd=rstd2[r])
-        ops.gemm(ln2[r], w1_16, bias=fb(b1), epilogue=act, aux_out=pre[r], out=h[r])
+        ops.gemm(ln2[r], w1_16, bias=fb(b1), epilogue=act, aux_out=dact[r], out=h[r])
         ops.gemm(h[r], w2_16, bias=fb(b2), epilogue=ops.EPI_RESIDUAL, aux_in=x1[r], out=y[r])
 
     if not streams or len(streams) == 1 or bsz < 2 * len(streams):
@@ -263,7 +268,7 @@
         for i, st in enumerate(streams):
             with _functional.on_stream(st):
                 run(cuts[i], cuts[i + 1])
-    saved = (x2, mean1, rstd1, ln1, qkv, o2, lse, x1, mean2, rstd2, ln2, pre, h, in_w16, out_w16, w1_16, w2_16)
+    saved = (x2, mean1, rstd1, ln1, qkv, o2, lse, x1, mean2, rstd2, ln2, dact, h, in_w16, out_w16, w1_16, w2_16)
     return y, saved
 
 
@@ -298,7 +303,7 @@
 
 def _block_bwd(saved: tuple, prm: tuple, num_heads: int, bsz: int, t: int, keep_mask: Optional[Tensor],
                causal: bool, d2: Tensor, quick: bool = False, streams: Optional[list] = None, head_only: bool = False) -> Tensor:
-    x2, mean1, rstd1, ln1, qkv, o2, lse, x1, mean2, rstd2, ln2, pre, h, in_w16, out_w16, w1_16, w2_16 = saved
+    x2, mean1, rstd1, ln1, qkv, o2, lse, x1, mean2, rstd2, ln2, dact, h, in_w16, out_w16, w1_16, w2_16 = saved
     ln1_w, ln1_b, in_w, qkv_b, out_w, out_b, ln2_w, ln2_b, w1, b1, w2, b2 = prm
     two = d2.dim() == 3
     d2_full = d2
@@ -306,7 +311,7 @@
     d = d2.shape[1]
     m = bsz * t
     E = lambda cols: torch.empty((m, cols), dtype=bf16, device=d2.device)
-    dpre, dqkv = E(pre.shape[1]), E(3 * d)
+    dpre, dqkv = E(dact.shape[1]), E(3 * d)
     if two:
         dx1_full, dx_full = (torch.empty((2, m, d), dtype=bf16, device=d2.device) for _ in range(2))
         (dx1, dx1_lo), (dx, dx_lo) = (dx1_full[0], dx1_full[1]), (dx_full[0], dx_full[1])
@@ -315,7 +320,7 @@
         dx1_lo = dx_lo = None
         dx_full = dx
     qkv3, dqkv3, o3 = qkv.view(bsz, t, 3 * d), dqkv.view(bsz, t, 3 * d), o2.view(bsz, t, d)
-    dact = ops.EPI_DQGELU if quick else ops.EPI_DGELU
+    dact_epi = ops.EPI_MUL_SAVED_GRAD if SAVE_ACT_GRAD else ops.EPI_DQGELU if quick else ops.EPI_DGELU
     nsl = len(streams) if streams else 1
     if bsz < 2 * nsl:
         nsl, streams = 1, None
@@ -351,10 +356,10 @@
                 ops.head_rows_zero(dpre[r], dpre.shape[1])
                 ops.head_rows_zero(dln2, d)
                 ops.head_rows_zero(d_o, d)
-            ops.gemm(hv(d2), w2_16, b_trans=True, epilogue=dact, aux_in=hv(pre), out=hv(dpre), config_rows=rows)
+            ops.gemm(hv(d2), w2_16, b_trans=True, epilogue=dact_epi, aux_in=hv(dact), out=hv(dpre), config_rows=rows)
             ops.gemm(hv(dpre), w1_16, b_trans=True, out=hv0(dln2), config_rows=rows)
         else:
-            ops.gemm(d2[r], w2_16, b_trans=True, epilogue=dact, aux_in=pre[r], out=dpre[r])
+            ops.gemm(d2[r], w2_16, b_trans=True, epilogue=dact_epi, aux_in=dact[r], out=dpre[r])
             dln2 = ops.gemm(dpre[r], w1_16, b_trans=True)
         ln(0, dln2, x1[r], ln2_w, ln2_b, mean2[r], rstd2[r], d2[r], dx1[r], None if d2_lo is None else d2_lo[r],
            None if dx1_lo is None else dx1_lo[r])
@@ -588,7 +593,7 @@
     return (tuple(x.shape), x.dtype, metas, causal, None if keep_mask is None else keep_mask.data_ptr(), FWD_HALVES, BWD_HALVES,
             DW_GROUP_BLOCKS, DW_GROUP_TILES, DW_TAIL_BLOCKS, DW_PEROP_TAIL, LN_REDUCE_ASIDE, DW_GROUP_ON_MAIN, FIRST_SLICE_SHARE, FUSE_BIAS_GRAD,
             ops.FORCE_SPLIT_K, tuple(id(cb) for cb in _functional.grad_ready_callbacks), x.requires_grad, GRAD_STREAM_WORDS, HEAD_ONLY,
-            HEAD_ONLY_MIN_ROWS, state)
+            HEAD_ONLY_MIN_ROWS, SAVE_ACT_GRAD, state)
 
 
 def _plan_for(x: Tensor, metas: tuple, keep_mask: Optional[Tensor], causal: bool, params: tuple, training: bool) -> Optional[StackPlan]:
diff --git a/carefree-learn_amd/ops.py b/carefree-learn_amd/ops.py
--- a/carefree-learn_amd/ops.py
+++ b/carefree-learn_amd/ops.py
@@ -11,6 +11,9 @@
 
 _H = _lib.DEFINES
 EPI_NONE, EPI_GELU, EPI_RESIDUAL, EPI_DGELU, EPI_QGELU, EPI_DQGELU = (_H["CFHIP_EPI_" + e] for e in ("NONE", "GELU", "RESIDUAL", "DGELU", "QGELU", "DQGELU"))
+EPI_GELU_SAVE_GRAD, EPI_QGELU_SAVE_GRAD, EPI_MUL_SAVED_GRAD = (_H["CFHIP_EPI_" + e] for e in ("GELU_SAVE_GRAD", "QGELU_SAVE_GRAD", "MUL_SAVED_GRAD"))
+EPI_LABELS = {EPI_NONE: "none", EPI_GELU: "gelu", EPI_RESIDUAL: "residual", EPI_DGELU: "dgelu", EPI_QGELU: "qgelu", EPI_DQGELU: "dqgelu",
+              EPI_GELU_SAVE_GRAD: "gelu", EPI_QGELU_SAVE_GRAD: "qgelu", EPI_MUL_SAVED_GRAD: "dgelu"}
 
 bf16 = torch.bfloat16
 f32 = torch.float32
diff --git a/include/cfhip.h b/include/cfhip.h
--- a/include/cfhip.h
+++ b/include/cfhip.h
@@ -25,6 +25,9 @@
 #define CFHIP_EPI_DGELU 3
 #define CFHIP_EPI_QGELU 4
 #define CFHIP_EPI_DQGELU 5
+#define CFHIP_EPI_GELU_SAVE_GRAD 6
+#define CFHIP_EPI_QGELU_SAVE_GRAD 7
+#define CFHIP_EPI_MUL_SAVED_GRAD 8
 
 int cfhip_gemm_bf16(const void* A, const void* B, void* C, const float* bias, const void* aux_in,
                     void* aux_out, int M, int N, int K, int64_t lda, int64_t ldb, int64_t ldc,
```
